# gisbi-kim/lt-mapper

Hardware: AMD Instinct MI355X
Metric: keyframe-pairs/sec (removert+diff) (higher is better)
Workload: dtype f32; 1 GPU; lot-2x500-os1-64-3res; sensor=os1-64

## Files before the change

### include/ltm.h

```cpp
#ifndef LTM_H
#define LTM_H

#include <stddef.h>
#include <stdint.h>

#ifdef __cplusplus
extern "C" {
#endif

#define LTM_ABI_VERSION 1

enum {
    LTM_OK = 0,
    LTM_E_INVALID = -1,
    LTM_E_DEVICE = -2,
    LTM_E_NOMEM = -3,
    LTM_E_UNSUPPORTED = -4
};

typedef struct ltm_ctx ltm_ctx;
typedef uint64_t ltm_cloud;
typedef uint64_t ltm_scanset;
typedef uint64_t ltm_poses;

// ... 40 lines not shown

int ltm_buffer_alloc(ltm_ctx*, size_t bytes, void** dev);
int ltm_buffer_free(ltm_ctx*, void* dev);
int ltm_buffer_fill(ltm_ctx*, void* dev, int byte_value, size_t bytes);
int ltm_buffer_copy(ltm_ctx*, void* dst, const void* src, size_t bytes, int kind);

typedef uint64_t ltm_upload;
int ltm_scanset_upload_begin(ltm_ctx*, size_t capacity_points, ltm_upload* up);
int ltm_scanset_upload_chunk(ltm_ctx*, ltm_upload up, const void* pts, size_t stride_bytes, const uint64_t* kf_sizes, size_t n_kf);
int ltm_scanset_upload_end(ltm_ctx*, ltm_upload up, ltm_scanset* out);

typedef struct ltm_fetch ltm_fetch;
int ltm_cloud_fetch_begin(ltm_ctx*, ltm_cloud, ltm_fetch** out);
int ltm_scanset_fetch_begin(ltm_ctx*, ltm_scanset, ltm_fetch** out);
int ltm_fetch_wait(ltm_fetch*, const void** host_xyzi, size_t* n_points, const uint64_t** offsets, size_t* n_kf);
int ltm_fetch_release(ltm_ctx*, ltm_fetch*);
int ltm_cloud_fetch_chunks_begin(ltm_ctx*, ltm_cloud, ltm_fetch** out);
int ltm_scanset_fetch_chunks_begin(ltm_ctx*, ltm_scanset, ltm_fetch** out);
int ltm_fetch_info(ltm_fetch*, size_t* n_points, const uint64_t** offsets, size_t* n_kf);
int ltm_fetch_next_chunk(ltm_fetch*, const void** host_xyzi, size_t* first_point, size_t* n_points, size_t* first_kf, size_t* n_kf);
int ltm_fetch_chunk_done(ltm_fetch*, const void* host_xyzi);

int ltm_poses_create(ltm_ctx*, size_t n_kf, const double* poses, const double* inv_or_null, ltm_poses* out);
int ltm_inverse4x4(const double* m16, double* inv16);
int ltm_poses_free(ltm_ctx*, ltm_poses);


int ltm_preclean(ltm_ctx*, ltm_scanset in, float radius, ltm_scanset* out);

int ltm_merge_to_global(ltm_ctx*, ltm_scanset scans, ltm_poses poses, ltm_cloud* out);

int ltm_voxel_centroid(ltm_ctx*, ltm_cloud in, float leaf, ltm_cloud* out);
int ltm_voxel_centroid_batch(ltm_ctx*, size_t n, const ltm_cloud* in, const float* leaf, ltm_cloud* out);
int ltm_voxel_centroid_shard(ltm_ctx*, ltm_cloud in, float leaf, uint32_t shard, uint32_t n_shards, ltm_cloud* out);
int ltm_cloud_bbox(ltm_ctx*, ltm_cloud in, float mn[3], float mx[3]);
int ltm_voxel_key_histogram(ltm_ctx*, ltm_cloud in, const float mn[3], const float mx[3], float leaf, uint32_t hist[4096]);
int ltm_voxel_key_split(ltm_ctx*, ltm_cloud in, const float mn[3], const float mx[3], float leaf, uint32_t n_parts, const uint32_t* cut_bins, ltm_cloud* parts);
int ltm_voxel_centroid_box(ltm_ctx*, ltm_cloud in, const float mn[3], const float mx[3], float leaf, ltm_cloud* out);
int ltm_voxel_centroid_scanset(ltm_ctx*, ltm_scanset in, float leaf, ltm_scanset* out);

int ltm_voxel_grid_scanset(ltm_ctx*, ltm_scanset in, float leaf, ltm_scanset* out);
typedef struct ltm_vgs ltm_vgs;
int ltm_voxel_grid_scanset_begin(ltm_ctx*, ltm_scanset in, float leaf, ltm_vgs** ticket);
int ltm_voxel_grid_scanset_end(ltm_ctx*, ltm_vgs* ticket, ltm_scanset* out);

int ltm_visibility_vote(ltm_ctx*, ltm_cloud map, ltm_scanset scans, ltm_poses poses, size_t kf_begin, size_t kf_end,
                        float res_alpha, float diff_thres, int mode, uint8_t* labels_dev);
int ltm_scanset_prepare_range_images(ltm_ctx*, ltm_scanset scans, size_t kf_begin, size_t kf_end, const float* res_alphas, size_t n_alphas);
int ltm_partition_by_labels(ltm_ctx*, ltm_cloud map, const uint8_t* labels_dev, ltm_cloud* kept, ltm_cloud* flagged);
int ltm_visibility_partition(ltm_ctx*, ltm_cloud map, ltm_scanset scans, ltm_poses poses, float res_alpha,
                             float diff_thres, int mode, ltm_cloud* kept, ltm_cloud* flagged, uint8_t* host_labels);

int ltm_reproject(ltm_ctx*, ltm_cloud map, ltm_poses poses, size_t kf_begin, size_t kf_end, float res_alpha, ltm_scanset* out);

int ltm_knn_partition(ltm_ctx*, ltm_cloud target, ltm_scanset scans, ltm_poses poses, size_t kf_begin, size_t kf_end,
                      int k, float thr, ltm_scanset* coexist, ltm_scanset* diff);
int ltm_knn_split_cloud(ltm_ctx*, ltm_cloud target, ltm_cloud query, int k, float thr, ltm_cloud* near, ltm_cloud* far);

typedef struct ltm_search ltm_search;
typedef struct ltm_search_result ltm_search_result;
int ltm_search_build(ltm_ctx*, ltm_cloud target, ltm_search** out);
int ltm_search_free(ltm_ctx*, ltm_search*);
int ltm_search_info(ltm_ctx*, ltm_search*, size_t* n_target, size_t* n_finite);
int ltm_knn_search(ltm_ctx*, ltm_search*, ltm_cloud query, int k, int32_t* idx_dev, float* d2_dev);
int ltm_radius_search(ltm_ctx*, ltm_search*, ltm_cloud query, float radius, int max_nn, ltm_search_result** out);
int ltm_search_result_info(ltm_ctx*, ltm_search_result*, size_t* n_query, size_t* total,
                           const uint64_t** offsets_dev, const int32_t** idx_dev, const float** d2_dev);
int ltm_search_result_free(ltm_ctx*, ltm_search_result*);

int ltm_search_estimate_normals(ltm_ctx*, size_t n_idx, ltm_search* const* idx, int k,
                                const float* viewpoints3_or_null );
int ltm_search_normals_info(ltm_ctx*, ltm_search*, int* k , const void** normals_dev );
int ltm_search_normals_download(ltm_ctx*, ltm_search*, float* nxyzc_host );

typedef struct ltm_sc ltm_sc;
typedef struct {
    double lidar_height;
    int    num_ring;
    int    num_sector;
    double max_radius;
    int    num_candidates;
    double search_ratio;
    double dist_thres;
} ltm_sc_params;
void ltm_sc_default_params(ltm_sc_params*);
int  ltm_sc_from_scanset(ltm_ctx*, ltm_scanset, size_t kf_begin, size_t kf_end, const ltm_sc_params*, ltm_sc** out);
int  ltm_sc_from_descriptors(ltm_ctx*, const double* desc_host, size_t n, const ltm_sc_params*, ltm_sc** out);
int  ltm_sc_info(ltm_ctx*, ltm_sc*, size_t* n, int* num_ring, int* num_sector);
int  ltm_sc_download(ltm_ctx*, ltm_sc*, double* desc, float* ring_keys, double* sector_keys);
int  ltm_sc_distance(ltm_ctx*, ltm_sc* a, ltm_sc* b, const int32_t* pairs_host, size_t n_pairs, const ltm_sc_params*, double* dist_host, int32_t* shift_host);
int  ltm_sc_detect(ltm_ctx*, ltm_sc* database, ltm_sc* queries, const ltm_sc_params*, int32_t* loop_id, int32_t* nn_idx, double* min_dist, int32_t* nn_align,
                   float* yaw_diff_rad);
int  ltm_sc_free(ltm_ctx*, ltm_sc*);

typedef struct {
    double max_corr_dist;
    int    max_iterations;
    double transformation_epsilon;
    double euclidean_fitness_epsilon;
} ltm_icp_params;
typedef struct {
    double   T[16];
    double   fitness;
    double   last_mse;
    int32_t  converged;
    int32_t  iterations;
// ... 69 lines not shown
```

### lt-mapper_amd/capi.py

```python
import ctypes as C
import os

import numpy as np

_HERE = os.path.dirname(os.path.abspath(__file__))
LIB_PATH = os.path.join(_HERE, "libltm_hip.so")

_lib = None

LTM_OK = 0
ERR_NAMES = {0: "LTM_OK", -1: "LTM_E_INVALID", -2: "LTM_E_DEVICE", -3: "LTM_E_NOMEM", -4: "LTM_E_UNSUPPORTED"}


class LtmError(RuntimeError):
    def __init__(self, code, msg):
        super().__init__(f"{ERR_NAMES.get(code, code)}: {msg}")
        self.code = code


class LtmConfig(C.Structure):
    _fields_ = [("vfov", C.c_float), ("hfov", C.c_float), ("lidar2base", C.c_double * 16),
                ("device", C.c_int), ("max_kf_batch", C.c_int)]


# ... 52 lines not shown
    "ltm_cloud_fetch_begin": (_i, [_vp, _u64, C.POINTER(_vp)]),
    "ltm_scanset_fetch_begin": (_i, [_vp, _u64, C.POINTER(_vp)]),
    "ltm_fetch_wait": (_i, [_vp, C.POINTER(_vp), _psz, C.POINTER(_pu64), _psz]),
    "ltm_fetch_release": (_i, [_vp, _vp]),
    "ltm_cloud_fetch_chunks_begin": (_i, [_vp, _u64, C.POINTER(_vp)]),
    "ltm_scanset_fetch_chunks_begin": (_i, [_vp, _u64, C.POINTER(_vp)]),
    "ltm_fetch_info": (_i, [_vp, _psz, C.POINTER(_pu64), _psz]),
    "ltm_fetch_next_chunk": (_i, [_vp, C.POINTER(_vp), _psz, _psz, _psz, _psz]),
    "ltm_fetch_chunk_done": (_i, [_vp, _vp]),
    "ltm_buffer_alloc": (_i, [_vp, _sz, C.POINTER(_vp)]),
    "ltm_buffer_free": (_i, [_vp, _vp]),
    "ltm_buffer_fill": (_i, [_vp, _vp, _i, _sz]),
    "ltm_buffer_copy": (_i, [_vp, _vp, _vp, _sz, _i]),
    "ltm_scanset_upload": (_i, [_vp, _vp, _sz, _pu64, _sz, _pu64]),
    "ltm_scanset_from_device": (_i, [_vp, _vp, _pu64, _sz, _pu64]),
    "ltm_scanset_info": (_i, [_vp, _u64, _psz, _psz]),
    "ltm_scanset_offsets": (_i, [_vp, _u64, _pu64]),
    "ltm_scanset_download": (_i, [_vp, _u64, _vp, _sz, _sz]),
    "ltm_scanset_device_ptr": (_i, [_vp, _u64, C.POINTER(_vp)]),
    "ltm_scanset_as_cloud": (_i, [_vp, _u64, _pu64]),
    "ltm_scanset_concat": (_i, [_vp, _pu64, _sz, _pu64]),
    "ltm_scanset_zip_concat": (_i, [_vp, _u64, _u64, _u64, _pu64]),
    "ltm_scanset_free": (_i, [_vp, _u64]),
    "ltm_poses_create": (_i, [_vp, _sz, _vp, _vp, _pu64]),
    "ltm_poses_free": (_i, [_vp, _u64]),
    "ltm_inverse4x4": (_i, [_vp, _vp]),
    "ltm_preclean": (_i, [_vp, _u64, _f, _pu64]),
    "ltm_merge_to_global": (_i, [_vp, _u64, _u64, _pu64]),
    "ltm_voxel_centroid": (_i, [_vp, _u64, _f, _pu64]),
    "ltm_voxel_centroid_shard": (_i, [_vp, _u64, _f, C.c_uint32, C.c_uint32, _pu64]),
    "ltm_voxel_centroid_batch": (_i, [_vp, _sz, _pu64, C.POINTER(_f), _pu64]),
    "ltm_cloud_bbox": (_i, [_vp, _u64, C.POINTER(_f), C.POINTER(_f)]),
    "ltm_voxel_key_histogram": (_i, [_vp, _u64, C.POINTER(_f), C.POINTER(_f), _f, C.POINTER(C.c_uint32)]),
    "ltm_voxel_key_split": (_i, [_vp, _u64, C.POINTER(_f), C.POINTER(_f), _f, C.c_uint32, C.POINTER(C.c_uint32), _pu64]),
    "ltm_voxel_centroid_box": (_i, [_vp, _u64, C.POINTER(_f), C.POINTER(_f), _f, _pu64]),
    "ltm_voxel_centroid_scanset": (_i, [_vp, _u64, _f, _pu64]),
    "ltm_voxel_grid_scanset": (_i, [_vp, _u64, _f, _pu64]),
    "ltm_voxel_grid_scanset_begin": (_i, [_vp, _u64, _f, C.POINTER(_vp)]),
    "ltm_voxel_grid_scanset_end": (_i, [_vp, _vp, _pu64]),
    "ltm_scanset_prepare_range_images": (_i, [_vp, _u64, _sz, _sz, C.POINTER(_f), _sz]),
    "ltm_visibility_vote": (_i, [_vp, _u64, _u64, _u64, _sz, _sz, _f, _f, _i, _vp]),
    "ltm_partition_by_labels": (_i, [_vp, _u64, _vp, _pu64, _pu64]),
    "ltm_visibility_partition": (_i, [_vp, _u64, _u64, _u64, _f, _f, _i, _pu64, _pu64, _vp]),
    "ltm_lane_create": (_i, [_vp, C.POINTER(_vp)]),
    "ltm_lane_fence": (_i, [_vp, _vp]),
    "ltm_event_record": (_i, [_vp, C.POINTER(_vp)]),
    "ltm_event_wait": (_i, [_vp, _vp]),
    "ltm_event_destroy": (None, [_vp]),
    "ltm_cloud_lend": (_i, [_vp, _u64, _vp, _pu64]),
    "ltm_cloud_give": (_i, [_vp, _u64, _vp, _pu64]),
    "ltm_scanset_lend": (_i, [_vp, _u64, _vp, _pu64]),
    "ltm_scanset_give": (_i, [_vp, _u64, _vp, _pu64]),
    "ltm_reproject": (_i, [_vp, _u64, _u64, _sz, _sz, _f, _pu64]),
    "ltm_knn_partition": (_i, [_vp, _u64, _u64, _u64, _sz, _sz, _i, _f, _pu64, _pu64]),
    "ltm_knn_split_cloud": (_i, [_vp, _u64, _u64, _i, _f, _pu64, _pu64]),
    "ltm_search_build": (_i, [_vp, _u64, C.POINTER(_vp)]),
    "ltm_search_free": (_i, [_vp, _vp]),
    "ltm_search_info": (_i, [_vp, _vp, _psz, _psz]),
    "ltm_knn_search": (_i, [_vp, _vp, _u64, _i, _vp, _vp]),
    "ltm_radius_search": (_i, [_vp, _vp, _u64, _f, _i, C.POINTER(_vp)]),
    "ltm_search_result_info": (_i, [_vp, _vp, _psz, _psz, C.POINTER(_vp), C.POINTER(_vp), C.POINTER(_vp)]),
    "ltm_search_result_free": (_i, [_vp, _vp]),
    "ltm_search_estimate_normals": (_i, [_vp, _sz, C.POINTER(_vp), _i, _vp]),
    "ltm_search_normals_info": (_i, [_vp, _vp, C.POINTER(_i), C.POINTER(_vp)]),
    "ltm_search_normals_download": (_i, [_vp, _vp, _vp]),
    "ltm_sc_default_params": (None, [C.POINTER(ScParams)]),
    "ltm_sc_from_scanset": (_i, [_vp, _u64, _sz, _sz, C.POINTER(ScParams), C.POINTER(_vp)]),
    "ltm_sc_from_descriptors": (_i, [_vp, _vp, _sz, C.POINTER(ScParams), C.POINTER(_vp)]),
    "ltm_sc_info": (_i, [_vp, _vp, _psz, C.POINTER(_i), C.POINTER(_i)]),
    "ltm_sc_download": (_i, [_vp, _vp, _vp, _vp, _vp]),
    "ltm_sc_distance": (_i, [_vp, _vp, _vp, _vp, _sz, C.POINTER(ScParams), _vp, _vp]),
    "ltm_sc_detect": (_i, [_vp, _vp, _vp, C.POINTER(ScParams), _vp, _vp, _vp, _vp, _vp]),
    "ltm_sc_free": (_i, [_vp, _vp]),
    "ltm_icp_default_params": (None, [C.POINTER(IcpParams)]),
    "ltm_icp_align": (_i, [_vp, _sz, C.POINTER(_vp), _pu64, _vp, C.POINTER(IcpParams), _vp, _vp]),
    "ltm_icp_align_scanset": (_i, [_vp, _sz, C.POINTER(_vp), _u64, _vp, _vp, C.POINTER(IcpParams), _vp, _vp]),
    "ltm_icp_align_plane": (_i, [_vp, _sz, C.POINTER(_vp), _pu64, _vp, C.POINTER(IcpParams), _vp, _vp]),
    "ltm_icp_align_plane_scanset": (_i, [_vp, _sz, C.POINTER(_vp), _u64, _vp, _vp, C.POINTER(IcpParams), _vp, _vp]),
    "ltm_icp_align_gicp": (_i, [_vp, _sz, C.POINTER(_vp), C.POINTER(_vp), _vp, C.POINTER(IcpParams), C.c_double, _vp, _vp]),
    "ltm_pose6d_to_affine3f": (_i, [_vp, _sz, _vp]),
    "ltm_submaps_assemble": (_i, [_vp, _u64, _vp, _vp, _sz, _i, _f, _i, _pu64]),
    "ltm_search_build_scanset": (_i, [_vp, _u64, _sz, _sz, C.POINTER(_vp)]),
    "ltm_debug_pool_live": (_i, [_vp, _pu64, _pu64]),
    "ltm_debug_range_image": (_i, [_vp, _u64, _vp, _vp, _f, _vp, _vp]),
    "ltm_debug_viz_images": (_i, [_vp, _u64, _u64, _u64, _sz, _f, _i, _f, _f, _f, _f, _vp, _vp, _vp, _vp]),
    "ltm_debug_project": (_i, [_vp, _vp, _sz, _f, _vp, _vp]),
    "ltm_debug_elevation_fit": (_i, [_f, C.POINTER(_f), C.POINTER(C.c_double)]),
    "ltm_debug_pcl_sort_order": (_i, [C.POINTER(C.c_uint32), C.c_size_t, C.POINTER(C.c_uint32), _i, C.POINTER(C.c_uint32)]),
    "ltm_debug_voxel_key_bits": (_i, [C.POINTER(_f), C.POINTER(_f), _f, _pu64, C.POINTER(C.c_uint), C.POINTER(C.c_double)]),
    "ltm_debug_selfcheck": (_i, [_vp, _pu64, C.POINTER(_i)]),
    "ltm_debug_cull_check": (_i, [_vp, _vp, _sz, _vp, _f, _pu64]),
    "ltm_debug_cull_stats": (_i, [_vp, _pu64, _pu64, _i]),
    "ltm_debug_proj_launch": (_i, [_f, _f, _f, _vp, _sz, _sz, _i, _vp, _vp, C.c_uint32, _sz, _vp, _vp]),
    "ltm_debug_vote_run_launch": (_i, [_sz, _sz, _i, C.c_uint32, _sz, _vp, _vp, _vp, _vp]),
    "ltm_debug_vote_queue_word": (_i, [C.c_float, C.c_float, C.c_float, _vp, _sz, _vp, _vp, _vp]),
    "ltm_debug_cull_validation": (_i, [_vp, _pu64, _pu64]),
    "ltm_debug_occlusion_stats": (_i, [_vp, _pu64, _pu64, _pu64, _i]),
    "ltm_debug_voxel_stats": (_i, [_vp, _pu64, _pu64, _i]),
    "ltm_debug_knn_stats": (_i, [_vp, _pu64, _pu64, _pu64, _pu64, _i]),
    "ltm_debug_sc_paths": (_i, [_i, _i, C.POINTER(_i), C.POINTER(_i)]),
    "ltm_rimg_size": (None, [_f, _f, _f, C.POINTER(_i), C.POINTER(_i)]),
    "ltm_profile_enable": (_i, [_vp, _i]),
    "ltm_profile_reset": (_i, [_vp]),
    "ltm_profile_read_compulsory": (_i, [_vp, C.POINTER(C.c_double), _i]),
    "ltm_profile_read": (_i, [_vp, C.POINTER(C.c_char_p), C.POINTER(C.c_double), _pu64, C.POINTER(C.c_double),
                              C.POINTER(C.c_double), _i]),
# ... 300 lines not shown
        return Cloud(self, out.value)

    def viz_images(self, cmap, scans, poses, kf, alpha, mode=0, range_axis=(0.0, 10.0), diff_axis=(0.0, 0.5)):
        rows, cols = self.rimg_size(alpha)
        out = {k: np.empty((rows, cols, 3), dtype=np.uint8) for k in ("scan", "map", "diff", "ptidx")}
        self._ck(self.lib.ltm_debug_viz_images(self.h, cmap.h, scans.h, poses.h, kf, alpha, mode, range_axis[0], range_axis[1],
                                               diff_axis[0], diff_axis[1], out["scan"].ctypes.data, out["map"].ctypes.data,
                                               out["diff"].ctypes.data, out["ptidx"].ctypes.data))
        return out

    def voxel_centroid_scanset(self, scans, leaf):
        out = _u64()
        self._ck(self.lib.ltm_voxel_centroid_scanset(self.h, scans.h, leaf, C.byref(out)))
        return ScanSet(self, out.value)

    def voxel_grid_scanset(self, scans, leaf):
        out = _u64()
        self._ck(self.lib.ltm_voxel_grid_scanset(self.h, scans.h, leaf, C.byref(out)))
        return ScanSet(self, out.value)

    def voxel_grid_scanset_begin(self, scans, leaf):
        t = C.c_void_p()
        self._ck(self.lib.ltm_voxel_grid_scanset_begin(self.h, scans.h, leaf, C.byref(t)))
        return VgsTicket(self, t, scans)

    def voxel_grid_scanset_end(self, ticket):
        return ticket.end()

    def prepare_scan_images(self, scans, alphas, kf_begin=0, kf_end=None):
        a = (_f * len(alphas))(*[float(x) for x in alphas])
        self._ck(self.lib.ltm_scanset_prepare_range_images(self.h, scans.h, kf_begin, scans.n_kf if kf_end is None else kf_end, a, len(alphas)))

    def visibility_vote(self, cmap, scans, poses, kf_begin, kf_end, alpha, thr, mode, labels_dev_ptr):
        self._ck(self.lib.ltm_visibility_vote(self.h, cmap.h, scans.h, poses.h, kf_begin, kf_end, alpha, thr, mode, labels_dev_ptr))

    def partition_by_labels(self, cmap, labels_dev_ptr):
        k, f = _u64(), _u64()
        self._ck(self.lib.ltm_partition_by_labels(self.h, cmap.h, labels_dev_ptr, C.byref(k), C.byref(f)))
        return Cloud(self, k.value), Cloud(self, f.value)

    def visibility_partition(self, cmap, scans, poses, alpha, thr=0.1, mode=0, want_labels=False):
        k, f = _u64(), _u64()
        labels = np.zeros(len(cmap), dtype=np.uint8) if want_labels else None
        self._ck(self.lib.ltm_visibility_partition(self.h, cmap.h, scans.h, poses.h, alpha, thr, mode, C.byref(k), C.byref(f),
                                                   labels.ctypes.data if want_labels else None))
        kept, flagged = Cloud(self, k.value), Cloud(self, f.value)
        return (kept, flagged, labels) if want_labels else (kept, flagged)

    def reproject(self, cmap, poses, alpha=3.0, kf_begin=0, kf_end=None):
        out = _u64()
        self._ck(self.lib.ltm_reproject(self.h, cmap.h, poses.h, kf_begin, poses.n if kf_end is None else kf_end, alpha, C.byref(out)))
        return ScanSet(self, out.value)

    def knn_partition(self, target, scans, poses, k, thr, kf_begin=0, kf_end=None):
        co, di = _u64(), _u64()
        self._ck(self.lib.ltm_knn_partition(self.h, target.h, scans.h, poses.h, kf_begin, poses.n if kf_end is None else kf_end,
                                            k, thr, C.byref(co), C.byref(di)))
        return ScanSet(self, co.value), ScanSet(self, di.value)

    def knn_split_cloud(self, target, query, k, thr):
        near, far = _u64(), _u64()
        self._ck(self.lib.ltm_knn_split_cloud(self.h, target.h, query.h, k, thr, C.byref(near), C.byref(far)))
        return Cloud(self, near.value), Cloud(self, far.value)

    def search_index(self, cloud):
        if not isinstance(cloud, Cloud):
            cloud = self.upload(_xyzi(cloud))
        h = _vp()
        self._ck(self.lib.ltm_search_build(self.h, cloud.h, C.byref(h)))
        return SearchIndex(self, h.value)

    def search_index_batch(self, scanset, kf_begin=0, kf_end=None):
        ke = scanset.n_kf if kf_end is None else kf_end
        n = max(int(ke) - int(kf_begin), 0)
        hs = (_vp * max(n, 1))()
        self._ck(self.lib.ltm_search_build_scanset(self.h, scanset.h, kf_begin, ke, hs))
        return [SearchIndex(self, hs[i]) for i in range(n)]

    def estimate_normals(self, indices, k=10, viewpoints=None):
        indices = list(indices)
        k = _normals_k(k)
        for x in indices:
            if not isinstance(x, SearchIndex):
                raise TypeError("estimate_normals takes SearchIndex objects (Context.search_index)")
        if len({id(x) for x in indices}) != len(indices):
            raise ValueError("an index is listed twice")
        n = len(indices)
        vp = None
        if viewpoints is not None:
            vp = np.ascontiguousarray(viewpoints, dtype=np.float32).reshape(-1)
            if vp.size != 3 * n:
                raise ValueError("one viewpoint (x, y, z) per index")
        hs = (_vp * max(n, 1))(*[x.h for x in indices])
        self._ck(self.lib.ltm_search_estimate_normals(self.h, n, hs, k, None if vp is None else vp.ctypes.data))

    def loop_submaps(self, scans, keys, search_num, leaf=0.3, affines=None, order="pcl"):
        k = np.ascontiguousarray(keys, dtype=np.int32).reshape(-1)
        a = None
        if affines is not None:
            a = np.ascontiguousarray(affines, dtype=np.float32).reshape(-1, 12)
            if a.shape[0] != scans.n_kf:
                raise ValueError("one affine per keyframe of the scan set")
        out = _u64()
        self._ck(self.lib.ltm_submaps_assemble(self.h, scans.h, None if a is None else a.ctypes.data, k.ctypes.data, k.size, int(search_num), float(leaf),
                                               ORDERS[order], C.byref(out)))
        return ScanSet(self, out.value)
# ... 560 lines not shown
```

### lt-mapper_amd/csrc/ltm_api_core.cpp

```cpp
#include "ltm_internal.h"

namespace ltm_detail {

bool inverse4x4(const double* m, double* inv)
{
    double A[2][2], B[2][2], C[2][2], D[2][2];
    for (int r = 0; r < 2; ++r)
        for (int k = 0; k < 2; ++k) {
            A[r][k] = m[4 * k + r]; B[r][k] = m[4 * (k + 2) + r];
            C[r][k] = m[4 * k + r + 2]; D[r][k] = m[4 * (k + 2) + r + 2];
        }
    const double dA = A[0][0] * A[1][1] - A[0][1] * A[1][0], dB = B[0][0] * B[1][1] - B[0][1] * B[1][0];
    const double dC = C[0][0] * C[1][1] - C[0][1] * C[1][0], dD = D[0][0] * D[1][1] - D[0][1] * D[1][0];
    double AB[2][2], DC[2][2];
    for (int j = 0; j < 2; ++j) {
        AB[0][j] = B[0][j] * A[1][1] - B[1][j] * A[0][1]; AB[1][j] = B[1][j] * A[0][0] - B[0][j] * A[1][0];
        DC[0][j] = C[0][j] * D[1][1] - C[1][j] * D[0][1]; DC[1][j] = C[1][j] * D[0][0] - C[0][j] * D[1][0];
    }
    const double tr = (AB[0][0] * DC[0][0] + AB[1][0] * DC[0][1]) + (AB[0][1] * DC[1][0] + AB[1][1] * DC[1][1]);
    double iA[2][2], iB[2][2], iC[2][2], iD[2][2];
    for (int i = 0; i < 2; ++i)
        for (int j = 0; j < 2; ++j) {
            iD[i][j] = D[i][j] * dA - (AB[0][j] * C[i][0] + AB[1][j] * C[i][1]);
            iA[i][j] = A[i][j] * dD - (DC[0][j] * B[i][0] + DC[1][j] * B[i][1]);
// ... 146 lines not shown
    unsigned char* d = static_cast<unsigned char*>(dst);
    const float one = 1.0f;
    for (size_t i = 0; i < n; ++i) {
        unsigned char* p = d + i * stride;
        if (stride >= 32) {
            memset(p, 0, 32);
            memcpy(p, &packed[4 * i], 12); memcpy(p + 12, &one, 4); memcpy(p + 16, &packed[4 * i + 3], 4);
        } else {
            memcpy(p, &packed[4 * i], 16);
        }
    }
}



}

extern "C" {

int ltm_abi_version(void) { return LTM_ABI_VERSION; }

int ltm_create(const ltm_config* cfg, ltm_ctx** out)
{
    if (!cfg || !out) return LTM_E_INVALID;
    *out = nullptr;
    int ndev = 0;
    if (hipGetDeviceCount(&ndev) != hipSuccess || ndev <= 0) return LTM_E_DEVICE;
    if (cfg->device < 0 || cfg->device >= ndev) return LTM_E_INVALID;
    ltm_ctx* c = new (std::nothrow) ltm_ctx();
    if (!c) return LTM_E_NOMEM;
    c->cfg = *cfg;
    c->device = cfg->device;
    if (cfg->max_kf_batch > 0) c->kf_batch = (size_t)cfg->max_kf_batch;
    double b2l[16];
    if (!(cfg->vfov > 0.0f) || !(cfg->hfov > 0.0f) || !inverse4x4(cfg->lidar2base, b2l)) { delete c; return LTM_E_INVALID; }
    c->l2b_identity = mat_is_identity(cfg->lidar2base);
    if (c->l2b_identity) memcpy(b2l, cfg->lidar2base, sizeof b2l);
    c->b2l_identity = mat_is_identity(b2l);
    c->L2B = to34(cfg->lidar2base); c->B2L = to34(b2l);
    if (hipSetDevice(c->device) != hipSuccess || hipStreamCreateWithFlags(&c->stream, hipStreamNonBlocking) != hipSuccess) {
        delete c;
        return LTM_E_DEVICE;
    }
    c->pool.stream = c->stream;
    auto env_int = [](const char* name, int dflt) { const char* v = getenv(name); return v ? atoi(v) : dflt; };
    c->kopts.map_kernel_variant = env_int("LTM_MAP_KERNEL", 2);
    c->kopts.vote_cull = env_int("LTM_VOTE_CULL", 1);
    c->kopts.tile_cull = env_int("LTM_TILE_CULL", 1);
    c->kopts.vote_tile_run = std::min(std::max(env_int("LTM_VOTE_TILE_RUN", 4), 1), 16);
    c->kopts.map_tile_run = getenv("LTM_MAP_TILE_RUN") ? std::min(std::max(env_int("LTM_MAP_TILE_RUN", 4), 1), 16) : 0;
    c->kopts.map_tile_persist = env_int("LTM_MAP_TILE_PERSIST", 1);
    c->kopts.map_tile_barrier = env_int("LTM_MAP_TILE_BARRIER", 0);
    c->kopts.stats_blockmin = env_int("LTM_STATS_BLOCKMIN", 0);
    {
        unsigned long long* d = nullptr;
        bool ok = hipMalloc(&d, 3 * sizeof(unsigned long long)) == hipSuccess && hipMemsetAsync(d, 0, 24, c->stream) == hipSuccess &&
                  selfcheck_fast_math(cfg->vfov, cfg->hfov, d, c->stream) == hipSuccess &&
                  hipMemcpyAsync(c->selfcheck, d, 24, hipMemcpyDeviceToHost, c->stream) == hipSuccess &&
                  hipStreamSynchronize(c->stream) == hipSuccess;
        if (d) (void)hipFree(d);
        if (!ok) { (void)hipStreamDestroy(c->stream); delete c; return LTM_E_DEVICE; }
        c->fast_math = (c->selfcheck[0] == 0 && c->selfcheck[1] == 0 && c->selfcheck[2] == 0) ? 1 : 0;
        if (const char* v = getenv("LTM_KNN_FAST")) c->knn_two_phase = atoi(v);
        if (const char* v = getenv("LTM_VOXEL_KEYBITS")) c->voxel_key_compress = atoi(v);
        if (const char* v = getenv("LTM_VOXEL_FUSED_TAIL")) c->voxel_fused_tail = atoi(v);
        if (const char* v = getenv("LTM_VOXEL_IDENTITY")) c->voxel_identity = atoi(v);
        if (const char* v = getenv("LTM_OCCLUSION")) c->occlusion_cull = atoi(v);
        if (getenv("LTM_OCCLUSION_STATS")) c->occlusion_stats_on = 1;
        if (const char* v = getenv("LTM_OCCLUSION_MIN_PAIRS")) c->occlusion_min_pairs = (size_t)atoll(v);
        if (const char* v = getenv("LTM_OCCLUSION_RNEAR")) {
            const float r = (float)atof(v);
            c->occlusion_r_near = std::isfinite(r) ? std::max(1.0f, r) : 60.0f;
        }
        if (const char* v = getenv("LTM_KNN_STATS")) c->knn_stats_on = atoi(v);
        if (const char* v = getenv("LTM_CULL_SELFCHECK")) c->cull_selfcheck = atoi(v);
        if (const char* v = getenv("LTM_CULL_EPS_SCALE")) c->cull_eps_scale = (float)atof(v);
        if (const char* v = getenv("LTM_CULL_EPS_FLOOR")) c->cull_eps_floor = (float)atof(v);
        c->el_fit = elevation_fit_for(c->cfg.vfov, c->el_c, &c->el_fit_err);
        if (const char* v = getenv("LTM_HEAVY_CHAIN")) c->heavy_chain_on = atoi(v);
        if (const char* v = getenv("LTM_HEAVY_MIN_BLOCKS")) c->heavy_min_blocks = (size_t)atoll(v);
    }
    c->heavy = std::make_shared<HeavyChain>();
    *out = c;
    return LTM_OK;
}

void ltm_destroy(ltm_ctx* c)
{
    if (!c) return;
    (void)hipSetDevice(c->device);
    (void)hipStreamSynchronize(c->stream);
    vgs_release_all(c);
    search_release_all(c);
    sc_release_all(c);
    for (Pending& p : c->pending) { (void)hipEventDestroy(p.a); (void)hipEventDestroy(p.b); }
    for (hipEvent_t e : c->event_pool) (void)hipEventDestroy(e);
    if (c->copy_stream) { (void)hipStreamSynchronize(c->copy_stream); (void)hipStreamDestroy(c->copy_stream); }
    for (auto& kv : c->uploads) { for (int b = 0; b < 2; ++b) if (kv.second.ev[b]) (void)hipEventDestroy(kv.second.ev[b]); c->pool.free(kv.second.d); }
    for (PinnedBlock& b : c->pinned) (void)hipHostFree(b.p);
    if (c->scratch_pinned) (void)hipHostFree(c->scratch_pinned);
    if (c->live_counts) (void)hipFree(c->live_counts);
    if (getenv("LTM_OCCLUSION_STATS") && c->occl_pairs)
        fprintf(stderr, "[ltm] occlusion cull of the exact-image kernel: %llu (tile, keyframe) pairs, %.2f %% in the first shell, %.2f %% projected in all, %.2f %% dropped\n",
                (unsigned long long)c->occl_pairs, 100.0 * c->occl_near / c->occl_pairs, 100.0 * c->occl_far_live / c->occl_pairs,
                100.0 * (c->occl_pairs - c->occl_far_live) / c->occl_pairs);
    if (getenv("LTM_OCCLUSION_STATS") && c->occl_quarters)
// ... 867 lines not shown
```

### lt-mapper_amd/csrc/ltm_api_vote.cpp

```cpp
#include "ltm_internal.h"

namespace ltm_detail {

static Geom geom_from(float vfov, float hfov, float alpha, int fast_math, int el_fit, const float* el_c, float cull_eps_scale, float cull_eps_floor)
{
    Geom g;
    g.vfov = vfov; g.hfov = hfov;
    g.rows = (int)roundf(vfov * alpha);
    g.cols = (int)roundf(hfov * alpha);
    g.fast = fast_math;
    const float ppd = std::max((float)g.rows / g.vfov, (float)g.cols / g.hfov);
    const float scale = cull_eps_scale > 0.0f ? cull_eps_scale : (el_fit ? 3.0e-4f : 6.0e-4f);
    g.cull_eps_px = std::max(cull_eps_floor, scale * ppd);
    g.el_fit = el_fit;
    for (int i = 0; i < 4; ++i) g.el_c[i] = el_c[i];
    const double out_deg = std::min(2.0, (double)g.vfov / std::max(g.rows, 1));
    g.el_tclamp = (float)std::tan((0.5 * (double)g.vfov + out_deg) * (3.14159265358979323846 / 180.0));
    return g;
}
Geom geom_for(const ltm_ctx* c, float alpha)
{
    return geom_from(c->cfg.vfov, c->cfg.hfov, alpha, c->fast_math, c->el_fit, c->el_c, c->cull_eps_scale, c->cull_eps_floor);
}

// ... 246 lines not shown
        const uint32_t* scan_img = scan_images(c, ss_handle, ss, kb, nb, g, &smax, cull ? thr : -1.0f, &qbound);
        {
            ProfScope p(c, "vote_fill", (double)(nb * npx), (double)(nb * npx * 8));
            LTM_HIP(fill_u64(map_img.as<uint64_t>(), (uint64_t)kNoPointBits << 32, nb * npx, c->stream));
        }
        {
            double pts = (double)map.n * nb, bytes = 16.0 * pts + (double)nb * 8.0 * npx, bytes_c = 16.0 * map.n + (double)nb * (cull ? 12.0 : 8.0) * npx;
            const bool count_live = cull && c->prof_on && (c->kopts.tile_cull != 0) && smax && c->pending_live.size() < (size_t)kLiveSlots;
            if (count_live) {
                if (!c->live_counts) LTM_HIP(hipMalloc(reinterpret_cast<void**>(&c->live_counts), sizeof(unsigned long long) * kLiveSlots));
                const int slot = (int)c->pending_live.size();
                LTM_HIP(hipMemsetAsync(c->live_counts + slot, 0, sizeof(unsigned long long), c->stream));
                LTM_HIP(count_live_tiles(ps.approx_dev, kb, nb, tb.as<float>(), n_tiles, smax, thr, c->live_counts + slot, c->stream));
                c->pending_live.push_back(PendingLive{prof_class(c, "vote_map_cull"), slot, pts, (double)nb * 8.0 * npx, (double)map.n, (double)nb * 12.0 * npx});
                pts = 0.0; bytes = 0.0; bytes_c = 0.0;
            }
            ProfScope p(c, cull ? "vote_map_cull" : "vote_map_exact", pts, bytes, bytes_c);
            if (cull) {
                HeavyScope hs(c, vote_run_blocks(map.n, nb, c->kopts.vote_tile_run));
                LTM_HIP(vote_map_range_images(map.d, map.n, ps.inv_dev, ps.approx_dev, kb, nb, c->B2L, c->b2l_identity, g, qbound, tb.as<float>(), smax, thr, mode,
                                              map_img.as<uint64_t>(), hs.stream(), c->kopts));
                hs.done();
            } else exact_map_images(c, map, ps, kb, nb, g, map_img.as<uint64_t>());
        }
        {
            ProfScope p(c, "vote_compare", (double)(nb * npx), (double)(nb * npx) * 12 + (double)nb * map.n / 8.0);
            LTM_HIP(compare_and_flag(scan_img, map_img.as<uint64_t>(), nb * npx, thr, mode, labels_dev, c->stream));
        }
    }
}

void do_partition(ltm_ctx* c, const Cloud& map, const uint8_t* labels, ltm_cloud* kept, ltm_cloud* flagged)
{
    const size_t n = map.n;
    if (n == 0) {
        float4* d;
        if (kept) *kept = alloc_cloud(c, 0, &d);
        if (flagged) *flagged = alloc_cloud(c, 0, &d);
        return;
    }
    DevBuf pos(c, n * sizeof(uint32_t));
    ProfScope p(c, "partition", (double)n, (double)n * (16 + 1 + 4 + 4 + 16));
    const size_t nf = count_flags(c, labels, n, pos);
    float4 *dk = nullptr, *df = nullptr;
    ltm_cloud hk = 0, hf = 0;
    if (kept) hk = alloc_cloud(c, n - nf, &dk);
    if (flagged) hf = alloc_cloud(c, nf, &df);
    LTM_HIP(partition_scatter(map.d, labels, pos.as<uint32_t>(), n, dk, df, c->stream));
    if (kept) { *kept = hk; inherit_frame(c, hk, map); }
    if (flagged) { *flagged = hf; inherit_frame(c, hf, map); }
}


}

extern "C" {

int ltm_scanset_prepare_range_images(ltm_ctx* c, ltm_scanset hs, size_t kf_begin, size_t kf_end, const float* alphas, size_t n_alphas)
{
    return guarded(c, [&] {
        LTM_REQUIRE(alphas || n_alphas == 0, "null argument");
        const ScanSet& ss = get_ss(c, hs);
        LTM_REQUIRE(kf_begin <= kf_end && kf_end <= ss.nkf(), "keyframe range out of bounds");
        if (kf_begin == kf_end || n_alphas == 0) return;
        std::vector<Geom> geoms;
        for (size_t i = 0; i < n_alphas; ++i) geoms.push_back(geom_for(c, alphas[i]));
        const size_t KB = std::min(c->kf_batch, kf_end - kf_begin);
        for (size_t kb = kf_begin; kb < kf_end; kb += KB) scan_images_prepare(c, hs, ss, kb, std::min(KB, kf_end - kb), geoms);
    });
}

int ltm_visibility_vote(ltm_ctx* c, ltm_cloud hmap, ltm_scanset hs, ltm_poses hp, size_t kf_begin, size_t kf_end, float alpha,
                        float thr, int mode, uint8_t* labels_dev)
{
    return guarded(c, [&] {
        LTM_REQUIRE(labels_dev, "null labels buffer");
        do_vote(c, get_cloud(c, hmap), hs, get_ss(c, hs), get_poses(c, hp), kf_begin, kf_end, alpha, thr, mode, labels_dev);
        sync(c);
    });
}

int ltm_partition_by_labels(ltm_ctx* c, ltm_cloud hmap, const uint8_t* labels_dev, ltm_cloud* kept, ltm_cloud* flagged)
{
    return guarded(c, [&] {
        LTM_REQUIRE(labels_dev || get_cloud(c, hmap).n == 0, "null labels buffer");
        const Cloud map = get_cloud(c, hmap);
        do_partition(c, map, labels_dev, kept, flagged);
        sync(c);
    });
}

int ltm_visibility_partition(ltm_ctx* c, ltm_cloud hmap, ltm_scanset hs, ltm_poses hp, float alpha, float thr, int mode,
                             ltm_cloud* kept, ltm_cloud* flagged, uint8_t* host_labels)
{
    return guarded(c, [&] {
        const Cloud map = get_cloud(c, hmap);
        const Poses& p = get_poses(c, hp);
        DevBuf labels(c, std::max<size_t>(map.n, 1));
        LTM_HIP(hipMemsetAsync(labels.p, 0, std::max<size_t>(map.n, 1), c->stream));
        do_vote(c, map, hs, get_ss(c, hs), p, 0, p.n, alpha, thr, mode, labels.as<uint8_t>());
        if (host_labels) d2h(c, host_labels, labels.p, map.n);
        do_partition(c, map, labels.as<uint8_t>(), kept, flagged);
    });
}

int ltm_reproject(ltm_ctx* c, ltm_cloud hmap, ltm_poses hp, size_t kf_begin, size_t kf_end, float alpha, ltm_scanset* out)
{
    return guarded(c, [&] {
        LTM_REQUIRE(out, "null argument");
        const Cloud map = get_cloud(c, hmap);
        const Poses& p = get_poses(c, hp);
        LTM_REQUIRE(kf_begin <= kf_end && kf_end <= p.n, "keyframe range out of bounds");
        LTM_REQUIRE(map.n < 0xffffffffull, "map too large for 32-bit point indices");
        const Geom g = geom_for(c, alpha);
        LTM_REQUIRE(g.rows > 0 && g.cols > 0, "empty range image");
        const size_t npx = (size_t)g.rows * g.cols;
        const size_t nk = kf_end - kf_begin;
        std::vector<uint64_t> off(nk + 1, 0);
        struct Piece { float4* d; size_t n; };
        std::vector<Piece> pieces;
        if (nk && map.n) {
            const size_t KB = std::min(c->kf_batch, nk);
            DevBuf img(c, KB * npx * 8), pos(c, KB * npx * 4);
            const size_t tb = scan_temp_bytes(KB * npx);
            DevBuf temp(c, tb), bout(c, (KB + 1) * 4);
            for (size_t kb = kf_begin; kb < kf_end; kb += KB) {
                const size_t nb = std::min(KB, kf_end - kb);
                LTM_HIP(fill_u64(img.as<uint64_t>(), (uint64_t)kNoPointBits << 32, nb * npx, c->stream));
                {
                    ProfScope ps(c, "reproject_map", (double)map.n * nb, (double)nb * (16.0 * map.n + 8.0 * npx), 16.0 * map.n + (double)nb * 8.0 * npx);
                    exact_map_images(c, map, p, kb, nb, g, img.as<uint64_t>());
                }
                ProfScope ps(c, "reproject_gather", (double)(nb * npx), (double)(nb * npx) * 12);
                LTM_HIP(exclusive_scan_img_valid(img.as<uint64_t>(), pos.as<uint32_t>(), nb * npx, temp.p, tb, c->stream));
                LTM_HIP(image_bounds(pos.as<uint32_t>(), img.as<uint64_t>(), npx, nb, bout.as<uint32_t>(), c->stream));
                std::vector<uint32_t> b(nb + 1);
                d2h(c, b.data(), bout.p, (nb + 1) * 4);
                const size_t total = b[nb];
                const uint64_t base = off[kb - kf_begin];
                for (size_t j = 1; j <= nb; ++j) off[kb - kf_begin + j] = base + b[j];
                float4* d = reinterpret_cast<float4*>(c->pool.alloc(std::max<size_t>(total, 1) * 16));
                LTM_HIP(reproject_gather(img.as<uint64_t>(), pos.as<uint32_t>(), npx, nb, map.d, p.inv_dev, kb, c->B2L, c->b2l_identity, d, c->stream));
                pieces.push_back(Piece{d, total});
            }
        }
        float4* d = nullptr;
        if (pieces.size() == 1) d = pieces[0].d;
        else {
            d = reinterpret_cast<float4*>(c->pool.alloc(std::max<size_t>(off[nk], 1) * 16));
            size_t at = 0;
            for (Piece& pc : pieces) { d2d(c, d + at, pc.d, pc.n * 16); at += pc.n; }
            sync(c);
            for (Piece& pc : pieces) c->pool.free(pc.d);
        }
        *out = new_scanset(c, d, std::move(off));
    });
}

int ltm_debug_range_image(ltm_ctx* c, ltm_cloud h, const double* T1, const double* T2, float alpha, float* rimg, int32_t* ptidx)
{
    return guarded(c, [&] {
        LTM_REQUIRE(rimg, "null argument");
        const Cloud cl = get_cloud(c, h);
        const Geom g = geom_for(c, alpha);
        const size_t npx = (size_t)g.rows * g.cols;
        DevBuf img(c, npx * 8), r(c, npx * 4), ix(c, npx * 4);
        LTM_HIP(fill_u64(img.as<uint64_t>(), (uint64_t)kNoPointBits << 32, npx, c->stream));
        HostMat34 a, b;
        if (T1) a = to34(T1);
        if (T2) b = to34(T2);
        LTM_HIP(single_range_image(cl.d, cl.n, T1 ? &a : nullptr, T2 ? &b : nullptr, g, img.as<uint64_t>(), c->stream));
        LTM_HIP(decode_image(img.as<uint64_t>(), npx, r.as<float>(), ix.as<int32_t>(), c->stream));
        d2h(c, rimg, r.p, npx * 4);
        if (ptidx) d2h(c, ptidx, ix.p, npx * 4);
    });
}

static void jet_lut_bgr(uint8_t* lut)
{
    for (int i = 0; i < 256; ++i) {
        const double x = (double)i / 255.0;
        const double bgr[3] = {std::min(4.0 * x + 0.5, 2.5 - 4.0 * x), std::min(4.0 * x - 0.5, 3.5 - 4.0 * x), std::min(4.0 * x - 1.5, 4.5 - 4.0 * x)};
        for (int ch = 0; ch < 3; ++ch) {
            const float sample = (float)std::min(1.0, std::max(0.0, bgr[ch]));
            lut[3 * i + ch] = (uint8_t)std::min(255l, std::max(0l, std::lrint((double)(sample * 255.0f))));
        }
    }
}

int ltm_debug_viz_images(ltm_ctx* c, ltm_cloud hmap, ltm_scanset hscans, ltm_poses hposes, size_t kf, float alpha, int mode,
                         float range_min, float range_max, float diff_min, float diff_max,
                         uint8_t* scan_bgr, uint8_t* map_bgr, uint8_t* diff_bgr, uint8_t* ptidx_bgr)
{
    return guarded(c, [&] {
        LTM_REQUIRE(mode == 0 || mode == 1, "mode must be 0 (scan-map) or 1 (map-scan)");
        LTM_REQUIRE(range_max != range_min && diff_max != diff_min, "empty colour axis");
        const Cloud map = get_cloud(c, hmap);
        const ScanSet& ss = get_ss(c, hscans);
        const Poses& ps = get_poses(c, hposes);
        LTM_REQUIRE(ss.nkf() == ps.n && kf < ps.n, "keyframe out of range");
        LTM_REQUIRE(map.n < 0x7fffffffull, "map too large for an int32 index image");
        const Geom g = geom_for(c, alpha);
        const size_t npx = (size_t)g.rows * g.cols;
        const uint32_t* smax = nullptr;
        const uint32_t* scan_img = scan_images(c, hscans, ss, kf, 1, g, &smax);
        DevBuf img(c, npx * 8), mr(c, npx * 4), mi(c, npx * 4), df(c, npx * 4), out(c, npx * 3), lutd(c, 768);
        LTM_HIP(fill_u64(img.as<uint64_t>(), (uint64_t)kNoPointBits << 32, npx, c->stream));
        if (map.n)
// ... 143 lines not shown
```

### lt-mapper_amd/csrc/ltm_k_projection.hip

```cpp
#include "ltm_kernels_common.h"
#include <rocprim/device/device_scan.hpp>
#include <rocprim/iterator/transform_iterator.hpp>

namespace ltm {

__global__ void k_fill_u32(uint32_t* p, uint32_t v, size_t n)
{
    size_t i = (size_t)blockIdx.x * blockDim.x + threadIdx.x;
    const size_t stride = (size_t)gridDim.x * blockDim.x;
    for (; i < n; i += stride) p[i] = v;
}
__global__ void k_fill_u64(uint64_t* p, uint64_t v, size_t n)
{
    size_t i = (size_t)blockIdx.x * blockDim.x + threadIdx.x;
    const size_t stride = (size_t)gridDim.x * blockDim.x;
    for (; i < n; i += stride) p[i] = v;
}
hipError_t fill_u32(uint32_t* p, uint32_t v, size_t n, hipStream_t s)
{
    if (!n) return hipSuccess;
    k_fill_u32<<<dim3((unsigned)std::min<size_t>(grid_for(n), 8192)), dim3(kBlock), 0, s>>>(p, v, n);
    return hipGetLastError();
}
hipError_t fill_u64(uint64_t* p, uint64_t v, size_t n, hipStream_t s)
// ... 229 lines not shown
}

template <bool EL3 = false>
__device__ __forceinline__ CullCand cull_candidates(const ProjLaunch& pl, float3 p)
{
    const RimgGeom& g = pl.g;
    CullCand cc;
    const float xy2 = __builtin_fmaf(p.x, p.x, p.y * p.y);
    cc.r2 = __builtin_fmaf(p.z, p.z, xy2);
    const float inv_rxy = __builtin_amdgcn_rsqf(xy2);
    const float t_el = fabsf(p.z) * inv_rxy;
    const float ax = fabsf(p.x), ay = fabsf(p.y);
    const float az_oct = asin_octant_approx(fminf(ax, ay) * inv_rxy);
    float el_abs;
    if (EL3) {
        const float t = fminf(t_el, g.el_tclamp), u = t * t;
        el_abs = t * __builtin_fmaf(__builtin_fmaf(__builtin_fmaf(g.el_c3, u, g.el_c2), u, g.el_c1), u, g.el_c0);
    } else {
        el_abs = atan_unit_approx(fminf(t_el, 1.0f));
    }
    const float el = __builtin_copysignf(el_abs, p.z);
    float az = (ay > ax) ? (1.57079632679f - az_oct) : az_oct;
    az = (p.x < 0.0f) ? (3.14159265359f - az) : az;
    az = __builtin_copysignf(az, p.y);
    cc.rowh = __builtin_fmaf(el, -pl.row_scale, pl.row_bias);
    cc.colh = __builtin_fmaf(az, pl.col_scale, pl.col_bias);
    const bool certain = fmaxf(__builtin_amdgcn_fractf(cc.rowh), __builtin_amdgcn_fractf(cc.colh)) < pl.certain_lim;
    cc.unusual = (fabsf(p.y) <= __builtin_fmaf(-1.0e-6f, p.x, 1.0e-18f)) | (cc.r2 > 6.4e7f);
    if (!EL3) cc.unusual |= !pl.steep_clamps & (t_el > 1.0f);
    cc.multi = !certain;
    cc.rb = (int)__builtin_amdgcn_fmed3f(cc.rowh, 0.0f, g.row_max);
    cc.cb = (int)__builtin_amdgcn_fmed3f(cc.colh, 0.0f, g.col_max);
    cc.r0 = cc.r1 = cc.rb; cc.c0 = cc.c1 = cc.cb;
    return cc;
}

__device__ __forceinline__ float cull_r_lo(float r2) { return __builtin_amdgcn_sqrtf(r2) * (1.0f - 1.5e-6f); }

__device__ __forceinline__ void cull_expand(const ProjLaunch& pl, CullCand& cc)
{
    const RimgGeom& g = pl.g;
    const float rfl = floorf(cc.rowh), cfl = floorf(cc.colh);
    const float rfr = cc.rowh - rfl, cfr = cc.colh - cfl;
    const int rc = (int)rfl, ccn = (int)cfl;
    const int rmax = g.rows - 1, cmax = g.cols - 1;
    const float lim = pl.certain_lim;
    cc.r0 = min(max(rc, 0), rmax);
    cc.r1 = min(max(rc + (rfr >= lim ? 1 : 0), 0), rmax);
    cc.c0 = min(max(ccn, 0), cmax);
    cc.c1 = min(max(ccn + (cfr >= lim ? 1 : 0), 0), cmax);
}


__device__ unsigned long long g_cull_stats[4];

static constexpr int kCullQueue = 2048;

static constexpr uint32_t kEmptyTag = 0xffffffffu;
template <int SLOTS>
__device__ __forceinline__ void table_init(uint32_t* __restrict__ tags, uint64_t* __restrict__ vals, uint32_t* __restrict__ amin)
{
    for (int s = threadIdx.x; s < SLOTS; s += kBlock) {
        if (tags) tags[s] = kEmptyTag;
        if (amin) amin[s] = 0x7f800000u;
        if (vals) vals[s] = ~0ull;
    }
}
template <int ROWS, int COLS>
__device__ __forceinline__ int table_claim(uint32_t* __restrict__ tags, int row, int col, uint32_t px)
{
    const int slot = ((row & (ROWS - 1)) * COLS) | (col & (COLS - 1));
    uint32_t t = tags[slot];
    if (t == kEmptyTag) {
        const uint32_t old = atomicCAS(&tags[slot], kEmptyTag, px);
        t = (old == kEmptyTag) ? px : old;
    }
    return (t == px) ? slot : -1;
}
template <int ROWS, int COLS>
__device__ __forceinline__ void table_min(uint64_t* __restrict__ vals, uint32_t* __restrict__ tags, uint64_t* __restrict__ imgk, int row, int col, uint32_t px,
                                          uint64_t v)
{
    const int slot = table_claim<ROWS, COLS>(tags, row, col, px);
    if (slot >= 0) { if (v < vals[slot]) __hip_atomic_fetch_min(&vals[slot], v, __ATOMIC_RELAXED, __HIP_MEMORY_SCOPE_WORKGROUP); }
    else img_min_u64(imgk + px, v);
}
template <int SLOTS>
__device__ __forceinline__ void table_flush(const uint32_t* __restrict__ tags, const uint64_t* __restrict__ vals, uint64_t* __restrict__ imgk)
{
    for (int s = threadIdx.x; s < SLOTS; s += kBlock) {
        const uint32_t t = tags[s];
        if (t != kEmptyTag && vals[s] != ~0ull) img_min_u64(imgk + t, vals[s]);
    }
}
template <bool B2L_IDENTITY, int ROWS, int COLS>
__device__ __forceinline__ void exact_insert(const float4* __restrict__ map, uint32_t i, const Mat34& Tinv, const HostMat34& b2l_h, const RimgGeom& g,
                                             uint64_t* __restrict__ vals, uint32_t* __restrict__ tags, uint64_t* __restrict__ imgk)
{
    const float4 p4 = map[i];
    float3 p = xform(Tinv, make_float3(p4.x, p4.y, p4.z));
    if (B2L_IDENTITY) p = xform_identity(p); else p = xform(to_dev(b2l_h), p);
    const Sph s = cart2sph(p.x, p.y, p.z);
    int row, col;
    pixel_row_col(g, s.az, s.el, row, col);
    table_min<ROWS, COLS>(vals, tags, imgk, row, col, (uint32_t)(row * g.cols + col), ((uint64_t)f2u(s.r) << 32) | (uint64_t)i);
}
template <bool B2L_IDENTITY>
// ... 235 lines not shown
                for (int u = 0; u < kInFlight; ++u) nxt[u] = mapr[(G << 10) + (uint32_t)u * kBlock + threadIdx.x];
            }
        }
        if (!more) break;
        float4 pt[kInFlight];
        CullCand cc[kInFlight];
        float q0[kInFlight];
        uint32_t pxi[kInFlight];
#pragma unroll
        for (int u = 0; u < kInFlight; ++u) pt[u] = nxt[u];
        float3 p[kInFlight];
#pragma unroll
        for (int u = 0; u < kInFlight; ++u) {
            bool ok;
            p[u] = xform_approx(ap, pt[u], ok);
        }
        const uint32_t Gcur = G;
        if ((G & 3u) != 3u) ++G;
        else if (rest) { G = (uint32_t)__builtin_ctz(rest) << 2; rest &= rest - 1u; }
        else more = false;
#pragma unroll
        for (int u = 0; u < kInFlight; ++u) nxt[u] = mapr[(G << 10) + (uint32_t)u * kBlock + threadIdx.x];
#pragma unroll
        for (int u = 0; u < kInFlight; ++u) {
            cc[u] = cull_candidates<EL3>(pl, p[u]);
            cc[u].unusual |= cc[u].multi | (B2L_IDENTITY ? false : (cc[u].r2 < pl.rmin2));
            pxi[u] = __umul24((uint32_t)cc[u].rb, (uint32_t)g.cols) + (uint32_t)cc[u].cb;
            q0[u] = *reinterpret_cast<const float*>(reinterpret_cast<const char*>(qk) + (pxi[u] << 2));
        }
        bool mt[kInFlight];
#pragma unroll
        for (int u = 0; u < kInFlight; ++u) {
            mt[u] = cc[u].unusual | (cc[u].r2 < q0[u]);
        }
        const Ballot4 qg = ballot4(mt);
        if (qg.total) {
            const uint32_t word = (Gcur << 26) | (lane << kVoteQueuePxBits);
#pragma unroll
            for (int u = 0; u < kInFlight; ++u)
                if (mt[u]) seg[nq + ballot4_pos(qg, u)] = (word | ((uint32_t)u << 24)) | (cc[u].unusual ? kVoteQueuePxUncertain : pxi[u]);
            nq += qg.total;
        }
    }
    if (__builtin_expect(slow != 0u, 0)) nsurv += exact_tiles<B2L_IDENTITY, 8, 64>(slow, first_tile, map, M, inv_pose, b2l_h, g, vals, tags, imgk);
    if (sampled && lane == 0u && nsurv) atomicAdd(&g_cull_stats[0], (unsigned long long)nsurv);
    __syncthreads();
    uncertain_tail<B2L_IDENTITY, 8, 64, kCullQueue>(uqueue, ucount, map, run_base, inv_pose, b2l_h, g, vals, tags, imgk);
    __syncthreads();
    table_flush<kCullSlots>(tags, vals, imgk);
}

hipError_t cull_stats(unsigned long long* out2, int reset, hipStream_t s, int which_kernel)
{
    hipError_t e = hipMemcpyFromSymbolAsync(out2, HIP_SYMBOL(g_cull_stats), 16, 16 * (size_t)(which_kernel ? 1 : 0), hipMemcpyDeviceToHost, s);
    if (e != hipSuccess) return e;
    e = hipStreamSynchronize(s);
    if (e != hipSuccess || !reset) return e;
    const unsigned long long z[4] = {0, 0, 0, 0};
    e = hipMemcpyToSymbolAsync(HIP_SYMBOL(g_cull_stats), z, 32, 0, hipMemcpyHostToDevice, s);
    return e == hipSuccess ? hipStreamSynchronize(s) : e;
}

hipError_t vote_map_range_images(const float4* map, size_t M, const double* inv_poses_dev, const float* approx_poses_dev, size_t kb, size_t nb,
                                 HostMat34 b2l, int b2l_identity, Geom g, const float* qbound_img, const float* tile_bounds_dev,
                                 const uint32_t* smax_bits_dev, float thr, int mode, uint64_t* map_img, hipStream_t s, const KernelOpts& ko)
{
    if (!M || !nb) return hipSuccess;
    if (mode != 0 || !ko.vote_cull || !approx_poses_dev || !qbound_img) return map_range_images(map, M, inv_poses_dev, approx_poses_dev, kb, nb, b2l, b2l_identity, g, map_img, s, ko);
    const ProjLaunch pl = make_proj_launch(g, b2l, b2l_identity, M);
    const RunLaunch rl = make_run_launch(pl.n_tiles, (uint32_t)std::max(ko.vote_tile_run, 1));
    dim3 grid(run_kf_grid(rl, nb));
    const float* tb = (ko.tile_cull && smax_bits_dev) ? tile_bounds_dev : nullptr;
    LTM_LAUNCH_ID_EL3(k_vote_map_cull, b2l_identity, g.el_fit != 0, grid, s, map, (uint32_t)M, inv_poses_dev, approx_poses_dev, (uint32_t)kb, (uint32_t)nb, b2l, pl, rl,
                      qbound_img, tb, smax_bits_dev, thr, map_img);
    return hipGetLastError();
}

__global__ void __launch_bounds__(kBlock)
k_cull_check(const float* __restrict__ xyz, size_t n, HostMat34 T, HostMat34 b2l, int b2l_identity, const float* __restrict__ ap, ProjLaunch pl,
             unsigned long long* __restrict__ bad)
{
    const size_t i = (size_t)blockIdx.x * blockDim.x + threadIdx.x;
    if (i >= n) return;
    const RimgGeom& g = pl.g;
    const float4 p4 = make_float4(xyz[3 * i], xyz[3 * i + 1], xyz[3 * i + 2], 0.0f);
    float3 pe = make_float3(p4.x, p4.y, p4.z), pa = pe;
    bool ok = true;
    if (ap) {
        pe = xform(to_dev(T), pe);
        pe = b2l_identity ? xform_identity(pe) : xform(to_dev(b2l), pe);
        pa = xform_approx(ap, p4, ok);
    }
    CullCand cc = g.el_fit ? cull_candidates<true>(pl, pa) : cull_candidates<false>(pl, pa);
    if (cc.unusual || !ok) return;
    if (ap && !b2l_identity && cc.r2 < pl.rmin2) return;
    if (cc.multi) cull_expand(pl, cc);
    const Sph s = cart2sph(pe.x, pe.y, pe.z);
    int row, col;
    pixel_row_col(g, s.az, s.el, row, col);
    const double re2 = (double)s.r * (double)s.r;
    const float r_lo = cull_r_lo(cc.r2);
    const bool good = (row == cc.r0 || row == cc.r1) && (col == cc.c0 || col == cc.c1) && (r_lo <= s.r) && (s.r <= r_lo * (1.0f + 3.0e-6f)) &&
                      (re2 >= (double)cc.r2 * (1.0 - 3.0e-6)) && (re2 <= (double)cc.r2 * (1.0 + 3.0e-6));
    if (!good) atomicAdd(bad, 1ull);
}
hipError_t cull_check(const float* xyz_dev, size_t n, const HostMat34* T, const HostMat34* b2l, int b2l_identity, const float* approx_pose_dev,
                      Geom g, unsigned long long* bad_dev, hipStream_t s)
{
    if (!n) return hipSuccess;
    HostMat34 z{};
    const int ident = b2l ? b2l_identity : 1;
    k_cull_check<<<dim3(grid_for(n)), dim3(kBlock), 0, s>>>(xyz_dev, n, T ? *T : z, b2l ? *b2l : z, ident,
// ... 334 lines not shown
                exact_insert<B2L_IDENTITY, kRows, 64>(map, block_base + li, Tinv, b2l_h, g, vals, tags, imgk);
            if (nloc == per_block) nsurv += per_block / (kBlock / 64);
        }
    }
    if ((blockIdx.x & 63u) == 0u) {
        if (threadIdx.x == 0) atomicAdd(&g_cull_stats[3], (unsigned long long)(n_full * per_block));
        if (lane == 0u && nsurv) atomicAdd(&g_cull_stats[2], (unsigned long long)nsurv);
    }
    __syncthreads();
    uncertain_tail<B2L_IDENTITY, kRows, 64, kBmRunUQueue>(uqueue, ucount, map, run_base, inv_pose, b2l_h, g, vals, tags, imgk);
    __syncthreads();
    for (int s = threadIdx.x; s < kSlots; s += kBlock) {
        const uint32_t tg = tags[s];
        if (tg != kEmptyTag && vals[s] != ~0ull) img_min_u64(imgk + tg, vals[s]);
    }
}

hipError_t map_range_images(const float4* map, size_t M, const double* inv_poses_dev, const float* approx_poses_dev, size_t kb, size_t nb,
                            HostMat34 b2l, int b2l_identity, Geom g, uint64_t* map_img, hipStream_t s, const KernelOpts& ko)
{
    if (!M || !nb) return hipSuccess;
    const ProjLaunch pl = make_proj_launch(g, b2l, b2l_identity, M);
    if (ko.map_kernel_variant >= 2 && approx_poses_dev && pl.packable && !pl.vote_queueable) {
        const size_t per_block = (size_t)kBlock * kPtsPerThread;
        dim3 grid(tile_kf_grid((M + per_block - 1) / per_block, nb));
        LTM_LAUNCH_ID_EL3(k_map_rimg_blockmin, b2l_identity, g.el_fit != 0, grid, s, map, (uint32_t)M, inv_poses_dev, approx_poses_dev, (uint32_t)kb, (uint32_t)nb, b2l, pl,
                          map_img, nullptr, 0u, nullptr);
        return hipGetLastError();
    }
    if (ko.map_kernel_variant >= 2 && approx_poses_dev) {
        uint32_t T = ko.map_tile_run > 0 ? (uint32_t)ko.map_tile_run : kBmRunDefaultT;
        if (ko.map_tile_run <= 0)
            while (T > 1u && (uint64_t)((pl.n_tiles + T - 1u) / T) * nb < kBmRunMinBlocks) T >>= 1;
        const RunLaunch rl = make_run_launch(pl.n_tiles, T);
        dim3 grid(run_kf_grid(rl, nb));
        const uint32_t flags = (ko.map_tile_barrier ? 0u : kBmRunNoBarrier) | (ko.map_tile_persist ? 0u : kBmRunResetPerTile);
        LTM_LAUNCH_ID_EL3(k_map_rimg_blockmin_run, b2l_identity, g.el_fit != 0, grid, s, map, (uint32_t)M, inv_poses_dev, approx_poses_dev, (uint32_t)kb, (uint32_t)nb, b2l, pl,
                          rl, flags, map_img);
        return hipGetLastError();
    }
    if (ko.map_kernel_variant >= 1) {
        const size_t per_block = (size_t)kBlock * kPtsPerThread;
        dim3 grid(tile_kf_grid((M + per_block - 1) / per_block, nb));
        if (b2l_identity) k_map_rimg_lds<true><<<grid, dim3(kBlock), 0, s>>>(map, (uint32_t)M, inv_poses_dev, (uint32_t)kb, (uint32_t)nb, b2l, pl, map_img);
        else k_map_rimg_lds<false><<<grid, dim3(kBlock), 0, s>>>(map, (uint32_t)M, inv_poses_dev, (uint32_t)kb, (uint32_t)nb, b2l, pl, map_img);
        return hipGetLastError();
    }
    dim3 grid(grid_for(M), (unsigned)nb);
    if (b2l_identity) k_map_rimg<true><<<grid, dim3(kBlock), 0, s>>>(map, M, inv_poses_dev, kb, b2l, pl, map_img);
    else k_map_rimg<false><<<grid, dim3(kBlock), 0, s>>>(map, M, inv_poses_dev, kb, b2l, pl, map_img);
    return hipGetLastError();
}

struct SphereRect { int r0, r1, c0, c1; float d_lo; bool cullable; };
__device__ __forceinline__ SphereRect sphere_rect(const RimgGeom& g, const float* __restrict__ ap, const float* __restrict__ tb)
{
    SphereRect o; o.cullable = false; o.r0 = o.r1 = o.c0 = o.c1 = 0; o.d_lo = 0.0f;
    const float smin = ap[15];
    if (!(smin > 0.999f)) return o;
    const float cx = 0.5f * (tb[0] + tb[3]), cy = 0.5f * (tb[1] + tb[4]), cz = 0.5f * (tb[2] + tb[5]);
    const float hx = 0.5f * (tb[3] - tb[0]), hy = 0.5f * (tb[4] - tb[1]), hz = 0.5f * (tb[5] - tb[2]);
    const float rho = __builtin_sqrtf(hx * hx + hy * hy + hz * hz) * 1.001f + 2.0e-3f;
    bool ok;
    const float3 l = xform_approx(ap, make_float4(cx, cy, cz, 0.0f), ok);
    const float d = __builtin_sqrtf(l.x * l.x + l.y * l.y + l.z * l.z);
    if (!ok || !(d > 2.0f * rho) || !(d < 8.0e3f)) return o;
    const float ratio = rho / d;
    const float alpha = asinf(ratio) * 1.01f + 2.0e-4f;
    const float rxy = __builtin_sqrtf(l.x * l.x + l.y * l.y);
    const float el0 = atan2f(l.z, rxy), az0 = atan2f(l.y, l.x);
    if (!(fabsf(el0) + alpha < 1.39f)) return o;
    const float sa = sinf(alpha) / cosf(fabsf(el0) + alpha);
    if (!(sa < 0.95f)) return o;
    const float daz = asinf(sa) * 1.01f + 2.0e-4f;
    if (!(az0 - daz > -3.1415f && az0 + daz < 3.1415f)) return o;
    const float r2d = 57.29577951308232f;
    const float row_hi_el = g.frows * (1.0f - ((el0 + alpha) * r2d + g.half_v) / g.vfov), row_lo_el = g.frows * (1.0f - ((el0 - alpha) * r2d + g.half_v) / g.vfov);
    const float col_lo = g.fcols * (((az0 - daz) * r2d + g.half_h) / g.hfov), col_hi = g.fcols * (((az0 + daz) * r2d + g.half_h) / g.hfov);
    o.r0 = (int)fminf(fmaxf(floorf(row_hi_el) - 1.0f, 0.0f), g.row_max);
    o.r1 = (int)fminf(fmaxf(ceilf(row_lo_el) + 1.0f, 0.0f), g.row_max);
    o.c0 = (int)fminf(fmaxf(floorf(col_lo) - 1.0f, 0.0f), g.col_max);
    o.c1 = (int)fminf(fmaxf(ceilf(col_hi) + 1.0f, 0.0f), g.col_max);
    o.d_lo = (d - rho) * 0.9995f - 2.0e-3f;
    o.cullable = o.d_lo > 0.0f;
    return o;
}

__global__ void __launch_bounds__(kBlock)
k_pair_shell_select(const float* __restrict__ approx_poses, uint32_t kb, uint32_t nb, const float* __restrict__ tile_bounds, uint32_t n_tiles, Geom gg,
                    float r_lo, float r_hi, const uint32_t* __restrict__ cmax, uint32_t rbs, uint32_t cbs, uint8_t* __restrict__ done, uint8_t* __restrict__ flags,
                    uint32_t* __restrict__ dirty, uint32_t dw, const float* __restrict__ sub_bounds, uint8_t* __restrict__ submask, unsigned long long* __restrict__ sub_stats)
{
    const uint32_t t = blockIdx.x * blockDim.x + threadIdx.x;
    if (t >= n_tiles * nb) return;
    if (done[t]) { flags[t] = 0; return; }
    const uint32_t tile = t / nb, kfb = t % nb;
    const float* ap = approx_poses + 16 * (size_t)(kb + kfb);
    const float* tb = tile_bounds + 6 * (size_t)tile;
    float d2 = 0.0f;
#pragma unroll
    for (int d = 0; d < 3; ++d) { const float c = ap[9 + d]; const float e = fmaxf(fmaxf(tb[d] - c, c - tb[3 + d]), 0.0f); d2 = __builtin_fmaf(e, e, d2); }
    const RimgGeom g = make_geom(gg);
    const SphereRect sr = sphere_rect(g, ap, tb);
    if (!sr.cullable || !(d2 == d2)) d2 = 0.0f;
    if (!(d2 >= r_lo * r_lo && d2 < r_hi * r_hi)) { flags[t] = 0; return; }
    bool live = true;
// ... 273 lines not shown
```

### lt-mapper_amd/csrc/ltm_kernels.h

```cpp
#pragma once
#include <hip/hip_runtime_api.h>
#include <stddef.h>
#include <stdint.h>

namespace ltm {

struct Geom {
    float vfov, hfov;
    int rows, cols;
    int fast;
    float cull_eps_px;
    int el_fit;
    float el_c[4];
    float el_tclamp;
};

struct HostMat34 { double m[12]; };

static const uint32_t kNoPointBits = 0x461C4000u;

hipError_t fill_u32(uint32_t* p, uint32_t v, size_t n, hipStream_t s);
hipError_t fill_u64(uint64_t* p, uint64_t v, size_t n, hipStream_t s);

hipError_t scan_range_images(const float4* scans, const uint64_t* offsets_dev, size_t kb, size_t nb,
                             uint64_t first_pt, uint64_t n_pts, uint64_t max_kf_pts, Geom g, uint32_t* scan_img, uint32_t* smax_bits, hipStream_t s);
static constexpr int kMaxScanShapes = 8;
hipError_t scan_range_images_multi(const float4* scans, const uint64_t* offsets_dev, size_t kb, size_t nb, uint64_t n_pts, uint64_t max_kf_pts, Geom g,
                                   int n_shapes, const int* rows, const int* cols, uint32_t* const* imgs, uint32_t* const* smax_bits, hipStream_t s);
hipError_t scan_qbound(const uint32_t* scan_img, size_t n, float thr, float* qbound, hipStream_t s);
hipError_t tile_bounds(const float4* map, size_t M, float* bounds, hipStream_t s);
hipError_t subtile_bounds(const float4* map, size_t M, float* bounds, hipStream_t s);
struct KernelOpts {
    int map_kernel_variant = 2;
    int vote_cull = 1;
    int tile_cull = 1;
    int vote_tile_run = 4;
    int map_tile_run = 0;
    int map_tile_persist = 1;
    int map_tile_barrier = 0;
    int stats_blockmin = 0;
};
hipError_t map_range_images(const float4* map, size_t M, const double* inv_poses_dev, const float* approx_poses_dev, size_t kb, size_t nb,
                            HostMat34 b2l, int b2l_identity, Geom g, uint64_t* map_img, hipStream_t s, const KernelOpts& ko);
hipError_t occlusion_shell_pairs(const float* approx_poses_dev, size_t kb, size_t nb, const float* tile_bounds_dev, size_t n_tiles, Geom g, float r_lo, float r_hi,
                                 const uint64_t* img, int use_cmax, uint32_t* cmax, uint8_t* done, uint8_t* flags, uint32_t* pos, uint32_t* list, uint32_t* count,
                                 void* temp, size_t temp_bytes, hipStream_t s, uint32_t* dirty_rows = nullptr,
                                 const float* sub_bounds_dev = nullptr, uint8_t* submask = nullptr, unsigned long long* sub_stats = nullptr);
hipError_t map_range_images_pairs(const float4* map, size_t M, const double* inv_poses_dev, const float* approx_poses_dev, size_t kb, size_t nb,
                                  HostMat34 b2l, int b2l_identity, Geom g, uint64_t* map_img, const uint32_t* pairs, size_t n_pairs, hipStream_t s, const KernelOpts& ko,
                                  const uint8_t* submask = nullptr);
hipError_t compare_and_flag(const uint32_t* scan_img, const uint64_t* map_img, size_t n_px_total, float thr, int mode,
                            uint8_t* labels, hipStream_t s);
hipError_t vote_map_range_images(const float4* map, size_t M, const double* inv_poses_dev, const float* approx_poses_dev, size_t kb, size_t nb,
                                 HostMat34 b2l, int b2l_identity, Geom g, const float* qbound_img, const float* tile_bounds_dev,
                                 const uint32_t* smax_bits_dev, float thr, int mode, uint64_t* map_img, hipStream_t s, const KernelOpts& ko);
hipError_t count_live_tiles(const float* approx_poses_dev, size_t kb, size_t nb, const float* tile_bounds_dev, size_t n_tiles,
                            const uint32_t* smax_bits_dev, float thr, unsigned long long* live_dev, hipStream_t s);
static constexpr int kProjLaunchFloats = 16, kProjLaunchWords = 12;
hipError_t proj_launch_debug(Geom g, HostMat34 b2l, int b2l_identity, size_t M, size_t nb, int on_device, float* f, uint32_t* u);
void proj_launch_blocks(size_t M, size_t nb, uint32_t first_block, size_t n, uint32_t* tile, uint32_t* kf);
size_t vote_run_blocks(size_t M, size_t nb, int tile_run);
unsigned vote_run_launch_blocks(size_t M, size_t nb, int tile_run, uint32_t first_block, size_t n, uint32_t* run, uint32_t* kf, uint32_t* run_len);
static constexpr int kVoteQueueWords = 8;
void vote_queue_word_debug(Geom g, uint32_t* u, size_t n, const uint32_t* px, uint32_t* row, uint32_t* col);
hipError_t cull_stats(unsigned long long* out2, int reset, hipStream_t s, int which_kernel);
hipError_t cull_check(const float* xyz_dev, size_t n, const HostMat34* T, const HostMat34* b2l, int b2l_identity, const float* approx_pose_dev,
                      Geom g, unsigned long long* bad_dev, hipStream_t s);
hipError_t cull_probe_points(Geom g, size_t n, const HostMat34* pose, float* xyz_dev, hipStream_t s);
hipError_t single_range_image(const float4* pts, size_t n, const HostMat34* T1, const HostMat34* T2, Geom g,
                              uint64_t* img, hipStream_t s);
hipError_t decode_image(const uint64_t* img, size_t npx, float* rimg, int32_t* ptidx, hipStream_t s);
hipError_t viz_diff(const uint32_t* scan_bits, const float* map_r, size_t n, int mode, float* out, hipStream_t s);
hipError_t viz_colormap_f32(const float* src, size_t n, float a, float b, const uint8_t* lut, uint8_t* bgr, hipStream_t s);
hipError_t viz_colormap_i32(const int32_t* src, size_t n, double a, double b, const uint8_t* lut, uint8_t* bgr, hipStream_t s);
hipError_t debug_project(const float* xyz_dev, size_t n, Geom g, float* az_el_r, int32_t* row_col, hipStream_t s);
hipError_t selfcheck_fast_math(float vfov, float hfov, unsigned long long* counts_dev, hipStream_t s);

size_t scan_temp_bytes(size_t n);
hipError_t exclusive_scan_u8(const uint8_t* labels, uint32_t* pos, size_t n, void* temp, size_t temp_bytes, hipStream_t s);
hipError_t exclusive_scan_img_valid(const uint64_t* img, uint32_t* pos, size_t n, void* temp, size_t temp_bytes, hipStream_t s);
hipError_t exclusive_scan_u32(const uint32_t* in, uint32_t* out, size_t n, void* temp, size_t temp_bytes, hipStream_t s);
hipError_t partition_scatter(const float4* in, const uint8_t* labels, const uint32_t* pos, size_t n,
                             float4* kept, float4* flagged, hipStream_t s);
hipError_t reproject_gather(const uint64_t* img, const uint32_t* pos, size_t npx, size_t nb, const float4* map,
                            const double* inv_poses_dev, size_t kb, HostMat34 b2l, int b2l_identity,
                            float4* out, hipStream_t s);
hipError_t image_bounds(const uint32_t* pos, const uint64_t* img, size_t npx, size_t nb, uint32_t* out, hipStream_t s);
hipError_t flag_bounds(const uint32_t* pos, const uint8_t* flag, size_t n, const uint64_t* offsets_dev, size_t kf0, uint64_t first, size_t nb,
                       uint32_t* out, hipStream_t s);
hipError_t gather_u32(const uint32_t* in, const uint64_t* idx_dev, size_t m, size_t n, uint32_t tail_value_index_n,
                      uint32_t* out, hipStream_t s);

hipError_t transform_cloud(const float4* in, size_t n, const HostMat34* t1, const HostMat34* t2, float4* out, hipStream_t s);
hipError_t transform_scans(const float4* in, const uint64_t* offsets_dev, size_t n_kf, uint64_t n_pts,
                           HostMat34 first, int first_identity, const double* per_kf_dev, float4* out, hipStream_t s);
hipError_t zip_concat(const float4* a, const uint64_t* oa, const float4* b, const uint64_t* ob, const float4* c, const uint64_t* oc,
// ... 144 lines not shown
```

### lt-mapper_amd/dist.py

```python
import os

import numpy as np
import torch


def shard_range(n, rank, world):
    return (n * rank) // world, (n * (rank + 1)) // world


class LazyScans:

    def __init__(self, sops, local, kb, ke, n):
        self.sops, self.local, self.kb, self.ke, self.n = sops, local, kb, ke, n
        self._full = None

    def full(self):
        if self._full is None:
            self._full = self.sops._allgather_scanset(self.local, self.n)
        return self._full

    def download(self):
        return self.full().download()

    def info(self):
# ... 6 lines not shown
    SESSION_GROUPS = os.environ.get("LTM_SESSION_GROUPS")

    def _session_groups_on(self):
        if self.SESSION_GROUPS is not None:
            return str(self.SESSION_GROUPS) not in ("0", "False")
        try:
            return self.dist.get_backend() != "nccl"
        except Exception:
            return True

    def __init__(self, ops, dist, rank, world, group=None, peer=None):
        self.ops, self.dist, self.rank, self.world, self.group = ops, dist, rank, world, group
        self.peer = peer
        self._pose_slices = {}
        self._session_groups = None

    def session_groups(self):
        if self.group is not None or self.world < 2 or self.world % 2 or not self._session_groups_on():
            return None
        if self._session_groups is None:
            pgs = [self.dist.new_group(ranks=list(range(g, self.world, 2))) for g in (0, 1)]
            g = self.rank % 2
            gops = ShardedOps(self.ops, self.dist, self.rank // 2, self.world // 2, group=pgs[g], peer=self.rank ^ 1)
            gops.VOXEL_SHARD_MIN = self.VOXEL_SHARD_MIN
            self._session_groups = (gops, g)
        return self._session_groups

    def swap_clouds_with_peer(self, clouds):
        assert self.peer is not None, "swap_clouds_with_peer is an operation of session-group ops"
        ts = [self.ops.cloud_to_tensor(c) for c in clouds]
        dev = ts[0].device
        mine_n = torch.tensor([t.shape[0] for t in ts], dtype=torch.int64, device=dev)
        their_n = torch.empty_like(mine_n)
        send = torch.cat(ts).contiguous() if int(mine_n.sum()) else torch.zeros((0, 4), dtype=torch.float32, device=dev)

        def swap(out, inp):
            if self.dist.get_rank() < self.peer:
                self.dist.send(inp, self.peer); self.dist.recv(out, self.peer)
            else:
                self.dist.recv(out, self.peer); self.dist.send(inp, self.peer)
        swap(their_n, mine_n)
        rows = [int(x) for x in their_n.cpu().tolist()]
        recv = torch.empty((sum(rows), 4), dtype=torch.float32, device=dev)
        if sum(rows) or send.shape[0]:
            swap(recv, send)
        out, at = [], 0
        for n in rows:
            out.append(self.ops.cloud_from_tensor(recv[at:at + n].contiguous()) if n else self.ops.empty_cloud())
            at += n
        return out

    def __getattr__(self, name):
        return getattr(self.ops, name)

    def _range(self, poses):
        return shard_range(self.ops.n_keyframes(poses), self.rank, self.world)

    def _local_poses(self, poses):
        kb, ke = self._range(poses)
        key = (id(poses), kb, ke)
        if key not in self._pose_slices:
            self._pose_slices[key] = (poses, self.ops.poses_slice(poses, kb, ke))
        return self._pose_slices[key][1]

    def _check(self, scans, poses):
        kb, ke = self._range(poses)
        assert (scans.kb, scans.ke, scans.n) == (kb, ke, self.ops.n_keyframes(poses)), "scan shard and pose shard disagree"
        return kb, ke

    def _allgather_scanset(self, local, n_total):
        pts, off = self.ops.scanset_to_tensors(local)
        n_local = len(off) - 1
        n_max = max(shard_range(n_total, r, self.world)[1] - shard_range(n_total, r, self.world)[0] for r in range(self.world))
        assert n_local <= n_max, "scan shard larger than any keyframe block"
        mine = torch.full((n_max + 2,), -1, dtype=torch.int64, device=pts.device)
        mine[0] = n_local
        mine[1: n_local + 2] = torch.as_tensor([int(x) for x in off], dtype=torch.int64)
        gathered = [torch.empty_like(mine) for _ in range(self.world)]
        self.dist.all_gather(gathered, mine, group=self.group)
        counts = []
        for h in torch.stack(gathered).cpu().tolist():
            counts.append(h[1: int(h[0]) + 2])
        sizes = [c[-1] for c in counts]
        cap = max(max(sizes), 1)
        pad = torch.zeros((cap, 4), dtype=torch.float32, device=pts.device)
        pad[: pts.shape[0]] = pts
        bufs = [torch.empty_like(pad) for _ in range(self.world)]
        self.dist.all_gather(bufs, pad, group=self.group)
        parts = [self.ops.scanset_from_tensors(bufs[r][: sizes[r]].contiguous(), counts[r]) for r in range(self.world)]
        return self.ops.concat_scansets(parts)

    def _allgather_cloud(self, local):
        t = self.ops.cloud_to_tensor(local)
        mine = torch.tensor([t.shape[0]], dtype=torch.int64, device=t.device)
        sizes = [torch.empty_like(mine) for _ in range(self.world)]
        self.dist.all_gather(sizes, mine, group=self.group)
        sizes = [int(x) for x in torch.cat(sizes).cpu().tolist()]
        cap = max(max(sizes), 1)
        pad = torch.zeros((cap, 4), dtype=torch.float32, device=t.device)
        pad[: t.shape[0]] = t
        bufs = [torch.empty_like(pad) for _ in range(self.world)]
        self.dist.all_gather(bufs, pad, group=self.group)
        return self.ops.cloud_from_tensor(torch.cat([bufs[r][: sizes[r]] for r in range(self.world)]).contiguous())

    def voxel(self, c, leaf):
        if self.world == 1 or self.ops.size(c) < self.VOXEL_SHARD_MIN:
# ... 99 lines not shown
        dev = self.ops.cloud_to_tensor(loc).device
        box = torch.tensor([float(v) for v in mn] + [-float(v) for v in mx], dtype=torch.float32, device=dev)
        self.dist.all_reduce(box, op=self.dist.ReduceOp.MIN, group=self.group)
        box = box.cpu().numpy()
        gmn, gmx = box[:3].astype(np.float32), (-box[3:]).astype(np.float32)
        if not np.isfinite(gmn).all():
            return self.ops.empty_cloud()
        hist = torch.as_tensor(self.ops.voxel_key_histogram(loc, gmn, gmx, leaf).astype(np.int64), device=dev)
        self.dist.all_reduce(hist, op=self.dist.ReduceOp.SUM, group=self.group)
        cuts = self.balanced_cuts(hist.cpu().numpy(), self.world)
        mine = self._alltoall_clouds(self.ops.voxel_key_split(loc, gmn, gmx, leaf, cuts))
        return self._allgather_cloud(self.ops.voxel_box(mine, gmn, gmx, leaf))

    def merge_voxel_batch(self, merges, clouds, leaf):
        outs = [self.merge_voxel(s, p, leaf) for s, p in merges]
        return outs + (self.voxel_batch(list(clouds), leaf) if clouds else [])


class CommMeter:

    def __init__(self, ops):
        self.ops = ops
        self.events = {"label_allreduce": [0, 0], "scans_allgather": [0, 0], "voxel_allgather": [0, 0], "points_alltoall": [0, 0]}
        self.sharded_voxel_points = 0
        self._tag = "_comm_meter_local_%x" % id(self)

    def __getattr__(self, name):
        return getattr(self.ops, name)

    def reset(self):
        for v in self.events.values():
            v[0] = v[1] = 0
        self.sharded_voxel_points = 0

    def _note(self, kind, nbytes):
        self.events[kind][0] += 1
        self.events[kind][1] += int(nbytes)

    def _mark(self, s):
        try:
            setattr(s, self._tag, True)
        except AttributeError:
            pass
        return s

    def _is_local(self, s):
        return getattr(s, self._tag, False) is True

    def vote_partition(self, cmap, scans, poses, alpha, thr, mode):
        self._note("label_allreduce", self.ops.size(cmap))
        return self.ops.vote_partition(cmap, scans, poses, alpha, thr, mode)

    def reproject(self, cmap, poses, alpha): return self._mark(self.ops.reproject(cmap, poses, alpha))

    def knn_partition(self, target, scans, poses, k, thr):
        co, di = self.ops.knn_partition(target, scans, poses, k, thr)
        return self._mark(co), self._mark(di)

    def zip_concat(self, a, b, c): return self._mark(self.ops.zip_concat(a, b, c))
    def voxel_scanset(self, s, leaf): return self._mark(self.ops.voxel_scanset(s, leaf))
    def voxel_grid_scanset(self, s, leaf): return self._mark(self.ops.voxel_grid_scanset(s, leaf)) if self._is_local(s) else self.ops.voxel_grid_scanset(s, leaf)

    def voxel_grid_scanset_begin(self, s, leaf): return (self.ops.voxel_grid_scanset_begin(s, leaf), self._is_local(s))

    def voxel_grid_scanset_end(self, ticket):
        out = self.ops.voxel_grid_scanset_end(ticket[0])
        return self._mark(out) if ticket[1] else out
    def preclean(self, s, radius): return self._mark(self.ops.preclean(s, radius)) if self._is_local(s) else self.ops.preclean(s, radius)

    def merge_to_global(self, scans, poses):
        if self._is_local(scans):
            n_kf, n_pts = scans.info()
            self._note("scans_allgather", 16 * n_pts + 8 * (n_kf + 2))
        return self.ops.merge_to_global(scans, poses)

    def merge_voxel_batch(self, merges, clouds, leaf):
        if hasattr(self.ops, "merge_voxel_batch"):
            outs = self.ops.merge_voxel_batch(merges, clouds, leaf)
        else:
            outs = self.ops.voxel_batch([self.ops.merge_to_global(s, p) for s, p in merges] + list(clouds), leaf)
        for (scans, _), o in zip(merges, outs):
            if self._is_local(scans):
                _, n_pts = scans.info()
                self._note("points_alltoall", 16 * n_pts)
                self._note("voxel_allgather", 16 * self.ops.size(o))
                self.sharded_voxel_points += n_pts
            elif self.ops.size(o) and scans.info()[1] >= ShardedOps.VOXEL_SHARD_MIN:
                self._note("voxel_allgather", 16 * self.ops.size(o))
                self.sharded_voxel_points += scans.info()[1]
        for c, o in zip(clouds, outs[len(merges):]):
            if self.ops.size(c) >= ShardedOps.VOXEL_SHARD_MIN:
                self._note("voxel_allgather", 16 * self.ops.size(o))
                self.sharded_voxel_points += self.ops.size(c)
        return outs

    def voxel(self, c, leaf):
        out = self.ops.voxel(c, leaf)
        if self.ops.size(c) >= ShardedOps.VOXEL_SHARD_MIN:
            self._note("voxel_allgather", 16 * self.ops.size(out))
            self.sharded_voxel_points += self.ops.size(c)
        return out

    def voxel_batch(self, clouds, leaf):
        outs = self.ops.voxel_batch(clouds, leaf)
        for c, o in zip(clouds, outs):
            if self.ops.size(c) >= ShardedOps.VOXEL_SHARD_MIN:
# ... 65 lines not shown
```

### lt-mapper_amd/host/removert/Session.h

```cpp
#pragma once
#include <memory>
#include <set>
#include <string>
#include <utility>
#include <vector>

#include "removert/Comm.h"
#include "removert/RosParamServer.h"
#include "removert/utility.h"

namespace ltremovert
{

struct Device
{
    ltm_ctx* ctx = nullptr;
    std::shared_ptr<Comm> comm;
    explicit Device(const RosParamServer& p, int device_ordinal = -1, std::shared_ptr<Comm> comm_ = nullptr);
    struct LaneOf { Device& parent; };
    explicit Device(LaneOf l);
    ~Device();
    int rank() const { return comm ? comm->rank() : 0; }
    int world() const { return comm ? comm->world() : 1; }
    Device(const Device&) = delete;
// ... 47 lines not shown
class Session : public RosParamServer
{
public:
    const float kReprojectionAlpha = 3.0;
    static size_t kVoxelShardMin;

    explicit Session(std::shared_ptr<Device> dev);

    std::shared_ptr<Device> dev_;
    std::shared_ptr<Comm> group_comm_;
    Comm* comm() const { return group_comm_ ? group_comm_.get() : dev_->comm.get(); }
    int rank() const { return comm() ? comm()->rank() : 0; }
    int world() const { return comm() ? comm()->world() : 1; }
    void enterSessionGroup(std::shared_ptr<Comm> group);
    void leaveSessionGroup();
    std::string sess_type_;
    float kDownsampleVoxelSize;
    std::string scan_dir_, pose_path_;

    std::vector<std::string> scan_names_, scan_paths_;
    std::vector<Matrix4d> scan_poses_, scan_inverse_poses_;
    int num_scans_ = 0;

    int keyframe_gap_ = 1;
    std::vector<std::string> keyframe_names_, keyframe_paths_;
    std::vector<Matrix4d> keyframe_poses_, keyframe_inverse_poses_;

    ltm_poses poses_h_ = 0;
    ltm_poses poses_local_h_ = 0;
    size_t kf_begin_ = 0, kf_end_ = 0;
    ScansPtr keyframe_scans_, keyframe_scans_static_projected_, keyframe_scans_dynamic_;
    ScansPtr scans_knn_coexist_, scans_knn_diff_;
    ScansPtr keyframe_scans_updated_, keyframe_scans_updated_strong_, keyframe_scans_pd_, keyframe_scans_strong_pd_,
        keyframe_scans_strong_nd_, keyframe_scans_weak_nd_;

    mutable CloudPtr map_global_orig_, map_global_curr_, map_global_curr_static_, map_global_curr_dynamic_;
    mutable CloudPtr map_global_updated_, map_global_updated_strong_;
    mutable CloudPtr map_global_nd_, map_global_nd_strong_, map_global_nd_weak_;
    mutable CloudPtr map_global_pd_, map_global_pd_orig_, map_global_pd_strong_, map_global_pd_weak_;

    void loadSessionInfo(std::string _sess_type, std::string _scan_dir, std::string _pose_path);
    void setDownsampleSize(float _voxel_size);
    void clearKeyframes(void);
    void parseKeyframes(int _gap = 1);
    void parseKeyframes(std::pair<int, int> _range, int _gap = 1);
    void parseKeyframesInROI(const std::vector<Matrix4d>& _roi_poses, int _gap = 1);
    void loadKeyframes(void);
    void precleaningKeyframes(float _radius);
    void mergeScansWithinGlobalCoord(void);

    void parseStaticScansViaProjection(void);
    void parseUpdatedStaticScansViaProjection(void);
    void parseUpdatedStrongStaticScansViaProjection(void);
    void parsePDScansViaProjection(void);
    void parseStrongPDScansViaProjection(void);
    void parseWeakNDScansViaProjection(void);
    void parseStrongNDScansViaProjection(void);
    void parseScansViaProjection(const CloudPtr& _map, ScansPtr& _vec_to_store);

    void updateScansScanwise();
    void extractLowDynPointsViaKnnDiff(const CloudPtr& _target_map);
    void extractHighDynPointsViaKnnDiff(const CloudPtr& _target_map);
    std::pair<CloudPtr, CloudPtr> partitionLowDynamicPointsOfScanByKnn(int _scan_idx);
    std::pair<CloudPtr, CloudPtr> partitionHighDynamicPointsOfScanByKnn(int _scan_idx);
    void allocateMemory() {}
    CloudPtr knn_target_map_;
    void constructGlobalNDMap();
    void removeWeakNDMapPointsHavingStrongNDInNear();
    void constructGlobalPDMap();
    void revertStrongPDMapPointsHavingWeakPDInNear();

    CloudPtr wrap(ltm_cloud h) const { return std::make_shared<CloudH>(dev_->ctx, h); }
    ScansPtr wrap_scans(ltm_scanset h) const { return std::make_shared<ScansH>(dev_->ctx, h); }
    ScansPtr wrap_shard(ltm_scanset h) const;
    ScansPtr gatherScans(const ScansPtr& scans) const;
    void stageArgs(const ScansPtr& scans, ltm_poses* poses, size_t* kb, size_t* ke) const;
    CloudPtr mergeScansToGlobal(const ScansPtr& scans) const;
    CloudPtr mergeVoxel(const ScansPtr& scans, float leaf) const;
    CloudPtr octreeDownsampling(const CloudPtr& src, float leaf) const;
    std::vector<CloudPtr> octreeDownsamplingBatch(const std::vector<CloudPtr>& src, float leaf) const;
    CloudPtr concat(const std::vector<CloudPtr>& parts) const;
    void uploadPoses();
    void setKeyframeBlock();
    void adoptKeyframes(const Session& from, bool with_scans);
};

}
```

### lt-mapper_amd/host/src/Removerter.cpp

```cpp
#include "removert/Removerter.h"

#include <algorithm>
#include <cstdlib>
#include <sstream>

#include <chrono>
#include <cmath>
#include <cstdio>
#include <cstring>
#include <fstream>
#include <iostream>
#include <stdexcept>
#include <thread>

namespace ltremovert
{

#define LTM_INFO(msg) do { if (!logQuiet()) std::cout << "\033[1;32m" << msg << "\033[0m" << std::endl; } while (0)

static std::shared_ptr<Device> make_device() { RosParamServer p; return std::make_shared<Device>(p); }

Removerter::Removerter() : Removerter(make_device()) {}

Removerter::Removerter(std::shared_ptr<Device> dev) : dev_(std::move(dev)), central_sess_(dev_), query_sess_(dev_)
// ... 420 lines not shown
        std::vector<CloudPtr> ins = {Q.mergeScansToGlobal(Q.scans_knn_coexist_), C.mergeScansToGlobal(C.scans_knn_coexist_),
                                     Q.mergeScansToGlobal(Q.scans_knn_diff_), C.mergeScansToGlobal(C.scans_knn_diff_),
                                     C.map_global_nd_weak_, Q.map_global_pd_strong_, Q.map_global_pd_weak_};
        if (has_strong_nd) ins.push_back(C.map_global_nd_strong_);
        ds = C.octreeDownsamplingBatch(ins, 0.05f);
    }
    union_q_ = ds[0];
    saveMap(save_pcd_directory_ + "union_map_queryside.pcd", union_q_);
    union_c_ = ds[1];
    saveMap(save_pcd_directory_ + "union_map_centralside.pcd", union_c_);
    saveMap(save_pcd_directory_ + "pd_map.pcd", ds[2]);
    saveMap(save_pcd_directory_ + "nd_map.pcd", ds[3]);
    LTM_INFO(" Union, PD, and ND map saved ");
    if (has_strong_nd) {
        C.map_global_nd_strong_ = ds[7];
        saveMap(save_pcd_directory_ + "strong_nd_map.pcd", C.map_global_nd_strong_);
    }
    C.map_global_nd_weak_ = ds[4];
    saveMap(save_pcd_directory_ + "weak_nd_map.pcd", C.map_global_nd_weak_);
    LTM_INFO(" Strong/Weak ND map saved ");
    Q.map_global_pd_strong_ = ds[5];
    saveMap(save_pcd_directory_ + "strong_pd_map.pcd", Q.map_global_pd_strong_);
    Q.map_global_pd_weak_ = ds[6];
    saveMap(save_pcd_directory_ + "weak_pd_map.pcd", Q.map_global_pd_weak_);
    LTM_INFO(" Strong/Weak PD map saved ");
}

void Removerter::updateCurrentMap(void)
{
    Session& C = central_sess_;
    CloudPtr updated = C.concat({union_q_, union_c_, C.map_global_nd_weak_});
    LTM_INFO(" -- The number of map points (updating ...): " << updated->size());
    auto ds = C.octreeDownsamplingBatch({C.concat({updated, C.map_global_pd_strong_}), C.concat({updated, C.map_global_pd_orig_})}, 0.05f);
    C.map_global_updated_strong_ = ds[0];
    LTM_INFO(" -- The number of strong map points (updating ...): " << C.map_global_updated_strong_->size());
    C.map_global_updated_ = ds[1];
    LTM_INFO(" -- The number of map points (updating ...): " << C.map_global_updated_->size());
    saveMap(save_pcd_directory_ + "updated_map.pcd", C.map_global_updated_);
    saveMap(save_pcd_directory_ + "updated_map_strong.pcd", C.map_global_updated_strong_);
    LTM_INFO(" -- The updated map is saved ");
}

void Removerter::parseStaticScansViaProjection(Session& _sess)
{
    LTM_INFO(" parse static scans via projection: " << _sess.sess_type_);
    _sess.parseStaticScansViaProjection();
}
void Removerter::parseStaticScansViaProjection(void) { parseStaticScansViaProjection(central_sess_); parseStaticScansViaProjection(query_sess_); }
void Removerter::updateScansScanwise() { updateScansScanwise(central_sess_); }
void Removerter::updateScansScanwise(Session& _sess) { _sess.updateScansScanwise(); LTM_INFO(" final update scans: " << _sess.sess_type_); }
void Removerter::parseUpdatedStaticScansViaProjection() { parseUpdatedStaticScansViaProjection(central_sess_); }
void Removerter::parseUpdatedStaticScansViaProjection(Session& _sess)
{
    _sess.parseUpdatedStaticScansViaProjection();
    _sess.parseUpdatedStrongStaticScansViaProjection();
    LTM_INFO(" parse updated scans via projection: " << _sess.sess_type_);
}
void Removerter::parseLDScansViaProjection() { parseLDScansViaProjection(central_sess_); }
void Removerter::parseLDScansViaProjection(Session& _sess)
{
    _sess.parsePDScansViaProjection();
    _sess.parseStrongPDScansViaProjection();
    _sess.parseWeakNDScansViaProjection();
    if (!_sess.map_global_nd_strong_) { ltm_cloud h = 0; PointType none{}; ltmCheck(dev_->ctx, ltm_cloud_upload(dev_->ctx, &none, 0, 16, &h), "ltm_cloud_upload"); _sess.map_global_nd_strong_ = _sess.wrap(h); }
    _sess.parseStrongNDScansViaProjection();
    LTM_INFO(" parse LD scans via projection: " << _sess.sess_type_);
}

void Removerter::saveAllTypeOfScans() { saveUpdatedScans(central_sess_); saveLDScans(central_sess_); }
void Removerter::saveLDScans(Session& _sess) { savePDScans(_sess); saveStrongPDScans(_sess); saveStrongNDScans(_sess); }
void Removerter::saveUpdatedScans(Session& _sess)
{
    saveScans(_sess, _sess.keyframe_scans_updated_, updated_scans_save_dir_, true);
    saveScans(_sess, _sess.keyframe_scans_updated_strong_, updated_strong_scans_save_dir_, false);
}
void Removerter::savePDScans(Session& _sess) { saveScans(_sess, _sess.keyframe_scans_pd_, pd_scans_save_dir, false); }
void Removerter::saveStrongPDScans(Session& _sess) { saveScans(_sess, _sess.keyframe_scans_strong_pd_, strong_pd_scans_save_dir, false); }
void Removerter::saveStrongNDScans(Session& _sess) { saveScans(_sess, _sess.keyframe_scans_strong_nd_, strong_nd_scans_save_dir, false); }

void Removerter::saveScans(Session& _sess, const ScansPtr& _scans, std::string _save_dir, bool octree_layout)
{
    if (bench_mode_) return;
    const size_t first = _scans->shard ? _scans->kb : 0;
    if (!_scans->shard && dev_->rank() != 0) return;
    if (gpu_async_io_) {
        if (!writer_) writer_.reset(new AsyncWriter((unsigned)std::max(1, kNumOmpCores)));
        ltm_fetch* t = nullptr;
        ltm_ctx* ctx = dev_->ctx;
        const size_t nk = _scans->numKeyframes();
        if (gpu_fetch_chunked_ && ltm_scanset_fetch_chunks_begin(ctx, _scans->h, &t) == LTM_OK) {
            auto ticket = std::make_shared<std::atomic<ltm_fetch*>>(t);
            fetches_.push_back(PendingFetch{ticket, nullptr, _scans});
            auto names = std::make_shared<std::vector<std::string>>();
            for (size_t idx_scan = 0; idx_scan < nk; ++idx_scan) names->push_back(_save_dir + "/" + _sess.keyframe_names_.at(first + idx_scan));
            const size_t pumps = (size_t)std::max(1, kNumOmpCores);
            auto remaining = std::make_shared<std::atomic<size_t>>(pumps);
            for (size_t p = 0; p < pumps; ++p)
                writer_->submit([t, ticket, remaining, ctx, names, octree_layout] {
                    std::exception_ptr failure;
                    const uint64_t* off = nullptr; size_t n_kf = 0;
                    if (ltm_fetch_info(t, nullptr, &off, &n_kf) != LTM_OK || n_kf != names->size())
                        failure = std::make_exception_ptr(std::runtime_error("ltm_fetch_info failed for " + (names->empty() ? std::string("a scan set") : names->front())));
                    for (;;) {
                        const void* pts = nullptr; size_t first_point = 0, cnt = 0, first_kf = 0, kfs = 0;
                        const int rc = ltm_fetch_next_chunk(t, &pts, &first_point, &cnt, &first_kf, &kfs);
                        if (rc <= 0) { if (rc < 0 && !failure) failure = std::make_exception_ptr(std::runtime_error("ltm_fetch_next_chunk failed")); break; }
                        for (size_t k = first_kf; k < first_kf + kfs && !failure; ++k) {
                            std::string err;
// ... 349 lines not shown
    forkLanes(M.ctx, LD.ctx,
        [&] {
            LTM_INFO(" parse low dynamic diff via knn: " << C.sess_type_ << " to " << Q.sess_type_);
            C.extractLowDynPointsViaKnnDiff(Q.map_global_curr_static_);
            C.constructGlobalNDMap();
            filterStrongND(C, Q);
            C.removeWeakNDMapPointsHavingStrongNDInNear();
            const bool has_strong_nd = C.map_global_nd_strong_->size() != 0;
            std::vector<CloudPtr> ins = {C.mergeScansToGlobal(C.scans_knn_coexist_), C.mergeScansToGlobal(C.scans_knn_diff_), C.map_global_nd_weak_};
            if (has_strong_nd) ins.push_back(C.map_global_nd_strong_);
            const auto ds = C.octreeDownsamplingBatch(ins, 0.05f);
            union_c_ = ds[0];
            saveMap(save_pcd_directory_ + "union_map_centralside.pcd", union_c_);
            saveMap(save_pcd_directory_ + "nd_map.pcd", ds[1]);
            if (has_strong_nd) { C.map_global_nd_strong_ = ds[3]; saveMap(save_pcd_directory_ + "strong_nd_map.pcd", C.map_global_nd_strong_); }
            C.map_global_nd_weak_ = ds[2];
            saveMap(save_pcd_directory_ + "weak_nd_map.pcd", C.map_global_nd_weak_);
        },
        [&] {
            Ql.extractLowDynPointsViaKnnDiff(Cl.map_global_curr_static_);
            Ql.constructGlobalPDMap();
            L.filterStrongPD(Ql, Cl);
            Ql.revertStrongPDMapPointsHavingWeakPDInNear();
            const auto ds = Ql.octreeDownsamplingBatch({Ql.mergeScansToGlobal(Ql.scans_knn_coexist_), Ql.mergeScansToGlobal(Ql.scans_knn_diff_),
                                                        Ql.map_global_pd_strong_, Ql.map_global_pd_weak_}, 0.05f);
            L.union_q_ = ds[0];
            L.saveMap(L.save_pcd_directory_ + "union_map_queryside.pcd", L.union_q_);
            L.saveMap(L.save_pcd_directory_ + "pd_map.pcd", ds[1]);
            Ql.map_global_pd_strong_ = ds[2];
            L.saveMap(L.save_pcd_directory_ + "strong_pd_map.pcd", Ql.map_global_pd_strong_);
            Ql.map_global_pd_weak_ = ds[3];
            L.saveMap(L.save_pcd_directory_ + "weak_pd_map.pcd", Ql.map_global_pd_weak_);
        });
    lap("stage B (low dynamic)");
    LTM_INFO(" Union, PD, and ND map saved ");
    LTM_INFO(" Strong/Weak ND map saved ");
    LTM_INFO(" Strong/Weak PD map saved ");
    Q.keyframe_scans_static_projected_.reset(); Q.knn_target_map_.reset(); C.knn_target_map_.reset();
    Cl.map_global_curr_static_.reset(); Cl.keyframe_scans_static_projected_.reset(); Ql.knn_target_map_.reset();
    Q.keyframe_scans_static_projected_ = giveScans(Ql.keyframe_scans_static_projected_, M);
    Q.scans_knn_coexist_ = giveScans(Ql.scans_knn_coexist_, M);
    Q.scans_knn_diff_ = giveScans(Ql.scans_knn_diff_, M);
    const bool pd_is_orig = Ql.map_global_pd_ == Ql.map_global_pd_orig_;
    Q.map_global_pd_orig_ = giveCloud(Ql.map_global_pd_orig_, M);
    if (pd_is_orig) { Ql.map_global_pd_.reset(); Q.map_global_pd_ = Q.map_global_pd_orig_; }
    else Q.map_global_pd_ = giveCloud(Ql.map_global_pd_, M);
    Q.map_global_pd_strong_ = giveCloud(Ql.map_global_pd_strong_, M);
    Q.map_global_pd_weak_ = giveCloud(Ql.map_global_pd_weak_, M);
    union_q_ = giveCloud(L.union_q_, M);
    C.map_global_pd_ = Q.map_global_pd_;
    C.map_global_pd_orig_ = Q.map_global_pd_orig_;
    C.map_global_pd_strong_ = Q.map_global_pd_strong_;

    updateCurrentMap();
    lap("hand-over + updateCurrentMap");
    if (!C.map_global_nd_strong_) { ltm_cloud h = 0; PointType none{}; ltmCheck(M.ctx, ltm_cloud_upload(M.ctx, &none, 0, 16, &h), "ltm_cloud_upload"); C.map_global_nd_strong_ = C.wrap(h); }
    Cl.map_global_pd_strong_ = lendCloud(C.map_global_pd_strong_, LD);
    Cl.map_global_nd_strong_ = lendCloud(C.map_global_nd_strong_, LD);
    Cl.map_global_updated_strong_ = lendCloud(C.map_global_updated_strong_, LD);
    const bool early = write_outputs && gpu_async_io_;
    forkLanes(M.ctx, LD.ctx,
        [&] {
            C.parseUpdatedStaticScansViaProjection();
            C.parsePDScansViaProjection();
            if (early) savePDScans(C);
            C.parseWeakNDScansViaProjection();
            updateScansScanwise();
        },
        [&] {
            Cl.parseStrongPDScansViaProjection();
            if (early) L.saveStrongPDScans(Cl);
            Cl.parseStrongNDScansViaProjection();
            if (early) L.saveStrongNDScans(Cl);
            Cl.parseUpdatedStrongStaticScansViaProjection();
            if (early) L.saveScans(Cl, Cl.keyframe_scans_updated_strong_, L.updated_strong_scans_save_dir_, false);
        });
    lap("stage C (Step 3)");
    LTM_INFO(" parse updated scans via projection: " << C.sess_type_);
    LTM_INFO(" parse LD scans via projection: " << C.sess_type_);
    Cl.map_global_pd_strong_.reset(); Cl.map_global_nd_strong_.reset(); Cl.map_global_updated_strong_.reset();
    C.keyframe_scans_strong_pd_ = giveScans(Cl.keyframe_scans_strong_pd_, M);
    C.keyframe_scans_strong_nd_ = giveScans(Cl.keyframe_scans_strong_nd_, M);
    C.keyframe_scans_updated_strong_ = giveScans(Cl.keyframe_scans_updated_strong_, M);
    Ql.keyframe_scans_.reset();
    if (write_outputs && !gpu_async_io_) {  }
}

void Removerter::run(void)
{
    using clk = std::chrono::steady_clock;
    const auto t0 = clk::now();
    const bool t0_detail = std::getenv("LTM_STEP0_TIMING") != nullptr;
    auto lap = [&, last = t0](const char* what) mutable {
        if (!t0_detail) return;
        ltm_synchronize(dev_->ctx);
        const auto now = clk::now();
        std::fprintf(stderr, "[ltm_run] step 0: %-22s %7.1f ms\n", what, std::chrono::duration<double, std::milli>(now - last).count());
        last = now;
    };
    loadSessionInfo(); lap("loadSessionInfo");
    parseKeyframes(); lap("parseKeyframes");
    central_sess_.loadKeyframes(); lap("loadKeyframes central");
    query_sess_.loadKeyframes(); lap("loadKeyframes query");
    precleaningKeyframes(2.5); lap("precleaningKeyframes");
    const auto t1 = clk::now();
    runStages(true);
    ltmCheck(dev_->ctx, ltm_synchronize(dev_->ctx), "ltm_synchronize");
    const auto t2 = clk::now();
    if (gpu_async_io_) saveScans(central_sess_, central_sess_.keyframe_scans_updated_, updated_scans_save_dir_, true);
    else saveAllTypeOfScans();
    finishOutputs();
    saveKeyframePoses(central_sess_);
    ltmCheck(dev_->ctx, ltm_synchronize(dev_->ctx), "ltm_synchronize");
    if (dev_->comm) dev_->comm->barrier();
    const auto t3 = clk::now();
    auto s = [](auto a, auto b) { return std::chrono::duration<double>(b - a).count(); };
    LTM_INFO(" [timing] step0 (load) " << s(t0, t1) << " s, makeGlobalMap + steps 1-3 " << s(t1, t2) << " s (includes map PCD writes), scan writes " << s(t2, t3) << " s");
    if (dev_->rank() == 0)
    std::cout << "[timing] ranks " << dev_->world() << " (" << (dev_->comm ? dev_->comm->backend() : "single") << ") T_total " << s(t0, t3) << " s T_step0 " << s(t0, t1) << " s T_steps123 " << s(t1, t2) << " s T_scan_writes " << s(t2, t3)
              << " s keyframes " << central_sess_.keyframe_names_.size() << " " << query_sess_.keyframe_names_.size() << std::endl;
}

}
```

### lt-mapper_amd/host/src/Session.cpp

```cpp
#include "removert/Session.h"

#include <cstdio>
#include <chrono>
#include <memory>
#include <algorithm>
#include <cmath>
#include <cstring>
#include <cstdlib>
#include <fstream>
#include <iostream>
#include <atomic>
#include <condition_variable>
#include <mutex>
#include <stdexcept>
#include <thread>

namespace ltremovert
{

size_t Session::kVoxelShardMin = getenv("LTM_VOXEL_SHARD_MIN") ? (size_t)atoll(getenv("LTM_VOXEL_SHARD_MIN")) : ((size_t)1 << 24);

Device::Device(const RosParamServer& p, int device_ordinal, std::shared_ptr<Comm> comm_) : comm(std::move(comm_))
{
    ltm_config cfg{};
// ... 528 lines not shown
        std::vector<uint64_t> sizes;
        comm()->allGatherU64(ctx, n, sizes);
        size_t total = 0;
        for (uint64_t& v : sizes) { total += v; v *= sizeof(PointType); }
        ltmCheck(ctx, ltm_cloud_alloc(ctx, total, &h), "ltm_cloud_alloc");
        CloudPtr out = wrap(h);
        const void *s = nullptr, *d = nullptr;
        ltmCheck(ctx, ltm_cloud_device_ptr(ctx, piece, &s), "ltm_cloud_device_ptr");
        ltmCheck(ctx, ltm_cloud_device_ptr(ctx, h, &d), "ltm_cloud_device_ptr");
        comm()->allGatherV(ctx, s, n * sizeof(PointType), const_cast<void*>(d), sizes);
        ltmCheck(ctx, ltm_synchronize(ctx), "ltm_synchronize");
        return out;
    }
    ltmCheck(ctx, ltm_voxel_centroid(ctx, src->h, leaf, &h), "ltm_voxel_centroid");
    return wrap(h);
}
std::vector<CloudPtr> Session::octreeDownsamplingBatch(const std::vector<CloudPtr>& src, float leaf) const
{
    std::vector<CloudPtr> out(src.size());
    std::vector<size_t> batch;
    for (size_t i = 0; i < src.size(); ++i) {
        if (world() > 1 && src[i]->size() >= kVoxelShardMin) out[i] = octreeDownsampling(src[i], leaf);
        else batch.push_back(i);
    }
    if (!batch.empty()) {
        std::vector<ltm_cloud> in(batch.size()), res(batch.size(), 0);
        std::vector<float> leafs(batch.size(), leaf);
        for (size_t k = 0; k < batch.size(); ++k) in[k] = src[batch[k]]->h;
        ltmCheck(dev_->ctx, ltm_voxel_centroid_batch(dev_->ctx, in.size(), in.data(), leafs.data(), res.data()), "ltm_voxel_centroid_batch");
        for (size_t k = 0; k < batch.size(); ++k) out[batch[k]] = wrap(res[k]);
    }
    return out;
}
CloudPtr Session::concat(const std::vector<CloudPtr>& parts) const
{
    std::vector<ltm_cloud> hs;
    for (const auto& p : parts) if (p) hs.push_back(p->h);
    ltm_cloud h = 0;
    ltmCheck(dev_->ctx, ltm_cloud_concat(dev_->ctx, hs.data(), hs.size(), &h), "ltm_cloud_concat");
    return wrap(h);
}

void Session::mergeScansWithinGlobalCoord(void) { map_global_orig_ = mergeScansToGlobal(keyframe_scans_); }

void Session::parseScansViaProjection(const CloudPtr& _map, ScansPtr& _vec_to_store)
{
    ltm_scanset h = 0;
    ltmCheck(dev_->ctx, ltm_reproject(dev_->ctx, _map->h, poses_h_, kf_begin_, kf_end_, kReprojectionAlpha, &h), "ltm_reproject");
    _vec_to_store = wrap_shard(h);
}
void Session::parseStaticScansViaProjection(void) { parseScansViaProjection(map_global_curr_, keyframe_scans_static_projected_); }
void Session::parseUpdatedStaticScansViaProjection(void) { parseScansViaProjection(map_global_updated_, keyframe_scans_updated_); }
void Session::parseUpdatedStrongStaticScansViaProjection(void) { parseScansViaProjection(map_global_updated_strong_, keyframe_scans_updated_strong_); }
void Session::parsePDScansViaProjection(void) { parseScansViaProjection(map_global_pd_orig_, keyframe_scans_pd_); }
void Session::parseStrongPDScansViaProjection(void) { parseScansViaProjection(map_global_pd_strong_, keyframe_scans_strong_pd_); }
void Session::parseWeakNDScansViaProjection(void) { parseScansViaProjection(map_global_nd_weak_, keyframe_scans_weak_nd_); }
void Session::parseStrongNDScansViaProjection(void) { parseScansViaProjection(map_global_nd_strong_, keyframe_scans_strong_nd_); }

void Session::updateScansScanwise()
{
    ltm_scanset merged = 0, voxelised = 0;
    ltmCheck(dev_->ctx, ltm_scanset_zip_concat(dev_->ctx, keyframe_scans_updated_->h, keyframe_scans_weak_nd_->h, keyframe_scans_pd_->h, &merged), "ltm_scanset_zip_concat");
    ScansPtr guard = wrap_scans(merged);
    ltmCheck(dev_->ctx, ltm_voxel_centroid_scanset(dev_->ctx, merged, 0.05f, &voxelised), "ltm_voxel_centroid_scanset");
    const bool shard = keyframe_scans_updated_->shard;
    keyframe_scans_updated_ = shard ? wrap_shard(voxelised) : wrap_scans(voxelised);
}

static std::pair<CloudPtr, CloudPtr> knnOneScan(const Session& s, const CloudPtr& target, const ScansPtr& scans, int idx)
{
    if (!target) throw std::runtime_error("no kNN target map yet: call extract*ViaKnnDiff first");
    if (scans->shard) throw std::runtime_error("the per-scan kNN wrappers address whole scan sets (single-GPU runs)");
    ltm_scanset co = 0, di = 0;
    ltmCheck(s.dev_->ctx, ltm_knn_partition(s.dev_->ctx, target->h, scans->h, s.poses_h_, (size_t)idx, (size_t)idx + 1, s.kNumKnnPointsToCompare,
                                            s.kScanKnnAndMapKnnAvgDiffThreshold, &co, &di), "ltm_knn_partition");
    const ScansH a(s.dev_->ctx, co), b(s.dev_->ctx, di);
    ltm_cloud ca = 0, cb = 0;
    ltmCheck(s.dev_->ctx, ltm_scanset_keyframe(s.dev_->ctx, co, 0, &ca), "ltm_scanset_keyframe");
    ltmCheck(s.dev_->ctx, ltm_scanset_keyframe(s.dev_->ctx, di, 0, &cb), "ltm_scanset_keyframe");
    return {s.wrap(ca), s.wrap(cb)};
}
std::pair<CloudPtr, CloudPtr> Session::partitionLowDynamicPointsOfScanByKnn(int _scan_idx) { return knnOneScan(*this, knn_target_map_, keyframe_scans_static_projected_, _scan_idx); }
std::pair<CloudPtr, CloudPtr> Session::partitionHighDynamicPointsOfScanByKnn(int _scan_idx) { return knnOneScan(*this, knn_target_map_, keyframe_scans_, _scan_idx); }

void Session::extractLowDynPointsViaKnnDiff(const CloudPtr& _target_map)
{
    knn_target_map_ = _target_map;
    ltm_scanset co = 0, di = 0;
    ltm_poses ph = 0; size_t kb = 0, ke = 0;
    stageArgs(keyframe_scans_static_projected_, &ph, &kb, &ke);
    ltmCheck(dev_->ctx, ltm_knn_partition(dev_->ctx, _target_map->h, keyframe_scans_static_projected_->h, ph, kb, ke,
                                          kNumKnnPointsToCompare, kScanKnnAndMapKnnAvgDiffThreshold, &co, &di), "ltm_knn_partition");
    scans_knn_coexist_ = wrap_shard(co); scans_knn_diff_ = wrap_shard(di);
}

void Session::extractHighDynPointsViaKnnDiff(const CloudPtr& _target_map)
{
    knn_target_map_ = _target_map;
    ltm_scanset di = 0;
    ltm_poses ph = 0; size_t kb = 0, ke = 0;
    stageArgs(keyframe_scans_, &ph, &kb, &ke);
    ltmCheck(dev_->ctx, ltm_knn_partition(dev_->ctx, _target_map->h, keyframe_scans_->h, ph, kb, ke,
                                          kNumKnnPointsToCompare, kScanKnnAndMapKnnAvgDiffThreshold, nullptr, &di), "ltm_knn_partition");
    keyframe_scans_dynamic_ = wrap_shard(di);
}

// ... 20 lines not shown
```

### lt-mapper_amd/removerter.py

```python
import time
from dataclasses import dataclass, field
from typing import List, Optional

import numpy as np


@dataclass
class Params:
    sequence_vfov: float = 50.0
    sequence_hfov: float = 360.0
    remove_resolution_list: List[float] = field(default_factory=lambda: [2.5])
    num_nn_points_within: int = 2
    dist_nn_points_within: float = 0.01
    downsample_voxel_size: float = 0.05
    repeat_removert_iter: int = 1
    ExtrinsicLiDARtoPoseBase: Optional[np.ndarray] = None
    gpu_use_self_removert: bool = False
    gpu_skip_hd_knn: bool = False
    gather_scan_outputs: bool = False


class HipOps:

    def __init__(self, ctx):
        self.ctx = ctx

    def clone(self, c): return c.clone()
    def concat(self, cs): return self.ctx.concat(cs)
    def size(self, c): return len(c)
    def empty_cloud(self): return self.ctx.upload(np.zeros((0, 4), np.float32))
    def merge_to_global(self, scans, poses): return self.ctx.merge_to_global(scans, poses)
    def voxel(self, c, leaf): return self.ctx.voxel_centroid(c, leaf)
    def voxel_batch(self, clouds, leaf): return self.ctx.voxel_centroid_batch(clouds, [leaf] * len(clouds))
    def voxel_shard(self, c, leaf, shard, n_shards): return self.ctx.voxel_centroid_shard(c, leaf, shard, n_shards)
    def bbox(self, c): return self.ctx.bbox(c)
    def voxel_key_histogram(self, c, mn, mx, leaf): return self.ctx.voxel_key_histogram(c, mn, mx, leaf)
    def voxel_key_split(self, c, mn, mx, leaf, cuts): return self.ctx.voxel_key_split(c, mn, mx, leaf, cuts)
    def voxel_box(self, c, mn, mx, leaf): return self.ctx.voxel_centroid_box(c, mn, mx, leaf)

    def merge_voxel_batch(self, merges, clouds, leaf):
        return self.voxel_batch([self.merge_to_global(s, p) for s, p in merges] + list(clouds), leaf)
    def voxel_scanset(self, s, leaf): return self.ctx.voxel_centroid_scanset(s, leaf)
    def voxel_grid_scanset(self, s, leaf): return self.ctx.voxel_grid_scanset(s, leaf)
    supports_deferred_grid = True

    def voxel_grid_scanset_begin(self, s, leaf): return self.ctx.voxel_grid_scanset_begin(s, leaf)
    def voxel_grid_scanset_end(self, ticket): return self.ctx.voxel_grid_scanset_end(ticket)
    def preclean(self, s, radius): return self.ctx.preclean(s, radius)
    def vote_partition(self, cmap, scans, poses, alpha, thr, mode): return self.ctx.visibility_partition(cmap, scans, poses, alpha, thr, mode)
    def prepare_scan_images(self, scans, alphas): self.ctx.prepare_scan_images(scans, alphas)
    def reproject(self, cmap, poses, alpha): return self.ctx.reproject(cmap, poses, alpha)
    def knn_partition(self, target, scans, poses, k, thr): return self.ctx.knn_partition(target, scans, poses, k, thr)
    def knn_split(self, target, query, k, thr): return self.ctx.knn_split_cloud(target, query, k, thr)
    def zip_concat(self, a, b, c): return self.ctx.zip_concat(a, b, c)
    def sync(self): self.ctx.synchronize()
    def materialize(self, scans): return scans
    def lane(self): return HipOps(self.ctx.lane())
    def poses_like(self, poses): return self.ctx.poses(poses.host_poses, poses.host_inv)

    def n_keyframes(self, poses): return poses.n
    def poses_slice(self, poses, kb, ke): return self.ctx.poses(poses.host_poses[kb:ke], poses.host_inv[kb:ke])

    def new_labels(self, n):
        import torch
        t = torch.zeros(max(n, 1), dtype=torch.uint8, device=f"cuda:{self.ctx.device}")[:n]
        torch.cuda.current_stream().synchronize()
        return t

    def vote(self, cmap, scans, poses, kb, ke, alpha, thr, mode, labels):
        if labels.numel():
            self.ctx.visibility_vote(cmap, scans, poses, kb, ke, alpha, thr, mode, labels.data_ptr())

    def partition(self, cmap, labels):
        import torch
        torch.cuda.current_stream().synchronize()
        return self.ctx.partition_by_labels(cmap, labels.data_ptr() if labels.numel() else None)

    def reproject_range(self, cmap, poses, alpha, kb, ke): return self.ctx.reproject(cmap, poses, alpha, kb, ke)
    def knn_partition_range(self, target, scans, poses, k, thr, kb, ke): return self.ctx.knn_partition(target, scans, poses, k, thr, kb, ke)
    def concat_scansets(self, sets): return self.ctx.concat_scansets(sets)

    def scanset_to_tensors(self, ss):
        import torch
        n_kf, n = ss.info()
        off = ss.offsets()
        self.ctx.synchronize()
        if n == 0:
            return torch.zeros((0, 4), dtype=torch.float32, device=f"cuda:{self.ctx.device}"), off
        view = _DeviceArray(ss.device_ptr(), (n, 4), "<f4")
        return torch.as_tensor(view, device=f"cuda:{self.ctx.device}").clone(), off

    def cloud_to_tensor(self, c):
        import torch
        n = len(c)
        self.ctx.synchronize()
        if n == 0:
            return torch.zeros((0, 4), dtype=torch.float32, device=f"cuda:{self.ctx.device}")
        return torch.as_tensor(_DeviceArray(c.device_ptr(), (n, 4), "<f4"), device=f"cuda:{self.ctx.device}")

    def cloud_from_tensor(self, t):
        import torch
        torch.cuda.current_stream().synchronize()
        if t.shape[0] == 0:
            return self.empty_cloud()
# ... 222 lines not shown
        C.scans_knn_coexist_, C.scans_knn_diff_ = self.ops.knn_partition(Q.map_global_curr_static_, C.keyframe_scans_static_projected_, C.keyframe_poses, k, thr)
        Q.scans_knn_coexist_, Q.scans_knn_diff_ = self.ops.knn_partition(C.map_global_curr_static_, Q.keyframe_scans_static_projected_, Q.keyframe_poses, k, thr)
        self._tick("ld_knn", t0)
        t0 = time.perf_counter()
        C.map_global_nd_ = self.mergeVoxelBatch([(C.scans_knn_diff_, C.keyframe_poses)], [], 0.05)[0]
        maps = (C.map_global_nd_, None, None)
        for _ in range(3):
            maps = self._removeOnceLD(maps, Q, 2.5, 1)
        C.map_global_nd_, C.map_global_nd_strong_, C.map_global_nd_weak_ = maps
        if self.ops.size(C.map_global_nd_strong_) != 0:
            add, new_weak = self.ops.knn_split(C.map_global_nd_strong_, C.map_global_nd_weak_, 2, 1.0)
            C.map_global_nd_strong_ = self.ops.concat([C.map_global_nd_strong_, add])
            C.map_global_nd_weak_ = new_weak
        Q.map_global_pd_ = self.mergeVoxelBatch([(Q.scans_knn_diff_, Q.keyframe_poses)], [], 0.05)[0]
        Q.map_global_pd_orig_ = Q.map_global_pd_
        maps = (Q.map_global_pd_, None, None)
        for _ in range(3):
            maps = self._removeOnceLD(maps, C, 2.5, 0)
        Q.map_global_pd_, Q.map_global_pd_strong_, Q.map_global_pd_weak_ = maps
        C.map_global_pd_, C.map_global_pd_orig_, C.map_global_pd_strong_ = Q.map_global_pd_, Q.map_global_pd_orig_, Q.map_global_pd_strong_
        self._tick("ld_filter", t0)
        t0 = time.perf_counter()
        o = self.outputs
        merges = [(Q.scans_knn_coexist_, Q.keyframe_poses), (C.scans_knn_coexist_, C.keyframe_poses),
                  (Q.scans_knn_diff_, Q.keyframe_poses), (C.scans_knn_diff_, C.keyframe_poses)]
        ins = [C.map_global_nd_weak_, Q.map_global_pd_strong_, Q.map_global_pd_weak_]
        has_strong_nd = self.ops.size(C.map_global_nd_strong_) != 0
        if has_strong_nd:
            ins.append(C.map_global_nd_strong_)
        res = self.mergeVoxelBatch(merges, ins, 0.05)
        self._union_q = o["union_map_queryside"] = res[0]
        self._union_c = o["union_map_centralside"] = res[1]
        o["pd_map"], o["nd_map"] = res[2], res[3]
        C.map_global_nd_weak_ = o["weak_nd_map"] = res[4]
        Q.map_global_pd_strong_ = o["strong_pd_map"] = res[5]
        Q.map_global_pd_weak_ = o["weak_pd_map"] = res[6]
        if has_strong_nd:
            C.map_global_nd_strong_ = o["strong_nd_map"] = res[7]
        self._tick("ld_maps", t0)

    def updateCurrentMap(self):
        t0 = time.perf_counter()
        C = self.central_sess_
        updated = self.ops.concat([self._union_q, self._union_c, C.map_global_nd_weak_])
        C.map_global_updated_strong_, C.map_global_updated_ = self.octreeDownsamplingBatch(
            [self.ops.concat([updated, C.map_global_pd_strong_]), self.ops.concat([updated, C.map_global_pd_orig_])], 0.05)
        self.outputs["updated_map"] = C.map_global_updated_
        self.outputs["updated_map_strong"] = C.map_global_updated_strong_
        self._tick("update_map", t0)

    def parseUpdatedStaticScansViaProjection(self):
        t0 = time.perf_counter()
        C = self.central_sess_
        C.keyframe_scans_updated_ = self.ops.reproject(C.map_global_updated_, C.keyframe_poses, self.kReprojectionAlpha)
        C.keyframe_scans_updated_strong_ = self.ops.reproject(C.map_global_updated_strong_, C.keyframe_poses, self.kReprojectionAlpha)
        self._tick("reproject_updated", t0)

    def parseLDScansViaProjection(self):
        t0 = time.perf_counter()
        C = self.central_sess_
        C.keyframe_scans_pd_ = self.ops.reproject(C.map_global_pd_orig_, C.keyframe_poses, self.kReprojectionAlpha)
        C.keyframe_scans_strong_pd_ = self.ops.reproject(C.map_global_pd_strong_, C.keyframe_poses, self.kReprojectionAlpha)
        C.keyframe_scans_weak_nd_ = self.ops.reproject(C.map_global_nd_weak_, C.keyframe_poses, self.kReprojectionAlpha)
        nd_strong = C.map_global_nd_strong_ if C.map_global_nd_strong_ is not None else self.ops.empty_cloud()
        C.keyframe_scans_strong_nd_ = self.ops.reproject(nd_strong, C.keyframe_poses, self.kReprojectionAlpha)
        self._tick("reproject_ld", t0)

    def updateScansScanwise(self):
        t0 = time.perf_counter()
        C = self.central_sess_
        merged = self.ops.zip_concat(C.keyframe_scans_updated_, C.keyframe_scans_weak_nd_, C.keyframe_scans_pd_)
        C.keyframe_scans_updated_ = self.ops.voxel_scanset(merged, 0.05)
        self._tick("update_scans", t0)

    def scan_outputs(self):
        C = self.central_sess_
        return {"scans_updated": C.keyframe_scans_updated_, "scans_updated_strong": C.keyframe_scans_updated_strong_,
                "scans_pd": C.keyframe_scans_pd_, "scans_pd_strong": C.keyframe_scans_strong_pd_,
                "scans_nd_strong": C.keyframe_scans_strong_nd_}

    def _fork(self, main_fn, lane_fn):
        import threading
        M, L = self.ops.ctx, self.lane_ops.ctx
        err = []

        def run():
            try:
                lane_fn()
            except BaseException as e:
                err.append(e)
        M.fence(L)
        th = threading.Thread(target=run)
        th.start()
        try:
            main_fn()
        finally:
            th.join()
        if err:
            raise err[0]
        L.fence(M)

    def run_two_lanes(self):
        ops, lops, P = self.ops, self.lane_ops, self.P
        M, L = ops.ctx, lops.ctx
        C, Q = self.central_sess_, self.query_sess_
        k, thr = P.num_nn_points_within, P.dist_nn_points_within
        o = self.outputs
        t0 = time.perf_counter()
        Ql = Session("Query", M.lend(Q.keyframe_scans_, L), lops.poses_like(Q.keyframe_poses))
# ... 23 lines not shown
        t0 = time.perf_counter()
        Qproj_view = L.lend(Ql.keyframe_scans_static_projected_, M)
        Cstat_view, Cproj_view = M.lend(C.map_global_curr_static_, L), M.lend(C.keyframe_scans_static_projected_, L)
        q_src = Session("Query", None, Q.keyframe_poses); q_src.keyframe_scans_static_projected_ = Qproj_view
        c_src = Session("Central", None, Cl_poses); c_src.keyframe_scans_static_projected_ = Cproj_view

        def central_side():
            C.scans_knn_coexist_, C.scans_knn_diff_ = ops.knn_partition(Q.map_global_curr_static_, C.keyframe_scans_static_projected_, C.keyframe_poses, k, thr)
            C.map_global_nd_ = ops.merge_voxel_batch([(C.scans_knn_diff_, C.keyframe_poses)], [], 0.05)[0]
            maps = (C.map_global_nd_, None, None)
            for _ in range(3):
                maps = self._removeOnceLD(maps, q_src, 2.5, 1, ops)
            C.map_global_nd_, C.map_global_nd_strong_, C.map_global_nd_weak_ = maps
            if ops.size(C.map_global_nd_strong_) != 0:
                add, new_weak = ops.knn_split(C.map_global_nd_strong_, C.map_global_nd_weak_, 2, 1.0)
                C.map_global_nd_strong_ = ops.concat([C.map_global_nd_strong_, add])
                C.map_global_nd_weak_ = new_weak
            has_strong_nd = ops.size(C.map_global_nd_strong_) != 0
            res = ops.merge_voxel_batch([(C.scans_knn_coexist_, C.keyframe_poses), (C.scans_knn_diff_, C.keyframe_poses)],
                                        [C.map_global_nd_weak_] + ([C.map_global_nd_strong_] if has_strong_nd else []), 0.05)
            self._union_c = o["union_map_centralside"] = res[0]
            o["nd_map"] = res[1]
            C.map_global_nd_weak_ = o["weak_nd_map"] = res[2]
            if has_strong_nd:
                C.map_global_nd_strong_ = o["strong_nd_map"] = res[3]

        def query_side():
            Ql.scans_knn_coexist_, Ql.scans_knn_diff_ = lops.knn_partition(Cstat_view, Ql.keyframe_scans_static_projected_, Ql.keyframe_poses, k, thr)
            Ql.map_global_pd_ = lops.merge_voxel_batch([(Ql.scans_knn_diff_, Ql.keyframe_poses)], [], 0.05)[0]
            Ql.map_global_pd_orig_ = Ql.map_global_pd_
            maps = (Ql.map_global_pd_, None, None)
            for _ in range(3):
                maps = self._removeOnceLD(maps, c_src, 2.5, 0, lops)
            Ql.map_global_pd_, Ql.map_global_pd_strong_, Ql.map_global_pd_weak_ = maps
            res = lops.merge_voxel_batch([(Ql.scans_knn_coexist_, Ql.keyframe_poses), (Ql.scans_knn_diff_, Ql.keyframe_poses)],
                                         [Ql.map_global_pd_strong_, Ql.map_global_pd_weak_], 0.05)
            Ql.union_q_, Ql.pd_map_, Ql.map_global_pd_strong_, Ql.map_global_pd_weak_ = res
        self._fork(central_side, query_side)
        del Cstat_view, Cproj_view, Qproj_view
        q_src.keyframe_scans_static_projected_ = c_src.keyframe_scans_static_projected_ = None
        to_main = lambda x: L.give(x, M)
        Q.keyframe_scans_static_projected_ = to_main(Ql.keyframe_scans_static_projected_)
        Q.scans_knn_coexist_, Q.scans_knn_diff_ = to_main(Ql.scans_knn_coexist_), to_main(Ql.scans_knn_diff_)
        same_pd = Ql.map_global_pd_orig_ is Ql.map_global_pd_
        Q.map_global_pd_orig_ = to_main(Ql.map_global_pd_orig_)
        Q.map_global_pd_ = Q.map_global_pd_orig_ if same_pd else to_main(Ql.map_global_pd_)
        self._union_q = o["union_map_queryside"] = to_main(Ql.union_q_)
        o["pd_map"] = to_main(Ql.pd_map_)
        Q.map_global_pd_strong_ = o["strong_pd_map"] = to_main(Ql.map_global_pd_strong_)
        Q.map_global_pd_weak_ = o["weak_pd_map"] = to_main(Ql.map_global_pd_weak_)
        C.map_global_pd_, C.map_global_pd_orig_, C.map_global_pd_strong_ = Q.map_global_pd_, Q.map_global_pd_orig_, Q.map_global_pd_strong_
        self._tick("lanes_low_dynamic", t0)
        t0 = time.perf_counter()
        self.updateCurrentMap()
        nd_strong = C.map_global_nd_strong_ if C.map_global_nd_strong_ is not None else ops.empty_cloud()
        views = [M.lend(x, L) for x in (C.map_global_pd_strong_, nd_strong, C.map_global_updated_strong_)]
        got = {}

        def main_side():
            a = self.kReprojectionAlpha
            C.keyframe_scans_updated_ = ops.reproject(C.map_global_updated_, C.keyframe_poses, a)
            C.keyframe_scans_pd_ = ops.reproject(C.map_global_pd_orig_, C.keyframe_poses, a)
            C.keyframe_scans_weak_nd_ = ops.reproject(C.map_global_nd_weak_, C.keyframe_poses, a)
            merged = ops.zip_concat(C.keyframe_scans_updated_, C.keyframe_scans_weak_nd_, C.keyframe_scans_pd_)
            C.keyframe_scans_updated_ = ops.voxel_scanset(merged, 0.05)

        def lane_side():
            a = self.kReprojectionAlpha
            got["strong_pd"] = lops.reproject(views[0], Cl_poses, a)
            got["strong_nd"] = lops.reproject(views[1], Cl_poses, a)
            got["updated_strong"] = lops.reproject(views[2], Cl_poses, a)
        self._fork(main_side, lane_side)
        del views
        C.keyframe_scans_strong_pd_, C.keyframe_scans_strong_nd_ = to_main(got["strong_pd"]), to_main(got["strong_nd"])
        C.keyframe_scans_updated_strong_ = to_main(got["updated_strong"])
        self._tick("lanes_step3", t0)
        self.outputs.update(central_map_static=C.map_global_curr_static_, central_map_dynamic=C.map_global_curr_dynamic_,
                            query_map_static=Q.map_global_curr_static_, query_map_dynamic=Q.map_global_curr_dynamic_)

    def run_steps_1_to_3(self):
        self.removeHighDynamicPoints()
        self.parseStaticScansViaProjection()
        self.detectLowDynamicPoints()
        self.updateCurrentMap()
        self.parseUpdatedStaticScansViaProjection()
        self.parseLDScansViaProjection()
        self.updateScansScanwise()
        C, Q = self.central_sess_, self.query_sess_
        if self.P.gather_scan_outputs:
            for name in ("keyframe_scans_updated_", "keyframe_scans_updated_strong_", "keyframe_scans_pd_", "keyframe_scans_strong_pd_",
                         "keyframe_scans_strong_nd_"):
                setattr(C, name, self.ops.materialize(getattr(C, name)))
        self.outputs.update(central_map_static=C.map_global_curr_static_, central_map_dynamic=C.map_global_curr_dynamic_,
                            query_map_static=Q.map_global_curr_static_, query_map_dynamic=Q.map_global_curr_dynamic_)

    def run(self):
        if self.lane_ops is not None and self.query_side is None and self._rankGroups() is None:
            return self.run_two_lanes()
        if self.central_scans_future is not None and (self.query_side is not None or self._rankGroups() is not None):
            self.central_sess_.keyframe_scans_ = self.central_scans_future()
            self.central_scans_future = None
        if self.query_side is None and self._rankGroups() is None and self.central_scans_future is None:
            self.makeGlobalMap()
        self.run_steps_1_to_3()
```

Before: 3487 keyframe-pairs/s.

## Fuse reprojection of updated and strong-updated maps via deduplicated union pass

Adds a paired reprojection path. It hash-joins the two maps, which largely overlap, into a deduplicated union with partner indices, then projects that union once into two sets of range images. It falls back to two separate reprojections when the overlap ratio is too low or the geometry is not fusable. The Step-3 schedule is also reordered: the pd, weak-nd and strong reprojections run on the lane while updateCurrentMap runs on main, and then the fused pair runs. This adds hash-table build cost and a host sync to read the union size, and the reordering changes which work overlaps.

```diff
diff --git a/include/ltm.h b/include/ltm.h
--- a/include/ltm.h
+++ b/include/ltm.h
@@ -116,6 +116,9 @@
                              float diff_thres, int mode, ltm_cloud* kept, ltm_cloud* flagged, uint8_t* host_labels);
 
 int ltm_reproject(ltm_ctx*, ltm_cloud map, ltm_poses poses, size_t kf_begin, size_t kf_end, float res_alpha, ltm_scanset* out);
+int ltm_reproject_pair(ltm_ctx*, ltm_cloud map_a, ltm_cloud map_b, ltm_poses poses, size_t kf_begin, size_t kf_end, float res_alpha, ltm_scanset* out_a,
+                       ltm_scanset* out_b);
+int ltm_reproject_pair_legal(ltm_ctx*, ltm_cloud map_a, ltm_cloud map_b, ltm_poses poses, size_t kf_begin, size_t kf_end, float res_alpha, int* legal);
 
 int ltm_knn_partition(ltm_ctx*, ltm_cloud target, ltm_scanset scans, ltm_poses poses, size_t kf_begin, size_t kf_end,
                       int k, float thr, ltm_scanset* coexist, ltm_scanset* diff);
diff --git a/lt-mapper_amd/capi.py b/lt-mapper_amd/capi.py
--- a/lt-mapper_amd/capi.py
+++ b/lt-mapper_amd/capi.py
@@ -128,6 +128,8 @@
     "ltm_scanset_lend": (_i, [_vp, _u64, _vp, _pu64]),
     "ltm_scanset_give": (_i, [_vp, _u64, _vp, _pu64]),
     "ltm_reproject": (_i, [_vp, _u64, _u64, _sz, _sz, _f, _pu64]),
+    "ltm_reproject_pair": (_i, [_vp, _u64, _u64, _u64, _sz, _sz, _f, _pu64, _pu64]),
+    "ltm_reproject_pair_legal": (_i, [_vp, _u64, _u64, _u64, _sz, _sz, _f, C.POINTER(C.c_int)]),
     "ltm_knn_partition": (_i, [_vp, _u64, _u64, _u64, _sz, _sz, _i, _f, _pu64, _pu64]),
     "ltm_knn_split_cloud": (_i, [_vp, _u64, _u64, _i, _f, _pu64, _pu64]),
     "ltm_search_build": (_i, [_vp, _u64, C.POINTER(_vp)]),
@@ -534,6 +536,16 @@
         self._ck(self.lib.ltm_reproject(self.h, cmap.h, poses.h, kf_begin, poses.n if kf_end is None else kf_end, alpha, C.byref(out)))
         return ScanSet(self, out.value)
 
+    def reproject_pair(self, map_a, map_b, poses, alpha=3.0, kf_begin=0, kf_end=None):
+        a, b = _u64(), _u64()
+        self._ck(self.lib.ltm_reproject_pair(self.h, map_a.h, map_b.h, poses.h, kf_begin, poses.n if kf_end is None else kf_end, alpha, C.byref(a), C.byref(b)))
+        return ScanSet(self, a.value), ScanSet(self, b.value)
+
+    def reproject_pair_legal(self, map_a, map_b, poses, alpha=3.0, kf_begin=0, kf_end=None):
+        legal = C.c_int(0)
+        self._ck(self.lib.ltm_reproject_pair_legal(self.h, map_a.h, map_b.h, poses.h, kf_begin, poses.n if kf_end is None else kf_end, alpha, C.byref(legal)))
+        return bool(legal.value)
+
     def knn_partition(self, target, scans, poses, k, thr, kf_begin=0, kf_end=None):
         co, di = _u64(), _u64()
         self._ck(self.lib.ltm_knn_partition(self.h, target.h, scans.h, poses.h, kf_begin, poses.n if kf_end is None else kf_end,
diff --git a/lt-mapper_amd/csrc/ltm_api_core.cpp b/lt-mapper_amd/csrc/ltm_api_core.cpp
--- a/lt-mapper_amd/csrc/ltm_api_core.cpp
+++ b/lt-mapper_amd/csrc/ltm_api_core.cpp
@@ -222,6 +222,7 @@
     c->kopts.map_tile_persist = env_int("LTM_MAP_TILE_PERSIST", 1);
     c->kopts.map_tile_barrier = env_int("LTM_MAP_TILE_BARRIER", 0);
     c->kopts.stats_blockmin = env_int("LTM_STATS_BLOCKMIN", 0);
+    c->kopts.reproject_pair = std::min(std::max(env_int("LTM_REPROJECT_PAIR", 1), 0), 2);
     {
         unsigned long long* d = nullptr;
         bool ok = hipMalloc(&d, 3 * sizeof(unsigned long long)) == hipSuccess && hipMemsetAsync(d, 0, 24, c->stream) == hipSuccess &&
diff --git a/lt-mapper_amd/csrc/ltm_api_vote.cpp b/lt-mapper_amd/csrc/ltm_api_vote.cpp
--- a/lt-mapper_amd/csrc/ltm_api_vote.cpp
+++ b/lt-mapper_amd/csrc/ltm_api_vote.cpp
@@ -322,6 +322,78 @@
 }
 
 
+struct ReprojectOut {
+    ltm_ctx* c; const Cloud map; const Poses& p; size_t kf_begin, nk, npx;
+    std::vector<uint64_t> off;
+    struct Piece { float4* d; size_t n; };
+    std::vector<Piece> pieces;
+    ReprojectOut(ltm_ctx* c_, const Cloud& map_, const Poses& p_, size_t kf_begin_, size_t kf_end, size_t npx_)
+        : c(c_), map(map_), p(p_), kf_begin(kf_begin_), nk(kf_end - kf_begin_), npx(npx_), off(nk + 1, 0) {}
+    void batch(const uint64_t* img, size_t kb, size_t nb, uint32_t* pos, void* temp, size_t tb, uint32_t* bout)
+    {
+        ProfScope ps(c, "reproject_gather", (double)(nb * npx), (double)(nb * npx) * 12);
+        LTM_HIP(exclusive_scan_img_valid(img, pos, nb * npx, temp, tb, c->stream));
+        LTM_HIP(image_bounds(pos, img, npx, nb, bout, c->stream));
+        std::vector<uint32_t> b(nb + 1);
+        d2h(c, b.data(), bout, (nb + 1) * 4);
+        const size_t total = b[nb];
+        const uint64_t base = off[kb - kf_begin];
+        for (size_t j = 1; j <= nb; ++j) off[kb - kf_begin + j] = base + b[j];
+        float4* d = reinterpret_cast<float4*>(c->pool.alloc(std::max<size_t>(total, 1) * 16));
+        LTM_HIP(reproject_gather(img, pos, npx, nb, map.d, p.inv_dev, kb, c->B2L, c->b2l_identity, d, c->stream));
+        pieces.push_back(Piece{d, total});
+    }
+    ltm_scanset finish()
+    {
+        float4* d = nullptr;
+        if (pieces.size() == 1) d = pieces[0].d;
+        else {
+            d = reinterpret_cast<float4*>(c->pool.alloc(std::max<size_t>(off[nk], 1) * 16));
+            size_t at = 0;
+            for (Piece& pc : pieces) { d2d(c, d + at, pc.d, pc.n * 16); at += pc.n; }
+            sync(c);
+            for (Piece& pc : pieces) c->pool.free(pc.d);
+        }
+        return new_scanset(c, d, std::move(off));
+    }
+};
+
+void do_reproject(ltm_ctx* c, const Cloud& map, const Poses& p, size_t kf_begin, size_t kf_end, float alpha, ltm_scanset* out)
+{
+    LTM_REQUIRE(kf_begin <= kf_end && kf_end <= p.n, "keyframe range out of bounds");
+    LTM_REQUIRE(map.n < 0xffffffffull, "map too large for 32-bit point indices");
+    const Geom g = geom_for(c, alpha);
+    LTM_REQUIRE(g.rows > 0 && g.cols > 0, "empty range image");
+    const size_t npx = (size_t)g.rows * g.cols;
+    ReprojectOut ro(c, map, p, kf_begin, kf_end, npx);
+    if (ro.nk && map.n) {
+        const size_t KB = std::min(c->kf_batch, ro.nk);
+        DevBuf img(c, KB * npx * 8), pos(c, KB * npx * 4);
+        const size_t tb = scan_temp_bytes(KB * npx);
+        DevBuf temp(c, tb), bout(c, (KB + 1) * 4);
+        for (size_t kb = kf_begin; kb < kf_end; kb += KB) {
+            const size_t nb = std::min(KB, kf_end - kb);
+            LTM_HIP(fill_u64(img.as<uint64_t>(), (uint64_t)kNoPointBits << 32, nb * npx, c->stream));
+            {
+                ProfScope ps(c, "reproject_map", (double)map.n * nb, (double)nb * (16.0 * map.n + 8.0 * npx), 16.0 * map.n + (double)nb * 8.0 * npx);
+                exact_map_images(c, map, p, kb, nb, g, img.as<uint64_t>());
+            }
+            ro.batch(img.as<uint64_t>(), kb, nb, pos.as<uint32_t>(), temp.p, tb, bout.as<uint32_t>());
+        }
+    }
+    *out = ro.finish();
+}
+
+static bool pair_legal(ltm_ctx* c, const Cloud& A, const Cloud& B, const Poses& p, size_t kf_begin, size_t nk, const Geom& g)
+{
+    const size_t KB = std::min(c->kf_batch, std::max<size_t>(nk, 1));
+    const size_t na_pad = (A.n + 4095) / 4096 * 4096;
+    if (c->kopts.reproject_pair == 0 || !nk || !A.n || !B.n || !p.approx_dev || na_pad + B.n >= 0xffffffffull) return false;
+    if (!pair_fusable(g, c->B2L, c->b2l_identity, c->kopts) || !cull_geometry_ok(c, g, p, kf_begin)) return false;
+    return !(c->occlusion_cull && ((na_pad + B.n + 4095) / 4096) * KB >= c->occlusion_min_pairs);
+}
+static constexpr double kPairRho = 1.50;
+
 }
 
 extern "C" {
@@ -378,52 +450,79 @@
 {
     return guarded(c, [&] {
         LTM_REQUIRE(out, "null argument");
-        const Cloud map = get_cloud(c, hmap);
+        do_reproject(c, get_cloud(c, hmap), get_poses(c, hp), kf_begin, kf_end, alpha, out);
+    });
+}
+
+int ltm_reproject_pair_legal(ltm_ctx* c, ltm_cloud hmap_a, ltm_cloud hmap_b, ltm_poses hp, size_t kf_begin, size_t kf_end, float alpha, int* legal)
+{
+    return guarded(c, [&] {
+        LTM_REQUIRE(legal, "null argument");
         const Poses& p = get_poses(c, hp);
         LTM_REQUIRE(kf_begin <= kf_end && kf_end <= p.n, "keyframe range out of bounds");
-        LTM_REQUIRE(map.n < 0xffffffffull, "map too large for 32-bit point indices");
         const Geom g = geom_for(c, alpha);
         LTM_REQUIRE(g.rows > 0 && g.cols > 0, "empty range image");
-        const size_t npx = (size_t)g.rows * g.cols;
-        const size_t nk = kf_end - kf_begin;
-        std::vector<uint64_t> off(nk + 1, 0);
-        struct Piece { float4* d; size_t n; };
-        std::vector<Piece> pieces;
-        if (nk && map.n) {
-            const size_t KB = std::min(c->kf_batch, nk);
-            DevBuf img(c, KB * npx * 8), pos(c, KB * npx * 4);
-            const size_t tb = scan_temp_bytes(KB * npx);
-            DevBuf temp(c, tb), bout(c, (KB + 1) * 4);
-            for (size_t kb = kf_begin; kb < kf_end; kb += KB) {
-                const size_t nb = std::min(KB, kf_end - kb);
-                LTM_HIP(fill_u64(img.as<uint64_t>(), (uint64_t)kNoPointBits << 32, nb * npx, c->stream));
-                {
-                    ProfScope ps(c, "reproject_map", (double)map.n * nb, (double)nb * (16.0 * map.n + 8.0 * npx), 16.0 * map.n + (double)nb * 8.0 * npx);
-                    exact_map_images(c, map, p, kb, nb, g, img.as<uint64_t>());
-                }
-                ProfScope ps(c, "reproject_gather", (double)(nb * npx), (double)(nb * npx) * 12);
-                LTM_HIP(exclusive_scan_img_valid(img.as<uint64_t>(), pos.as<uint32_t>(), nb * npx, temp.p, tb, c->stream));
-                LTM_HIP(image_bounds(pos.as<uint32_t>(), img.as<uint64_t>(), npx, nb, bout.as<uint32_t>(), c->stream));
-                std::vector<uint32_t> b(nb + 1);
-                d2h(c, b.data(), bout.p, (nb + 1) * 4);
-                const size_t total = b[nb];
-                const uint64_t base = off[kb - kf_begin];
-                for (size_t j = 1; j <= nb; ++j) off[kb - kf_begin + j] = base + b[j];
-                float4* d = reinterpret_cast<float4*>(c->pool.alloc(std::max<size_t>(total, 1) * 16));
-                LTM_HIP(reproject_gather(img.as<uint64_t>(), pos.as<uint32_t>(), npx, nb, map.d, p.inv_dev, kb, c->B2L, c->b2l_identity, d, c->stream));
-                pieces.push_back(Piece{d, total});
+        *legal = pair_legal(c, get_cloud(c, hmap_a), get_cloud(c, hmap_b), p, kf_begin, kf_end - kf_begin, g) ? 1 : 0;
+    });
+}
+
+int ltm_reproject_pair(ltm_ctx* c, ltm_cloud hmap_a, ltm_cloud hmap_b, ltm_poses hp, size_t kf_begin, size_t kf_end, float alpha, ltm_scanset* out_a, ltm_scanset* out_b)
+{
+    return guarded(c, [&] {
+        LTM_REQUIRE(out_a && out_b, "null argument");
+        const Cloud A = get_cloud(c, hmap_a), B = get_cloud(c, hmap_b);
+        const Poses& p = get_poses(c, hp);
+        LTM_REQUIRE(kf_begin <= kf_end && kf_end <= p.n, "keyframe range out of bounds");
+        LTM_REQUIRE(A.n < 0xffffffffull && B.n < 0xffffffffull, "map too large for 32-bit point indices");
+        const Geom g = geom_for(c, alpha);
+        LTM_REQUIRE(g.rows > 0 && g.cols > 0, "empty range image");
+        const size_t npx = (size_t)g.rows * g.cols, nk = kf_end - kf_begin;
+        const size_t KB = std::min(c->kf_batch, std::max<size_t>(nk, 1));
+        const size_t na_pad = (A.n + 4095) / 4096 * 4096;
+        bool fused = pair_legal(c, A, B, p, kf_begin, nk, g);
+        size_t n_union = 0;
+        std::unique_ptr<DevBuf> un, partner;
+        if (fused) {
+            const size_t slots = pair_table_slots(B.n), tb = scan_temp_bytes(B.n + 1);
+            un.reset(new DevBuf(c, (na_pad + B.n) * 16)); partner.reset(new DevBuf(c, (na_pad + B.n) * 4));
+            DevBuf table(c, slots * 4), free_b(c, (B.n + 1) * 4), pos(c, (B.n + 1) * 4), temp(c, tb);
+            ProfScope ps(c, "reproject_map", 0.0, 0.0, 0.0, false);
+            LTM_HIP(pair_join(A.d, A.n, B.d, B.n, table.as<uint32_t>(), slots, free_b.as<uint32_t>(), pos.as<uint32_t>(), temp.p, tb, un->as<float4>(), partner->as<uint32_t>(), c->stream));
+            uint32_t n_tail = 0;
+            d2h(c, &n_tail, pos.as<uint32_t>() + B.n, 4);
+            const size_t n_or = A.n + n_tail;
+            if (c->kopts.reproject_pair == 1 && !(kPairRho * (double)n_or < (double)A.n + (double)B.n)) fused = false;
+            else {
+                LTM_HIP(pair_join_tail(B.d, B.n, free_b.as<uint32_t>(), pos.as<uint32_t>(), A.n, un->as<float4>(), partner->as<uint32_t>(), c->stream));
+                n_union = na_pad + n_tail;
             }
         }
-        float4* d = nullptr;
-        if (pieces.size() == 1) d = pieces[0].d;
-        else {
-            d = reinterpret_cast<float4*>(c->pool.alloc(std::max<size_t>(off[nk], 1) * 16));
-            size_t at = 0;
-            for (Piece& pc : pieces) { d2d(c, d + at, pc.d, pc.n * 16); at += pc.n; }
-            sync(c);
-            for (Piece& pc : pieces) c->pool.free(pc.d);
-        }
-        *out = new_scanset(c, d, std::move(off));
+        if (!fused) {
+            un.reset(); partner.reset();
+            do_reproject(c, A, p, kf_begin, kf_end, alpha, out_a);
+            do_reproject(c, B, p, kf_begin, kf_end, alpha, out_b);
+            return;
+        }
+        ReprojectOut ra(c, A, p, kf_begin, kf_end, npx), rb(c, B, p, kf_begin, kf_end, npx);
+        DevBuf img_a(c, KB * npx * 8), img_b(c, KB * npx * 8), pos(c, KB * npx * 4);
+        const size_t tb = scan_temp_bytes(KB * npx);
+        DevBuf temp(c, tb), bout(c, (KB + 1) * 4);
+        for (size_t kb = kf_begin; kb < kf_end; kb += KB) {
+            const size_t nb = std::min(KB, kf_end - kb);
+            LTM_HIP(fill_u64(img_a.as<uint64_t>(), (uint64_t)kNoPointBits << 32, nb * npx, c->stream));
+            LTM_HIP(fill_u64(img_b.as<uint64_t>(), (uint64_t)kNoPointBits << 32, nb * npx, c->stream));
+            {
+                ProfScope ps(c, "reproject_map", (double)n_union * nb, (double)nb * (16.0 * (A.n + B.n) + 16.0 * npx), 16.0 * (A.n + B.n) + (double)nb * 16.0 * npx);
+                HeavyScope hs(c, ((n_union + 4095) / 4096) * nb);
+                LTM_HIP(map_range_images_pair(un->as<float4>(), partner->as<uint32_t>(), n_union, p.inv_dev, p.approx_dev, kb, nb, c->B2L, c->b2l_identity, g,
+                                              img_a.as<uint64_t>(), img_b.as<uint64_t>(), hs.stream(), c->kopts));
+                hs.done();
+            }
+            ra.batch(img_a.as<uint64_t>(), kb, nb, pos.as<uint32_t>(), temp.p, tb, bout.as<uint32_t>());
+            rb.batch(img_b.as<uint64_t>(), kb, nb, pos.as<uint32_t>(), temp.p, tb, bout.as<uint32_t>());
+        }
+        *out_a = ra.finish();
+        *out_b = rb.finish();
     });
 }
 
diff --git a/lt-mapper_amd/csrc/ltm_k_projection.hip b/lt-mapper_amd/csrc/ltm_k_projection.hip
--- a/lt-mapper_amd/csrc/ltm_k_projection.hip
+++ b/lt-mapper_amd/csrc/ltm_k_projection.hip
@@ -305,7 +305,7 @@
 }
 
 
-__device__ unsigned long long g_cull_stats[4];
+__device__ unsigned long long g_cull_stats[6];
 
 static constexpr int kCullQueue = 2048;
 
@@ -647,12 +647,12 @@
 
 hipError_t cull_stats(unsigned long long* out2, int reset, hipStream_t s, int which_kernel)
 {
-    hipError_t e = hipMemcpyFromSymbolAsync(out2, HIP_SYMBOL(g_cull_stats), 16, 16 * (size_t)(which_kernel ? 1 : 0), hipMemcpyDeviceToHost, s);
+    hipError_t e = hipMemcpyFromSymbolAsync(out2, HIP_SYMBOL(g_cull_stats), 16, 16 * (size_t)(which_kernel < 0 ? 0 : which_kernel > 2 ? 2 : which_kernel), hipMemcpyDeviceToHost, s);
     if (e != hipSuccess) return e;
     e = hipStreamSynchronize(s);
     if (e != hipSuccess || !reset) return e;
-    const unsigned long long z[4] = {0, 0, 0, 0};
-    e = hipMemcpyToSymbolAsync(HIP_SYMBOL(g_cull_stats), z, 32, 0, hipMemcpyHostToDevice, s);
+    const unsigned long long z[6] = {0, 0, 0, 0, 0, 0};
+    e = hipMemcpyToSymbolAsync(HIP_SYMBOL(g_cull_stats), z, 48, 0, hipMemcpyHostToDevice, s);
     return e == hipSuccess ? hipStreamSynchronize(s) : e;
 }
 
@@ -1093,6 +1093,321 @@
     return hipGetLastError();
 }
 
+static constexpr uint32_t kPairNone = 0xffffffffu;
+static constexpr uint32_t kPairProbeMax = 1024;
+__device__ __forceinline__ uint32_t pair_hash(float4 p)
+{
+    uint32_t h = f2u(p.x) * 0x9E3779B1u;
+    h = (h ^ (h >> 15) ^ f2u(p.y)) * 0x85EBCA77u;
+    h = (h ^ (h >> 13) ^ f2u(p.z)) * 0xC2B2AE3Du;
+    return h ^ (h >> 16);
+}
+__global__ void __launch_bounds__(kBlock)
+k_pair_hash_insert(const float4* __restrict__ b, uint32_t nb_pts, uint32_t* __restrict__ table, uint32_t mask)
+{
+    const uint32_t j = blockIdx.x * kBlock + threadIdx.x;
+    if (j >= nb_pts) return;
+    uint32_t h = pair_hash(b[j]) & mask;
+    for (uint32_t k = 0; k <= mask; ++k, h = (h + 1u) & mask)
+        if (atomicCAS(&table[h], kPairNone, j) == kPairNone) break;
+}
+__global__ void __launch_bounds__(kBlock)
+k_pair_probe(const float4* __restrict__ a, uint32_t na, uint32_t na_pad, const float4* __restrict__ b, const uint32_t* __restrict__ table, uint32_t mask,
+             uint32_t* __restrict__ free_b, float4* __restrict__ un, uint32_t* __restrict__ partner)
+{
+    const uint32_t i = blockIdx.x * kBlock + threadIdx.x;
+    if (i >= na_pad) return;
+    if (i >= na) { const float nan = u2f(0x7fc00000u); un[i] = make_float4(nan, nan, nan, 0.0f); partner[i] = kPairNone; return; }
+    const float4 p = a[i];
+    uint32_t found = kPairNone;
+    uint32_t h = pair_hash(p) & mask;
+    for (uint32_t k = 0; k < kPairProbeMax; ++k, h = (h + 1u) & mask) {
+        const uint32_t j = table[h];
+        if (j == kPairNone) break;
+        const float4 q = b[j];
+        if (f2u(q.x) == f2u(p.x) && f2u(q.y) == f2u(p.y) && f2u(q.z) == f2u(p.z) && free_b[j] != 0u && atomicCAS(&free_b[j], 1u, 0u) == 1u) { found = j; break; }
+    }
+    un[i] = make_float4(p.x, p.y, p.z, u2f(found != kPairNone ? 3u : 1u));
+    partner[i] = found;
+}
+__global__ void __launch_bounds__(kBlock)
+k_pair_tail(const float4* __restrict__ b, uint32_t nb_pts, const uint32_t* __restrict__ free_b, const uint32_t* __restrict__ pos, float4* __restrict__ un_tail,
+            uint32_t* __restrict__ partner_tail)
+{
+    const uint32_t j = blockIdx.x * kBlock + threadIdx.x;
+    if (j >= nb_pts || free_b[j] == 0u) return;
+    const float4 q = b[j];
+    un_tail[pos[j]] = make_float4(q.x, q.y, q.z, u2f(2u));
+    partner_tail[pos[j]] = j;
+}
+size_t pair_table_slots(size_t nb_pts) { size_t s = 1024; while (s < 2 * nb_pts) s <<= 1; return s; }
+hipError_t pair_join(const float4* a, size_t na, const float4* b, size_t nb_pts, uint32_t* table, size_t slots, uint32_t* free_b, uint32_t* pos, void* temp, size_t temp_bytes,
+                     float4* un, uint32_t* partner, hipStream_t s)
+{
+    const size_t per_block = (size_t)kBlock * kPtsPerThread;
+    const size_t na_pad = (na + per_block - 1) / per_block * per_block;
+    hipError_t e = hipMemsetAsync(table, 0xff, slots * 4, s);
+    if (e != hipSuccess) return e;
+    if ((e = fill_u32(free_b, 1u, nb_pts, s)) != hipSuccess) return e;
+    if ((e = hipMemsetAsync(free_b + nb_pts, 0, 4, s)) != hipSuccess) return e;
+    k_pair_hash_insert<<<dim3(grid_for(nb_pts)), dim3(kBlock), 0, s>>>(b, (uint32_t)nb_pts, table, (uint32_t)(slots - 1));
+    k_pair_probe<<<dim3(grid_for(na_pad)), dim3(kBlock), 0, s>>>(a, (uint32_t)na, (uint32_t)na_pad, b, table, (uint32_t)(slots - 1), free_b, un, partner);
+    if ((e = hipGetLastError()) != hipSuccess) return e;
+    return exclusive_scan_u32(free_b, pos, nb_pts + 1, temp, temp_bytes, s);
+}
+hipError_t pair_join_tail(const float4* b, size_t nb_pts, const uint32_t* free_b, const uint32_t* pos, size_t na, float4* un, uint32_t* partner, hipStream_t s)
+{
+    const size_t per_block = (size_t)kBlock * kPtsPerThread;
+    const size_t na_pad = (na + per_block - 1) / per_block * per_block;
+    k_pair_tail<<<dim3(grid_for(nb_pts)), dim3(kBlock), 0, s>>>(b, (uint32_t)nb_pts, free_b, pos, un + na_pad, partner + na_pad);
+    return hipGetLastError();
+}
+
+template <int ROWS, int COLS>
+__device__ __forceinline__ void pair_min(uint64_t* __restrict__ vals, uint32_t* __restrict__ tags, uint64_t* __restrict__ img_a, uint64_t* __restrict__ img_b,
+                                         const uint32_t* __restrict__ partner, int row, int col, uint32_t px, uint64_t rb, uint32_t i, uint32_t memb)
+{
+    const uint64_t v = rb | (uint64_t)i;
+    if (memb != 3u) {
+        if (memb & 1u) img_min_u64(img_a + px, v);
+        else if (memb & 2u) img_min_u64(img_b + px, rb | (uint64_t)partner[i]);
+        return;
+    }
+    const int slot = table_claim<ROWS, COLS>(tags, row, col, px);
+    if (slot < 0) { img_min_u64(img_a + px, v); img_min_u64(img_b + px, rb | (uint64_t)partner[i]); return; }
+    const uint64_t cur = vals[slot];
+    if (v < cur) {
+        const uint64_t old = atomicMin(reinterpret_cast<unsigned long long*>(&vals[slot]), (unsigned long long)v);
+        if ((old >> 32) == (v >> 32) && old != v) img_min_u64(img_b + px, rb | (uint64_t)partner[(uint32_t)(old > v ? old : v)]);
+    } else if ((cur >> 32) == (v >> 32) && cur != v) img_min_u64(img_b + px, rb | (uint64_t)partner[i]);
+}
+template <int SLOTS>
+__device__ __forceinline__ void pair_flush(const uint32_t* __restrict__ tags, const uint64_t* __restrict__ vals, uint64_t* __restrict__ img_a, uint64_t* __restrict__ img_b,
+                                           const uint32_t* __restrict__ partner)
+{
+    for (int s = threadIdx.x; s < SLOTS; s += kBlock) {
+        const uint32_t tg = tags[s];
+        const uint64_t v = vals[s];
+        if (tg == kEmptyTag || v == ~0ull) continue;
+        img_min_u64(img_a + tg, v);
+        img_min_u64(img_b + tg, (v & 0xffffffff00000000ull) | (uint64_t)partner[(uint32_t)v]);
+    }
+}
+template <bool B2L_IDENTITY, int ROWS, int COLS>
+__device__ __forceinline__ void exact_insert_pair(const float4* __restrict__ un, const uint32_t* __restrict__ partner, uint32_t i, const Mat34& Tinv, const HostMat34& b2l_h,
+                                                  const RimgGeom& g, uint64_t* __restrict__ vals, uint32_t* __restrict__ tags, uint64_t* __restrict__ img_a,
+                                                  uint64_t* __restrict__ img_b)
+{
+    const float4 p4 = un[i];
+    const uint32_t memb = f2u(p4.w);
+    if (!memb) return;
+    float3 p = xform(Tinv, make_float3(p4.x, p4.y, p4.z));
+    if (B2L_IDENTITY) p = xform_identity(p); else p = xform(to_dev(b2l_h), p);
+    const Sph s = cart2sph(p.x, p.y, p.z);
+    int row, col;
+    pixel_row_col(g, s.az, s.el, row, col);
+    pair_min<ROWS, COLS>(vals, tags, img_a, img_b, partner, row, col, (uint32_t)(row * g.cols + col), (uint64_t)f2u(s.r) << 32, i, memb);
+}
+
+template <bool B2L_IDENTITY, bool EL3>
+__global__ void __launch_bounds__(kBlock) __attribute__((amdgpu_waves_per_eu(7, 7)))
+k_map_rimg_blockmin_pair(const float4* __restrict__ un, const uint32_t* __restrict__ partner, uint32_t M, const double* __restrict__ inv_poses,
+                         const float* __restrict__ approx_poses, uint32_t kb, uint32_t nb, HostMat34 b2l_h, ProjLaunch pl, RunLaunch rl, uint64_t* __restrict__ img_a,
+                         uint64_t* __restrict__ img_b)
+{
+    constexpr int kRows = 16, kSlots = kRows * 64;
+    __shared__ uint64_t vals[kSlots];
+    __shared__ uint32_t tags[kSlots];
+    __shared__ uint32_t amin[kSlots];
+    __shared__ uint32_t queue[kBmRunSeg * (kBlock / 64)];
+    __shared__ uint16_t uqueue[kBmRunUQueue];
+    __shared__ uint32_t ucount;
+    const uint32_t per_block = (uint32_t)(kBlock * kPtsPerThread);
+    const RunKf rk = run_kf_of_block(blockIdx.x, rl, nb);
+    if (!rk.valid) return;
+    const RimgGeom& g = pl.g;
+    const uint32_t kf = kb + rk.kfb;
+    const uint32_t first_tile = rk.run * rl.T;
+    const uint32_t run_base = first_tile * per_block;
+    const uint32_t n_run = min(rl.T, pl.n_tiles - first_tile);
+    uint64_t* __restrict__ imga = img_a + (size_t)rk.kfb * pl.npx;
+    uint64_t* __restrict__ imgb = img_b + (size_t)rk.kfb * pl.npx;
+    const float* __restrict__ ap = approx_poses + 16 * (size_t)kf;
+    const double* __restrict__ inv_pose = inv_poses + 12 * (size_t)kf;
+    for (int s = threadIdx.x; s < kSlots; s += kBlock) { tags[s] = kEmptyTag; amin[s] = 0x7f800000u; vals[s] = ~0ull; }
+    if (threadIdx.x == 0) ucount = 0;
+    __syncthreads();
+    const uint32_t n_full = (first_tile + n_run == pl.n_tiles && (M & (per_block - 1u)) != 0u) ? n_run - 1u : n_run;
+    const uint32_t n_fast = (pl.vote_queueable & ((f2u(ap[15]) << 1) != 0u)) ? n_full : 0u;
+    const float4* __restrict__ mapr = un + run_base;
+    uint32_t* __restrict__ seg = queue + (uint32_t)__builtin_amdgcn_readfirstlane((int)(threadIdx.x >> 6)) * kBmRunSeg;
+    const uint32_t lane = threadIdx.x & 63u;
+    const uint32_t wave_off = threadIdx.x & 192u;
+    uint32_t nq = 0, nsurv = 0;
+    auto drain = [&]() {
+        __builtin_amdgcn_fence(__ATOMIC_ACQ_REL, "wavefront");
+        const Mat34 Tinv = load_mat(inv_pose);
+        for (uint32_t q = lane; q < nq; q += 64u) {
+            const uint32_t e = seg[q];
+            const uint32_t off = ((e >> 24) << 8) | wave_off | ((e >> kVoteQueuePxBits) & 63u);
+            const uint32_t px = e & kVoteQueuePxUncertain;
+            if (px == kVoteQueuePxUncertain) {
+                const uint32_t ticket = atomicAdd(&ucount, 1u);
+                if (ticket < (uint32_t)kBmRunUQueue) uqueue[ticket] = (uint16_t)off;
+                else exact_insert_pair<B2L_IDENTITY, kRows, 64>(un, partner, run_base + off, Tinv, b2l_h, g, vals, tags, imga, imgb);
+                continue;
+            }
+            const uint32_t i = run_base + off;
+            uint32_t row, col;
+            vote_queue_row_col(px, (uint32_t)g.cols, pl.px_magic, pl.px_shift, row, col);
+            const float4 p4 = un[i];
+            pair_min<kRows, 64>(vals, tags, imga, imgb, partner, (int)row, (int)col, px, (uint64_t)exact_range_bits<B2L_IDENTITY>(p4, Tinv, b2l_h) << 32, i, f2u(p4.w));
+        }
+        nsurv += nq;
+        nq = 0;
+        __builtin_amdgcn_s_waitcnt(0x0f70);
+    };
+    float4 nxt[4];
+    if (n_fast) {
+#pragma unroll
+        for (int u = 0; u < 4; ++u) nxt[u] = mapr[(uint32_t)u * kBlock + threadIdx.x];
+    }
+    uint32_t rec[kPtsPerThread];
+    uint32_t svm = 0;
+    bool resume = false;
+    uint32_t jstart = 0;
+    for (uint32_t t = 0;;) {
+        const float4* __restrict__ mapt = mapr + t * per_block;
+        const bool last = t == n_fast;
+        if (resume | (last & (nq != 0u))) {
+            drain();
+            if (!last) {
+                const float4* __restrict__ nx = t + 1u < n_fast ? mapt + per_block : mapt + 12 * kBlock;
+#pragma unroll
+                for (int u = 0; u < 4; ++u) nxt[u] = nx[(uint32_t)u * kBlock + threadIdx.x];
+            }
+        }
+        if (last) break;
+        if (!resume) {
+        float rlo[kPtsPerThread];
+        uint32_t both = 0;
+#pragma unroll
+        for (int j0 = 0; j0 < kPtsPerThread; j0 += 4) {
+            float3 p[4];
+            CullCand cc[4];
+#pragma unroll
+            for (int u = 0; u < 4; ++u) {
+                bool ok;
+                p[u] = xform_approx(ap, nxt[u], ok);
+                both |= f2u(nxt[u].w) == 3u ? (1u << (j0 + u)) : 0u;
+            }
+            const float4* __restrict__ nx = j0 < 12 ? mapt + (j0 + 4) * kBlock : (t + 1u < n_fast ? mapt + per_block : mapt + 12 * kBlock);
+#pragma unroll
+            for (int u = 0; u < 4; ++u) nxt[u] = nx[(uint32_t)u * kBlock + threadIdx.x];
+#pragma unroll
+            for (int u = 0; u < 4; ++u) cc[u] = cull_candidates<EL3>(pl, p[u]);
+#pragma unroll
+            for (int u = 0; u < 4; ++u) {
+                const int j = j0 + u;
+                const bool certain = pixel_certain(pl, cc[u]);
+                const uint32_t px = __umul24((uint32_t)cc[u].rb, (uint32_t)g.cols) + (uint32_t)cc[u].cb;
+                rec[j] = certain ? px : kVoteQueuePxUncertain;
+                const float r_lo = cull_r_lo(cc[u].r2);
+                rlo[j] = -1.0f;
+                if (certain) {
+                    const int slot = table_claim<kRows, 64>(tags, cc[u].rb, cc[u].cb, px);
+                    if (slot >= 0) {
+                        rec[j] |= (uint32_t)slot << kVoteQueuePxBits;
+                        const uint32_t hi = f2u(r_lo * (1.0f + 3.5e-6f));
+                        if (((both >> j) & 1u) && hi < amin[slot]) atomicMin(&amin[slot], hi);
+                        rlo[j] = r_lo;
+                    }
+                }
+            }
+        }
+        svm = 0;
+#pragma unroll
+        for (int j0 = 0; j0 < kPtsPerThread; j0 += 4) {
+            float am[4];
+#pragma unroll
+            for (int u = 0; u < 4; ++u) am[u] = u2f(amin[rec[j0 + u] >> kVoteQueuePxBits]);
+#pragma unroll
+            for (int u = 0; u < 4; ++u) svm |= (rlo[j0 + u] > am[u]) ? 0u : (1u << (j0 + u));
+        }
+        jstart = 0;
+        }
+        const uint32_t word = (t << 28) | (lane << kVoteQueuePxBits);
+        resume = false;
+#pragma unroll
+        for (int j0 = 0; j0 < kPtsPerThread; j0 += 4) {
+            if ((uint32_t)j0 < jstart) continue;
+            bool sv[4];
+#pragma unroll
+            for (int u = 0; u < 4; ++u) sv[u] = ((svm >> (j0 + u)) & 1u) != 0u;
+            const uint64_t b0 = __builtin_amdgcn_ballot_w64(sv[0]), b1 = __builtin_amdgcn_ballot_w64(sv[1]),
+                           b2 = __builtin_amdgcn_ballot_w64(sv[2]), b3 = __builtin_amdgcn_ballot_w64(sv[3]);
+            const uint32_t n0 = (uint32_t)__popcll(b0), n1 = (uint32_t)__popcll(b1), n2 = (uint32_t)__popcll(b2), n3 = (uint32_t)__popcll(b3);
+            const uint32_t total = n0 + n1 + n2 + n3;
+            if (!total) continue;
+            if (__builtin_expect(nq + total > kBmRunSeg, 0)) { jstart = (uint32_t)j0; resume = true; break; }
+            const uint64_t bal[4] = {b0, b1, b2, b3};
+            const uint32_t off[4] = {nq, nq + n0, nq + n0 + n1, nq + n0 + n1 + n2};
+#pragma unroll
+            for (int u = 0; u < 4; ++u) {
+                if (!sv[u]) continue;
+                const uint32_t below = __builtin_amdgcn_mbcnt_hi((uint32_t)(bal[u] >> 32), __builtin_amdgcn_mbcnt_lo((uint32_t)bal[u], 0u));
+                seg[off[u] + below] = (word | ((uint32_t)(j0 + u) << 24)) | (rec[j0 + u] & kVoteQueuePxUncertain);
+            }
+            nq += total;
+        }
+        if (!resume) ++t;
+    }
+    if (__builtin_expect(n_fast < n_run, 0)) {
+        const Mat34 Tinv = load_mat(inv_pose);
+        for (uint32_t t = n_fast; t < n_run; ++t) {
+            const uint32_t block_base = run_base + t * per_block;
+            const uint32_t nloc = min(per_block, M - block_base);
+            for (uint32_t li = threadIdx.x; li < nloc; li += kBlock)
+                exact_insert_pair<B2L_IDENTITY, kRows, 64>(un, partner, block_base + li, Tinv, b2l_h, g, vals, tags, imga, imgb);
+            if (nloc == per_block) nsurv += per_block / (kBlock / 64);
+        }
+    }
+    if ((blockIdx.x & 63u) == 0u) {
+        if (threadIdx.x == 0) atomicAdd(&g_cull_stats[5], (unsigned long long)(n_full * per_block));
+        if (lane == 0u && nsurv) atomicAdd(&g_cull_stats[4], (unsigned long long)nsurv);
+    }
+    __syncthreads();
+    {
+        const uint32_t nu = min(ucount, (uint32_t)kBmRunUQueue);
+        if (nu) {
+            const Mat34 Tinv = load_mat(inv_pose);
+            for (uint32_t q = threadIdx.x; q < nu; q += kBlock)
+                exact_insert_pair<B2L_IDENTITY, kRows, 64>(un, partner, run_base + uqueue[q], Tinv, b2l_h, g, vals, tags, imga, imgb);
+        }
+    }
+    __syncthreads();
+    pair_flush<kSlots>(tags, vals, imga, imgb, partner);
+}
+
+bool pair_fusable(Geom g, HostMat34 b2l, int b2l_identity, const KernelOpts& ko)
+{
+    return ko.map_kernel_variant >= 2 && make_proj_launch(g, b2l, b2l_identity, 1).vote_queueable;
+}
+hipError_t map_range_images_pair(const float4* un, const uint32_t* partner, size_t M, const double* inv_poses_dev, const float* approx_poses_dev, size_t kb, size_t nb,
+                                 HostMat34 b2l, int b2l_identity, Geom g, uint64_t* img_a, uint64_t* img_b, hipStream_t s, const KernelOpts& ko)
+{
+    if (!M || !nb) return hipSuccess;
+    const ProjLaunch pl = make_proj_launch(g, b2l, b2l_identity, M);
+    uint32_t T = ko.map_tile_run > 0 ? (uint32_t)ko.map_tile_run : kBmRunDefaultT;
+    if (ko.map_tile_run <= 0)
+        while (T > 1u && (uint64_t)((pl.n_tiles + T - 1u) / T) * nb < kBmRunMinBlocks) T >>= 1;
+    const RunLaunch rl = make_run_launch(pl.n_tiles, T);
+    dim3 grid(run_kf_grid(rl, nb));
+    LTM_LAUNCH_ID_EL3(k_map_rimg_blockmin_pair, b2l_identity, g.el_fit != 0, grid, s, un, partner, (uint32_t)M, inv_poses_dev, approx_poses_dev, (uint32_t)kb, (uint32_t)nb, b2l, pl,
+                      rl, img_a, img_b);
+    return hipGetLastError();
+}
+
 struct SphereRect { int r0, r1, c0, c1; float d_lo; bool cullable; };
 __device__ __forceinline__ SphereRect sphere_rect(const RimgGeom& g, const float* __restrict__ ap, const float* __restrict__ tb)
 {
diff --git a/lt-mapper_amd/csrc/ltm_kernels.h b/lt-mapper_amd/csrc/ltm_kernels.h
--- a/lt-mapper_amd/csrc/ltm_kernels.h
+++ b/lt-mapper_amd/csrc/ltm_kernels.h
@@ -38,10 +38,18 @@
     int map_tile_run = 0;
     int map_tile_persist = 1;
     int map_tile_barrier = 0;
+    int reproject_pair = 1;
     int stats_blockmin = 0;
 };
 hipError_t map_range_images(const float4* map, size_t M, const double* inv_poses_dev, const float* approx_poses_dev, size_t kb, size_t nb,
                             HostMat34 b2l, int b2l_identity, Geom g, uint64_t* map_img, hipStream_t s, const KernelOpts& ko);
+size_t pair_table_slots(size_t nb_pts);
+hipError_t pair_join(const float4* a, size_t na, const float4* b, size_t nb_pts, uint32_t* table, size_t slots, uint32_t* free_b, uint32_t* pos, void* temp, size_t temp_bytes,
+                     float4* un, uint32_t* partner, hipStream_t s);
+hipError_t pair_join_tail(const float4* b, size_t nb_pts, const uint32_t* free_b, const uint32_t* pos, size_t na, float4* un, uint32_t* partner, hipStream_t s);
+bool pair_fusable(Geom g, HostMat34 b2l, int b2l_identity, const KernelOpts& ko);
+hipError_t map_range_images_pair(const float4* un, const uint32_t* partner, size_t M, const double* inv_poses_dev, const float* approx_poses_dev, size_t kb, size_t nb,
+                                 HostMat34 b2l, int b2l_identity, Geom g, uint64_t* img_a, uint64_t* img_b, hipStream_t s, const KernelOpts& ko);
 hipError_t occlusion_shell_pairs(const float* approx_poses_dev, size_t kb, size_t nb, const float* tile_bounds_dev, size_t n_tiles, Geom g, float r_lo, float r_hi,
                                  const uint64_t* img, int use_cmax, uint32_t* cmax, uint8_t* done, uint8_t* flags, uint32_t* pos, uint32_t* list, uint32_t* count,
                                  void* temp, size_t temp_bytes, hipStream_t s, uint32_t* dirty_rows = nullptr,
diff --git a/lt-mapper_amd/dist.py b/lt-mapper_amd/dist.py
--- a/lt-mapper_amd/dist.py
+++ b/lt-mapper_amd/dist.py
@@ -82,6 +82,9 @@
 
     def __getattr__(self, name):
         return getattr(self.ops, name)
+
+    reproject_pair = None
+    reproject_pair_legal = None
 
     def _range(self, poses):
         return shard_range(self.ops.n_keyframes(poses), self.rank, self.world)
@@ -287,6 +290,13 @@
         return self.ops.vote_partition(cmap, scans, poses, alpha, thr, mode)
 
     def reproject(self, cmap, poses, alpha): return self._mark(self.ops.reproject(cmap, poses, alpha))
+
+    @property
+    def reproject_pair(self):
+        pair = getattr(self.ops, "reproject_pair", None)
+        if pair is None:
+            return None
+        return lambda map_a, map_b, poses, alpha: tuple(self._mark(s) for s in pair(map_a, map_b, poses, alpha))
 
     def knn_partition(self, target, scans, poses, k, thr):
         co, di = self.ops.knn_partition(target, scans, poses, k, thr)
diff --git a/lt-mapper_amd/host/removert/Session.h b/lt-mapper_amd/host/removert/Session.h
--- a/lt-mapper_amd/host/removert/Session.h
+++ b/lt-mapper_amd/host/removert/Session.h
@@ -123,6 +123,8 @@
     void parseStaticScansViaProjection(void);
     void parseUpdatedStaticScansViaProjection(void);
     void parseUpdatedStrongStaticScansViaProjection(void);
+    void parseUpdatedPairViaProjection(void);
+    bool updatedPairFusable(void) const;
     void parsePDScansViaProjection(void);
     void parseStrongPDScansViaProjection(void);
     void parseWeakNDScansViaProjection(void);
diff --git a/lt-mapper_amd/host/src/Removerter.cpp b/lt-mapper_amd/host/src/Removerter.cpp
--- a/lt-mapper_amd/host/src/Removerter.cpp
+++ b/lt-mapper_amd/host/src/Removerter.cpp
@@ -496,8 +496,7 @@
 void Removerter::parseUpdatedStaticScansViaProjection() { parseUpdatedStaticScansViaProjection(central_sess_); }
 void Removerter::parseUpdatedStaticScansViaProjection(Session& _sess)
 {
-    _sess.parseUpdatedStaticScansViaProjection();
-    _sess.parseUpdatedStrongStaticScansViaProjection();
+    _sess.parseUpdatedPairViaProjection();
     LTM_INFO(" parse updated scans via projection: " << _sess.sess_type_);
 }
 void Removerter::parseLDScansViaProjection() { parseLDScansViaProjection(central_sess_); }
@@ -953,36 +952,47 @@
     C.map_global_pd_orig_ = Q.map_global_pd_orig_;
     C.map_global_pd_strong_ = Q.map_global_pd_strong_;
 
-    updateCurrentMap();
-    lap("hand-over + updateCurrentMap");
+    lap("hand-over");
     if (!C.map_global_nd_strong_) { ltm_cloud h = 0; PointType none{}; ltmCheck(M.ctx, ltm_cloud_upload(M.ctx, &none, 0, 16, &h), "ltm_cloud_upload"); C.map_global_nd_strong_ = C.wrap(h); }
+    Cl.map_global_pd_orig_ = lendCloud(C.map_global_pd_orig_, LD);
     Cl.map_global_pd_strong_ = lendCloud(C.map_global_pd_strong_, LD);
+    Cl.map_global_nd_weak_ = lendCloud(C.map_global_nd_weak_, LD);
     Cl.map_global_nd_strong_ = lendCloud(C.map_global_nd_strong_, LD);
-    Cl.map_global_updated_strong_ = lendCloud(C.map_global_updated_strong_, LD);
     const bool early = write_outputs && gpu_async_io_;
     forkLanes(M.ctx, LD.ctx,
+        [&] { updateCurrentMap(); },
         [&] {
-            C.parseUpdatedStaticScansViaProjection();
-            C.parsePDScansViaProjection();
-            if (early) savePDScans(C);
-            C.parseWeakNDScansViaProjection();
-            updateScansScanwise();
-        },
-        [&] {
+            Cl.parsePDScansViaProjection();
+            if (early) L.savePDScans(Cl);
             Cl.parseStrongPDScansViaProjection();
             if (early) L.saveStrongPDScans(Cl);
+            Cl.parseWeakNDScansViaProjection();
             Cl.parseStrongNDScansViaProjection();
             if (early) L.saveStrongNDScans(Cl);
-            Cl.parseUpdatedStrongStaticScansViaProjection();
-            if (early) L.saveScans(Cl, Cl.keyframe_scans_updated_strong_, L.updated_strong_scans_save_dir_, false);
         });
+    Cl.map_global_pd_orig_.reset(); Cl.map_global_pd_strong_.reset(); Cl.map_global_nd_weak_.reset(); Cl.map_global_nd_strong_.reset();
+    C.keyframe_scans_pd_ = giveScans(Cl.keyframe_scans_pd_, M);
+    C.keyframe_scans_strong_pd_ = giveScans(Cl.keyframe_scans_strong_pd_, M);
+    C.keyframe_scans_weak_nd_ = giveScans(Cl.keyframe_scans_weak_nd_, M);
+    C.keyframe_scans_strong_nd_ = giveScans(Cl.keyframe_scans_strong_nd_, M);
+    if (C.updatedPairFusable()) {
+        C.parseUpdatedPairViaProjection();
+        if (early) saveScans(C, C.keyframe_scans_updated_strong_, updated_strong_scans_save_dir_, false);
+    } else {
+        Cl.map_global_updated_strong_ = lendCloud(C.map_global_updated_strong_, LD);
+        forkLanes(M.ctx, LD.ctx,
+            [&] { C.parseUpdatedStaticScansViaProjection(); },
+            [&] {
+                Cl.parseUpdatedStrongStaticScansViaProjection();
+                if (early) L.saveScans(Cl, Cl.keyframe_scans_updated_strong_, L.updated_strong_scans_save_dir_, false);
+            });
+        Cl.map_global_updated_strong_.reset();
+        C.keyframe_scans_updated_strong_ = giveScans(Cl.keyframe_scans_updated_strong_, M);
+    }
+    updateScansScanwise();
     lap("stage C (Step 3)");
     LTM_INFO(" parse updated scans via projection: " << C.sess_type_);
     LTM_INFO(" parse LD scans via projection: " << C.sess_type_);
-    Cl.map_global_pd_strong_.reset(); Cl.map_global_nd_strong_.reset(); Cl.map_global_updated_strong_.reset();
-    C.keyframe_scans_strong_pd_ = giveScans(Cl.keyframe_scans_strong_pd_, M);
-    C.keyframe_scans_strong_nd_ = giveScans(Cl.keyframe_scans_strong_nd_, M);
-    C.keyframe_scans_updated_strong_ = giveScans(Cl.keyframe_scans_updated_strong_, M);
     Ql.keyframe_scans_.reset();
     if (write_outputs && !gpu_async_io_) {  }
 }
diff --git a/lt-mapper_amd/host/src/Session.cpp b/lt-mapper_amd/host/src/Session.cpp
--- a/lt-mapper_amd/host/src/Session.cpp
+++ b/lt-mapper_amd/host/src/Session.cpp
@@ -604,6 +604,23 @@
 void Session::parseStaticScansViaProjection(void) { parseScansViaProjection(map_global_curr_, keyframe_scans_static_projected_); }
 void Session::parseUpdatedStaticScansViaProjection(void) { parseScansViaProjection(map_global_updated_, keyframe_scans_updated_); }
 void Session::parseUpdatedStrongStaticScansViaProjection(void) { parseScansViaProjection(map_global_updated_strong_, keyframe_scans_updated_strong_); }
+bool Session::updatedPairFusable(void) const
+{
+    if (world() > 1) return false;
+    int legal = 0;
+    ltmCheck(dev_->ctx, ltm_reproject_pair_legal(dev_->ctx, map_global_updated_->h, map_global_updated_strong_->h, poses_h_, kf_begin_, kf_end_, kReprojectionAlpha, &legal),
+             "ltm_reproject_pair_legal");
+    return legal != 0;
+}
+void Session::parseUpdatedPairViaProjection(void)
+{
+    if (world() > 1) { parseUpdatedStaticScansViaProjection(); parseUpdatedStrongStaticScansViaProjection(); return; }
+    ltm_scanset ha = 0, hb = 0;
+    ltmCheck(dev_->ctx, ltm_reproject_pair(dev_->ctx, map_global_updated_->h, map_global_updated_strong_->h, poses_h_, kf_begin_, kf_end_, kReprojectionAlpha, &ha, &hb),
+             "ltm_reproject_pair");
+    keyframe_scans_updated_ = wrap_shard(ha);
+    keyframe_scans_updated_strong_ = wrap_shard(hb);
+}
 void Session::parsePDScansViaProjection(void) { parseScansViaProjection(map_global_pd_orig_, keyframe_scans_pd_); }
 void Session::parseStrongPDScansViaProjection(void) { parseScansViaProjection(map_global_pd_strong_, keyframe_scans_strong_pd_); }
 void Session::parseWeakNDScansViaProjection(void) { parseScansViaProjection(map_global_nd_weak_, keyframe_scans_weak_nd_); }
diff --git a/lt-mapper_amd/removerter.py b/lt-mapper_amd/removerter.py
--- a/lt-mapper_amd/removerter.py
+++ b/lt-mapper_amd/removerter.py
@@ -50,6 +50,8 @@
     def vote_partition(self, cmap, scans, poses, alpha, thr, mode): return self.ctx.visibility_partition(cmap, scans, poses, alpha, thr, mode)
     def prepare_scan_images(self, scans, alphas): self.ctx.prepare_scan_images(scans, alphas)
     def reproject(self, cmap, poses, alpha): return self.ctx.reproject(cmap, poses, alpha)
+    def reproject_pair(self, map_a, map_b, poses, alpha): return self.ctx.reproject_pair(map_a, map_b, poses, alpha)
+    def reproject_pair_legal(self, map_a, map_b, poses, alpha): return self.ctx.reproject_pair_legal(map_a, map_b, poses, alpha)
     def knn_partition(self, target, scans, poses, k, thr): return self.ctx.knn_partition(target, scans, poses, k, thr)
     def knn_split(self, target, query, k, thr): return self.ctx.knn_split_cloud(target, query, k, thr)
     def zip_concat(self, a, b, c): return self.ctx.zip_concat(a, b, c)
@@ -378,9 +380,14 @@
     def parseUpdatedStaticScansViaProjection(self):
         t0 = time.perf_counter()
         C = self.central_sess_
-        C.keyframe_scans_updated_ = self.ops.reproject(C.map_global_updated_, C.keyframe_poses, self.kReprojectionAlpha)
-        C.keyframe_scans_updated_strong_ = self.ops.reproject(C.map_global_updated_strong_, C.keyframe_poses, self.kReprojectionAlpha)
+        C.keyframe_scans_updated_, C.keyframe_scans_updated_strong_ = self._reprojectUpdatedPair(self.ops, C.map_global_updated_, C.map_global_updated_strong_, C.keyframe_poses)
         self._tick("reproject_updated", t0)
+
+    def _reprojectUpdatedPair(self, ops, updated, updated_strong, poses):
+        pair = getattr(ops, "reproject_pair", None)
+        if pair is not None:
+            return pair(updated, updated_strong, poses, self.kReprojectionAlpha)
+        return ops.reproject(updated, poses, self.kReprojectionAlpha), ops.reproject(updated_strong, poses, self.kReprojectionAlpha)
 
     def parseLDScansViaProjection(self):
         t0 = time.perf_counter()
@@ -510,28 +517,33 @@
         C.map_global_pd_, C.map_global_pd_orig_, C.map_global_pd_strong_ = Q.map_global_pd_, Q.map_global_pd_orig_, Q.map_global_pd_strong_
         self._tick("lanes_low_dynamic", t0)
         t0 = time.perf_counter()
-        self.updateCurrentMap()
         nd_strong = C.map_global_nd_strong_ if C.map_global_nd_strong_ is not None else ops.empty_cloud()
-        views = [M.lend(x, L) for x in (C.map_global_pd_strong_, nd_strong, C.map_global_updated_strong_)]
+        views = [M.lend(x, L) for x in (C.map_global_pd_orig_, C.map_global_pd_strong_, C.map_global_nd_weak_, nd_strong)]
         got = {}
-
-        def main_side():
-            a = self.kReprojectionAlpha
-            C.keyframe_scans_updated_ = ops.reproject(C.map_global_updated_, C.keyframe_poses, a)
-            C.keyframe_scans_pd_ = ops.reproject(C.map_global_pd_orig_, C.keyframe_poses, a)
-            C.keyframe_scans_weak_nd_ = ops.reproject(C.map_global_nd_weak_, C.keyframe_poses, a)
-            merged = ops.zip_concat(C.keyframe_scans_updated_, C.keyframe_scans_weak_nd_, C.keyframe_scans_pd_)
-            C.keyframe_scans_updated_ = ops.voxel_scanset(merged, 0.05)
 
         def lane_side():
             a = self.kReprojectionAlpha
-            got["strong_pd"] = lops.reproject(views[0], Cl_poses, a)
-            got["strong_nd"] = lops.reproject(views[1], Cl_poses, a)
-            got["updated_strong"] = lops.reproject(views[2], Cl_poses, a)
-        self._fork(main_side, lane_side)
+            for name, view in zip(("pd", "strong_pd", "weak_nd", "strong_nd"), views):
+                got[name] = lops.reproject(view, Cl_poses, a)
+        self._fork(self.updateCurrentMap, lane_side)
         del views
+        C.keyframe_scans_pd_, C.keyframe_scans_weak_nd_ = to_main(got["pd"]), to_main(got["weak_nd"])
         C.keyframe_scans_strong_pd_, C.keyframe_scans_strong_nd_ = to_main(got["strong_pd"]), to_main(got["strong_nd"])
-        C.keyframe_scans_updated_strong_ = to_main(got["updated_strong"])
+        legal = getattr(ops, "reproject_pair_legal", None)
+        if legal is None or legal(C.map_global_updated_, C.map_global_updated_strong_, C.keyframe_poses, self.kReprojectionAlpha):
+            C.keyframe_scans_updated_, C.keyframe_scans_updated_strong_ = self._reprojectUpdatedPair(ops, C.map_global_updated_, C.map_global_updated_strong_, C.keyframe_poses)
+        else:
+            view = M.lend(C.map_global_updated_strong_, L)
+
+            def main_side():
+                C.keyframe_scans_updated_ = ops.reproject(C.map_global_updated_, C.keyframe_poses, self.kReprojectionAlpha)
+
+            def strong_side():
+                got["updated_strong"] = lops.reproject(view, Cl_poses, self.kReprojectionAlpha)
+            self._fork(main_side, strong_side)
+            del view
+            C.keyframe_scans_updated_strong_ = to_main(got["updated_strong"])
+        self.updateScansScanwise()
         self._tick("lanes_step3", t0)
         self.outputs.update(central_map_static=C.map_global_curr_static_, central_map_dynamic=C.map_global_curr_dynamic_,
                             query_map_static=Q.map_global_curr_static_, query_map_dynamic=Q.map_global_curr_dynamic_)
```

Result: no change. 3486 keyframe-pairs/s, median of 2 (-0.0%).
